# antonilo/unsupervised_detection

Hardware: NVIDIA B200
Metric: frame-pairs/sec adversarial train step 256x448 (higher is better)
Workload: dtype bf16

## Files before the change

### include/cis_b200.h

```cpp
#ifndef CIS_B200_H_
#define CIS_B200_H_
#include <stdint.h>
#include <stddef.h>

#ifdef __cplusplus
extern "C" {
#endif

typedef void* cis_stream_t;

enum { CIS_OK = 0, CIS_ERR_BAD_ARG = 1, CIS_ERR_UNSUPPORTED = 2, CIS_ERR_CUDA = 3 };
enum { CIS_ACT_NONE = 0, CIS_ACT_ELU = 1, CIS_ACT_LEAKY = 2 };
enum { CIS_MAX_TAPS = 49, CIS_MAX_SRC = 4 };

typedef struct {
  const void* ptr;
  int32_t pitch;
  int32_t c_off;
  int32_t chunks;
  int32_t n_mod;
} CisSrc;

typedef struct {
  int32_t N, H, W;
  int32_t OH, OW;
  int32_t sh, sw;
  int32_t ntaps;
  int16_t dh[CIS_MAX_TAPS];
  int16_t dw[CIS_MAX_TAPS];
  int32_t nsrc;
  CisSrc src[CIS_MAX_SRC];
  const void* wpack;
  int32_t K_pad;
  int32_t BN;
  int32_t n_tiles;
  const float* bias;
  int32_t act;
  float alpha;
  int32_t DH, DW;
  int32_t osh, osw, oa, ob;
  void* out;
  int32_t out_pitch, out_coff, out_ch;
  float* outf;
  int32_t outf_pitch, outf_coff, outf_ch;
  const void* add_pre;
  int32_t add_pre_pitch, add_pre_coff;
  const float* addf_pre;
  int32_t addf_pitch, addf_coff;
  const void* add_post;
  int32_t add_post_pitch, add_post_coff;
  int32_t mode;
  int32_t halo;
  int32_t dil;
  int32_t MT;
  int32_t hoy, hox;
  int32_t ey, ex;
  int32_t splits;
  float* sk_scratch;
  int32_t* sk_counters;
  int32_t nph;
  int32_t ph_tap[5];
  int32_t sk_cluster;
  int32_t nsub;
  struct {
    int32_t tap0, ntaps;
    int32_t hoy, hox;
    int32_t OH, OW, oa, ob;
    const void* wpack;
  } sub[4];
} CisConv;

typedef struct {
  int32_t N, H, W, OH, OW, sh, sw, ntaps;
  int16_t dh[CIS_MAX_TAPS];
  int16_t dw[CIS_MAX_TAPS];
  int32_t nsrc;
  CisSrc src[CIS_MAX_SRC];
  const void* g;
  int32_t g_pitch, g_coff, g_chunks;
  float* dwp;
  int32_t Cout;
  int32_t K_pad;
  int32_t splits;
  int32_t tma;
} CisWgrad;

const char* cis_last_error(void);
int cis_version(void);
uint32_t cis_crc32c(uint32_t crc, const void* data, size_t n);
int cis_host_resize_bilinear_legacy(const float* src, int32_t H, int32_t W, int32_t C, float* dst, int32_t OH, int32_t OW);
int cis_host_bgr8_to_rgb_resized(const unsigned char* bgr, int32_t H, int32_t W, float* dst, int32_t OH, int32_t OW);

int cis_conv_igemm(const CisConv* d, cis_stream_t stream);
int cis_set_persist_mode(int mode);
int cis_conv_wgrad(const CisWgrad* d, cis_stream_t stream);

int cis_pack_weights(const float* w, const int32_t* kmap, int32_t K_pad, int32_t rows, int32_t cout, int32_t sn, const int32_t* nmap,
                     void* wp, cis_stream_t stream);
int cis_pack_weights_tiled(const float* w, const int32_t* kmap, int32_t cin8, int32_t ntaps, int32_t n_tiles, int32_t BN, int32_t cout,
                           int32_t sn, const int32_t* nmap, void* out, cis_stream_t stream);
int cis_unpack_wgrad(const float* dwp, const int32_t* kmap, int32_t K_pad, int32_t cout, int32_t nsplit, float* dw, const float* colpart,
                     int32_t nblocks, int32_t nch, float* db, int32_t layout, cis_stream_t stream);
int cis_bn_fold(const float* w, const float* bias, const float* gamma, const float* beta, int64_t nw, int32_t cout, float* w_eff,
                float* b_eff, cis_stream_t stream);
int cis_bn_chain(const float* w, const float* bias, const float* gamma, float* dw_eff_to_dw, const float* db_eff, int64_t nw,
                 int32_t cout, float* dbias, float* dgamma, float* dbeta, cis_stream_t stream);

enum { CIS_JOB_PACK = 0, CIS_JOB_PACK_TILED = 1, CIS_JOB_UNPACK = 2, CIS_JOB_BN_FOLD = 3, CIS_JOB_BN_CHAIN = 4 };
typedef struct {
  int32_t kind;
  int32_t i[8];
  int64_t n;
  const void* p[8];
} CisParamJob;
int cis_param_multi(const CisParamJob* jobs_dev, int32_t njobs, int32_t total_blocks, cis_stream_t stream);

int cis_dact_mul(void* g, int32_t g_pitch, int32_t g_coff, const void* y, int32_t y_pitch, int32_t y_coff, const void* res,
                 int32_t res_pitch, int32_t res_coff, int64_t npix, int32_t chunks, int32_t act, float alpha, cis_stream_t stream);
int cis_add_slice(void* dst, int32_t dst_pitch, int32_t dst_coff, const void* src, int32_t src_pitch, int32_t src_coff,
                  int64_t npix_dst, int32_t chunks, int32_t reps, int32_t accumulate, cis_stream_t stream);
int cis_colsum(const void* g, int32_t g_pitch, int32_t g_coff, int64_t npix, int32_t nch, float* part, int32_t nblocks, cis_stream_t stream);

int cis_zero(void* ptr, int64_t nbytes, cis_stream_t stream);

int cis_dact_colsum(void* g, int32_t g_pitch, int32_t g_coff, const void* y, int32_t y_pitch, int32_t y_coff, const void* res,
                    int32_t res_pitch, int32_t res_coff, int64_t npix, int32_t nch, int32_t act, float alpha, float* part, int32_t nblocks,
                    cis_stream_t stream);

int cis_resize_bilinear_bf16(const void* src, int32_t s_pitch, int32_t s_coff, int32_t N, int32_t H, int32_t W, void* dst,
                             int32_t d_pitch, int32_t d_coff, int32_t OH, int32_t OW, int32_t chunks, cis_stream_t stream);
int cis_resize_concat_bf16(const CisSrc* srcs, int32_t nsrc, int32_t N, int32_t H, int32_t W, void* dst, int32_t d_pitch, int32_t d_coff,
                           int32_t OH, int32_t OW, cis_stream_t stream);
int cis_resize_concat_bf16_bwd(const void* ddst, int32_t d_pitch, int32_t d_coff, int32_t N, int32_t OH, int32_t OW, const CisSrc* grads,
                               const int32_t* want, const int32_t* accumulate, int32_t nsrc, int32_t H, int32_t W, cis_stream_t stream);
int cis_resize_bilinear_bf16_bwd(const void* ddst, int32_t d_pitch, int32_t d_coff, int32_t N, int32_t OH, int32_t OW, void* dsrc,
                                 int32_t s_pitch, int32_t s_coff, int32_t H, int32_t W, int32_t chunks, int32_t accumulate,
                                 cis_stream_t stream);
int cis_resize_bilinear_f32(const float* src, int32_t N, int32_t H, int32_t W, int32_t C, float* dst, int32_t OH, int32_t OW,
                            float scale, cis_stream_t stream);
int cis_upsample_nn2x(const void* src, int32_t N, int32_t H, int32_t W, int32_t pitch, void* dst, cis_stream_t stream);
int cis_upsample_nn2x_bwd(const void* ddst, int32_t N, int32_t H, int32_t W, int32_t pitch, void* dsrc, int32_t accumulate,
                          cis_stream_t stream);
int cis_crop_resize_bilinear_f32(const float* src, int32_t Hs, int32_t Ws, int32_t C, int32_t y0, int32_t x0, int32_t ch, int32_t cw, float* dst,
                                 int32_t OH, int32_t OW, cis_stream_t stream);
int cis_resize_nn_f32(const float* src, int32_t N, int32_t H, int32_t W, int32_t C, float* dst, int32_t OH, int32_t OW,
                      cis_stream_t stream);

int cis_warp_costvol(const void* c1, int32_t c1_pitch, int32_t c1_coff, const void* c2, int32_t c2_pitch, int32_t c2_coff,
                     const float* flow, float flow_scale, int32_t B, int32_t h, int32_t w, int32_t C, void* out, int32_t out_pitch,
                     int32_t out_coff, cis_stream_t stream);
int cis_dense_image_warp(const void* img, int32_t pitch, int32_t coff, const float* flow, float flow_scale, int32_t B, int32_t h,
                         int32_t w, int32_t C, void* out, int32_t out_pitch, cis_stream_t stream);

int cis_pack_f32_to_bf16(const float* src, int64_t npix, int32_t C, float offset, void* dst, int32_t d_pitch, int32_t d_coff,
                         cis_stream_t stream);
int cis_flow_stats(const float* flow, int32_t B, int64_t hw, double* stats, cis_stream_t stream);
int cis_pack_generator_input(const float* image, const float* flow, const double* stats, int32_t B, int64_t hw, void* dst,
                             cis_stream_t stream);

int cis_mask_apply(const float* flow, const float* mask, int32_t B, int64_t hw, void* dst, cis_stream_t stream);
int cis_charbonnier_sum(const float* gt, const float* pred, const float* mask, int32_t B, int64_t hw, int32_t C, int32_t mask_c, float cbn,
                        double* sums, cis_stream_t stream);
int cis_cis_loss_fwd(const float* flow, const float* mask, const float* flow1, int32_t B, int32_t H, int32_t W, int32_t h1,
                     int32_t w1, float cbn, double* sums, float* pred_out , cis_stream_t stream);
int cis_cis_loss_reduce(const double* sums, int32_t B, int32_t global_batch, int64_t hw, float epsilon, float* scalars, float* coef,
                        cis_stream_t stream);
int cis_cis_loss_bwd(const float* flow, const float* mask, const float* flow1, const float* coef, const float* scalars, int32_t B,
                     int32_t H, int32_t W, int32_t h1, int32_t w1, float cbn, int32_t which, float* dpred, float* dmask,
                     cis_stream_t stream);
int cis_resize_f32_bwd_to_bf16(const float* ddst, int32_t N, int32_t OH, int32_t OW, int32_t C, int32_t H, int32_t W, void* dsrc,
                               int32_t s_pitch, cis_stream_t stream);
int cis_mask_bwd(const float* flow, const float* mask, const float* dmask_direct, const void* d_in, int32_t B, int64_t hw,
                 void* dlogits, cis_stream_t stream);

int cis_abs_sum(const float* g, int64_t n, float* stat, cis_stream_t stream);
int cis_grad_avg_abs(const float* g, const int64_t* seg_off, int32_t nseg, float* out_avg, cis_stream_t stream);
int cis_clip_adam(float* param, float* m, float* v, const float* grad, int64_t n, float grad_scale, float clip, float lr, float beta1,
                  float beta2, float eps, int64_t* step_state, const float* avg_abs, int32_t can_change, uint64_t seed,
                  cis_stream_t stream);
int cis_cast_f32_to_bf16(const float* src, int64_t n, void* dst, cis_stream_t stream);
int cis_cast_bf16_to_f32(const void* src, int64_t npix, int32_t pitch, int32_t coff, int32_t C, float* dst, cis_stream_t stream);

#ifdef __cplusplus
// ... 4 lines not shown
```

### unsupervised_detection_b200/_lib.py

```python
import ctypes as C
import os

_HERE = os.path.dirname(os.path.abspath(__file__))
LIB_PATH = os.path.join(_HERE, os.environ.get('CIS_LIB_NAME', 'libcis_b200.so'))

MAX_TAPS, MAX_SRC = 49, 4
ACT_NONE, ACT_ELU, ACT_LEAKY = 0, 1, 2


class CisSrc(C.Structure):
    _fields_ = [('ptr', C.c_void_p), ('pitch', C.c_int32), ('c_off', C.c_int32), ('chunks', C.c_int32), ('n_mod', C.c_int32)]


class CisParamJob(C.Structure):
    _fields_ = [('kind', C.c_int32), ('i', C.c_int32 * 8), ('n', C.c_int64), ('p', C.c_void_p * 8)]


JOB_PACK, JOB_PACK_TILED, JOB_UNPACK, JOB_BN_FOLD, JOB_BN_CHAIN = range(5)


class CisSub(C.Structure):
    _fields_ = [('tap0', C.c_int32), ('ntaps', C.c_int32), ('hoy', C.c_int32), ('hox', C.c_int32), ('OH', C.c_int32), ('OW', C.c_int32),
                ('oa', C.c_int32), ('ob', C.c_int32), ('wpack', C.c_void_p)]


class CisConv(C.Structure):
    _fields_ = [('N', C.c_int32), ('H', C.c_int32), ('W', C.c_int32), ('OH', C.c_int32), ('OW', C.c_int32),
                ('sh', C.c_int32), ('sw', C.c_int32), ('ntaps', C.c_int32),
                ('dh', C.c_int16 * MAX_TAPS), ('dw', C.c_int16 * MAX_TAPS),
                ('nsrc', C.c_int32), ('src', CisSrc * MAX_SRC),
                ('wpack', C.c_void_p), ('K_pad', C.c_int32), ('BN', C.c_int32), ('n_tiles', C.c_int32),
                ('bias', C.c_void_p), ('act', C.c_int32), ('alpha', C.c_float),
                ('DH', C.c_int32), ('DW', C.c_int32), ('osh', C.c_int32), ('osw', C.c_int32), ('oa', C.c_int32), ('ob', C.c_int32),
                ('out', C.c_void_p), ('out_pitch', C.c_int32), ('out_coff', C.c_int32), ('out_ch', C.c_int32),
                ('outf', C.c_void_p), ('outf_pitch', C.c_int32), ('outf_coff', C.c_int32), ('outf_ch', C.c_int32),
                ('add_pre', C.c_void_p), ('add_pre_pitch', C.c_int32), ('add_pre_coff', C.c_int32),
                ('addf_pre', C.c_void_p), ('addf_pitch', C.c_int32), ('addf_coff', C.c_int32),
                ('add_post', C.c_void_p), ('add_post_pitch', C.c_int32), ('add_post_coff', C.c_int32),
                ('mode', C.c_int32),
                ('halo', C.c_int32), ('dil', C.c_int32), ('MT', C.c_int32), ('hoy', C.c_int32), ('hox', C.c_int32),
                ('ey', C.c_int32), ('ex', C.c_int32),
                ('splits', C.c_int32), ('sk_scratch', C.c_void_p), ('sk_counters', C.c_void_p),
                ('nph', C.c_int32), ('ph_tap', C.c_int32 * 5), ('sk_cluster', C.c_int32),
                ('nsub', C.c_int32), ('sub', CisSub * 4)]


class CisWgrad(C.Structure):
    _fields_ = [('N', C.c_int32), ('H', C.c_int32), ('W', C.c_int32), ('OH', C.c_int32), ('OW', C.c_int32),
                ('sh', C.c_int32), ('sw', C.c_int32), ('ntaps', C.c_int32),
                ('dh', C.c_int16 * MAX_TAPS), ('dw', C.c_int16 * MAX_TAPS),
                ('nsrc', C.c_int32), ('src', CisSrc * MAX_SRC),
                ('g', C.c_void_p), ('g_pitch', C.c_int32), ('g_coff', C.c_int32), ('g_chunks', C.c_int32),
                ('dwp', C.c_void_p), ('Cout', C.c_int32), ('K_pad', C.c_int32), ('splits', C.c_int32), ('tma', C.c_int32)]


_i32, _i64, _f32, _p, _u64 = C.c_int32, C.c_int64, C.c_float, C.c_void_p, C.c_uint64

_PROTOS = {
    'cis_conv_igemm': [C.POINTER(CisConv)],
    'cis_conv_wgrad': [C.POINTER(CisWgrad)],
    'cis_pack_weights': [_p, _p, _i32, _i32, _i32, _i32, _p, _p],
    'cis_pack_weights_tiled': [_p, _p, _i32, _i32, _i32, _i32, _i32, _i32, _p, _p],
    'cis_unpack_wgrad': [_p, _p, _i32, _i32, _i32, _p, _p, _i32, _i32, _p, _i32],
    'cis_bn_fold': [_p, _p, _p, _p, _i64, _i32, _p, _p],
    'cis_param_multi': [_p, _i32, _i32],
    'cis_bn_chain': [_p, _p, _p, _p, _p, _i64, _i32, _p, _p, _p],
    'cis_dact_mul': [_p, _i32, _i32, _p, _i32, _i32, _p, _i32, _i32, _i64, _i32, _i32, _f32],
    'cis_add_slice': [_p, _i32, _i32, _p, _i32, _i32, _i64, _i32, _i32, _i32],
    'cis_colsum': [_p, _i32, _i32, _i64, _i32, _p, _i32],
    'cis_zero': [_p, _i64],
    'cis_dact_colsum': [_p, _i32, _i32, _p, _i32, _i32, _p, _i32, _i32, _i64, _i32, _i32, _f32, _p, _i32],
    'cis_resize_bilinear_bf16': [_p, _i32, _i32, _i32, _i32, _i32, _p, _i32, _i32, _i32, _i32, _i32],
    'cis_resize_concat_bf16': [C.POINTER(CisSrc), _i32, _i32, _i32, _i32, _p, _i32, _i32, _i32, _i32],
    'cis_resize_concat_bf16_bwd': [_p, _i32, _i32, _i32, _i32, _i32, C.POINTER(CisSrc), C.POINTER(C.c_int32), C.POINTER(C.c_int32), _i32, _i32, _i32],
    'cis_resize_bilinear_bf16_bwd': [_p, _i32, _i32, _i32, _i32, _i32, _p, _i32, _i32, _i32, _i32, _i32, _i32],
    'cis_resize_bilinear_f32': [_p, _i32, _i32, _i32, _i32, _p, _i32, _i32, _f32],
    'cis_upsample_nn2x': [_p, _i32, _i32, _i32, _i32, _p],
    'cis_upsample_nn2x_bwd': [_p, _i32, _i32, _i32, _i32, _p, _i32],
    'cis_crop_resize_bilinear_f32': [_p, _i32, _i32, _i32, _i32, _i32, _i32, _i32, _p, _i32, _i32],
    'cis_resize_nn_f32': [_p, _i32, _i32, _i32, _i32, _p, _i32, _i32],
    'cis_warp_costvol': [_p, _i32, _i32, _p, _i32, _i32, _p, _f32, _i32, _i32, _i32, _i32, _p, _i32, _i32],
    'cis_dense_image_warp': [_p, _i32, _i32, _p, _f32, _i32, _i32, _i32, _i32, _p, _i32],
    'cis_pack_f32_to_bf16': [_p, _i64, _i32, _f32, _p, _i32, _i32],
    'cis_flow_stats': [_p, _i32, _i64, _p],
    'cis_pack_generator_input': [_p, _p, _p, _i32, _i64, _p],
    'cis_mask_apply': [_p, _p, _i32, _i64, _p],
    'cis_charbonnier_sum': [_p, _p, _p, _i32, _i64, _i32, _i32, _f32, _p],
    'cis_cis_loss_fwd': [_p, _p, _p, _i32, _i32, _i32, _i32, _i32, _f32, _p, _p],
    'cis_cis_loss_reduce': [_p, _i32, _i32, _i64, _f32, _p, _p],
    'cis_cis_loss_bwd': [_p, _p, _p, _p, _p, _i32, _i32, _i32, _i32, _i32, _f32, _i32, _p, _p],
    'cis_resize_f32_bwd_to_bf16': [_p, _i32, _i32, _i32, _i32, _i32, _i32, _p, _i32],
    'cis_mask_bwd': [_p, _p, _p, _p, _i32, _i64, _p],
    'cis_abs_sum': [_p, _i64, _p],
    'cis_grad_avg_abs': [_p, _p, _i32, _p],
    'cis_clip_adam': [_p, _p, _p, _p, _i64, _f32, _f32, _f32, _f32, _f32, _f32, _p, _p, _i32, _u64],
    'cis_cast_f32_to_bf16': [_p, _i64, _p],
    'cis_cast_bf16_to_f32': [_p, _i64, _i32, _i32, _i32, _p],
}
EXPORTS = sorted(list(_PROTOS) + ['cis_last_error', 'cis_version', 'cis_set_persist_mode', 'cis_crc32c', 'cis_host_resize_bilinear_legacy',
                                  'cis_host_bgr8_to_rgb_resized'])

_lib = None


def load():
    global _lib
    if _lib is None:
        if not os.path.exists(LIB_PATH):
            raise RuntimeError('libcis_b200.so not built: run `python -c "import __graft_entry__ as g; g.build()"` '
                               '(no CPU fallback exists for the product path)')
        lib = C.CDLL(LIB_PATH)
        lib.cis_last_error.restype = C.c_char_p
        lib.cis_version.restype = C.c_int
        lib.cis_set_persist_mode.argtypes = [C.c_int]
        lib.cis_set_persist_mode.restype = C.c_int
        lib.cis_crc32c.argtypes = [C.c_uint32, C.c_void_p, C.c_size_t]
        lib.cis_crc32c.restype = C.c_uint32
        lib.cis_host_resize_bilinear_legacy.argtypes = [C.c_void_p, C.c_int32, C.c_int32, C.c_int32, C.c_void_p, C.c_int32, C.c_int32]
        lib.cis_host_resize_bilinear_legacy.restype = C.c_int
        lib.cis_host_bgr8_to_rgb_resized.argtypes = [C.c_void_p, C.c_int32, C.c_int32, C.c_void_p, C.c_int32, C.c_int32]
        lib.cis_host_bgr8_to_rgb_resized.restype = C.c_int
        for name, args in _PROTOS.items():
            fn = getattr(lib, name)
            fn.argtypes = list(args) + [C.c_void_p]
            fn.restype = C.c_int
        _lib = lib
    return _lib


def check(rc, what=''):
    if rc != 0:
        raise RuntimeError('libcis_b200 %s failed (code %d): %s' % (what, rc, load().cis_last_error().decode()))


def call(name, *args):
    check(getattr(load(), name)(*args), name)
```

### unsupervised_detection_b200/csrc/conv_igemm.cu

```cuda
#include "ptx.cuh"
#include "../../include/cis_b200.h"
#include "common.cuh"
#include <cuda.h>
#include <stdlib.h>
#include <string.h>


namespace cis {

#ifdef CIS_TRACE
__device__ unsigned long long* g_trace = nullptr;
__device__ int g_trace_cap = 0;
#define CIS_TRACE_AT(slot)                                                                                         \
  do {                                                                                                             \
    if (g_trace && blockIdx.x == 0 && blockIdx.y == 0 && blockIdx.z == 0 && (slot) < g_trace_cap) g_trace[(slot)] = clock64(); \
  } while (0)
#else
#define CIS_TRACE_AT(slot) ((void)0)
#endif

static constexpr int kBM = 128;
static constexpr int kBK = 64;
static constexpr int kAStage = kBM * 128;
static constexpr int kThreads = 160;
// ... 421 lines not shown
    for (int i = Cfg::kLag - 1; i >= 0; --i) {
      if (nkb - 1 - i < 0) continue;
      if (i == 3) cp_async_wait<3>();
      else if (i == 2) cp_async_wait<2>();
      else if (i == 1) cp_async_wait<1>();
      else cp_async_wait<0>();
      fence_proxy_async();
      mbar_arrive(bar_full + 8 * ((nkb - 1 - i) % S));
    }

    mbar_wait(bar_accum, 0);
    tc_fence_after();
    if (tid == 0) CIS_TRACE_AT(2);
    const int qtr = warp & 3, half = warp >> 2;
    const int row = qtr * 32 + lane;
    const int g = blockIdx.x * kBM + row;
    const bool valid = g < M;
    size_t dpix = 0;
    if (valid) {
      const int ow = g % p.OW;
      const int t = g / p.OW;
      const int oh = t % p.OH;
      const int n = t / p.OH;
      dpix = (size_t)(n * p.DH + oh * p.osh + p.oa) * p.DW + ow * p.osw + p.ob;
    }
    const uint32_t t_row = tmem + ((uint32_t)(qtr * 32) << 16);
    const int cbase = ny * BN;
    constexpr int kHalf = BN >= 32 ? BN / 2 : BN;
    const int c_lo = half * kHalf, c_hi = (BN >= 32 || half == 0) ? c_lo + kHalf : c_lo;
    if (nsplit > 1 && p.sk_cluster) {
      tmem_to_stage(t_row, row, tile_base, c_lo, c_hi);
    } else if (nsplit > 1) {
      const int tile_id = blockIdx.x * gridDim.y + ny;
      float* tile0 = p.sk_scratch + (size_t)tile_id * nsplit * kBM * BN;
      splitk_store_partial<BN>(tile0 + (size_t)blockIdx.z * kBM * BN, t_row, row, c_lo, c_hi);
    } else {
      epi_cols<BN>(p, t_row, cbase, dpix, valid, s_bias, c_lo, c_hi);
    }
  } else {
    constexpr uint32_t idesc = make_idesc_bf16(kBM, BN, 0, 0);
    for (int kb = 0; kb < nkb; ++kb) {
      const int s = kb % S;
      const uint32_t ph = (uint32_t)((kb / S) & 1);
      mbar_wait(bar_full + 8 * s, ph);
      tc_fence_after();
      if (elect_one()) {
        CIS_TRACE_AT(8 + 2 * kb);
        const uint32_t alo = desc_lo(a_base + s * kAStage, 16), blo = desc_lo(b_base + s * Cfg::kBStage, 16);
        const uint32_t dhi = desc_hi(1024);
#pragma unroll
        for (int k = 0; k < kBK / 16; ++k) umma_bf16_lh(tmem, alo + 2 * k, dhi, blo + 2 * k, dhi, idesc, (uint32_t)((kb | k) != 0));
        umma_commit(bar_empty + 8 * s);
        if (kb == nkb - 1) umma_commit(bar_accum);
        CIS_TRACE_AT(9 + 2 * kb);
      }
      __syncwarp();
    }
  }
  if (nsplit > 1 && p.sk_cluster) {
    cluster_sync_all();
    if (warp < kMmaWarp) {
      const int cbase = ny * BN;
      cluster_reduce_rows<BN>(p, tile_base, nsplit, (int)cluster_ctarank(), tid, kGProducers, cbase, [&](int row, bool& valid) -> size_t {
        const int g = blockIdx.x * kBM + row;
        valid = g < M;
        if (!valid) return 0;
        const int ow = g % p.OW;
        const int t = g / p.OW;
        const int oh = t % p.OH;
        const int n = t / p.OH;
        return (size_t)(n * p.DH + oh * p.osh + p.oa) * p.DW + ow * p.osw + p.ob;
      });
    }
    cluster_sync_all();
  }
  tc_fence_before();
  __syncthreads();
  if (tid == 0) CIS_TRACE_AT(3);
  if (warp == kMmaWarp) tmem_dealloc<Cfg::kTmemCols>(tmem);
}


static constexpr int kHaloMaxBStages = 8;
struct HaloMaps {
  CUtensorMap m[CIS_MAX_SRC * 4];
};

template <int NK>
__device__ __forceinline__ void halo_issue_mt1(const uint32_t tmem, const uint32_t hlo, uint32_t blo, const uint32_t* s_aoff, const int gt,
                                               const uint32_t bstep, const uint32_t ahi, const uint32_t bhi, const uint32_t idesc,
                                               const bool first) {
  int tt = 0;
  uint32_t acc = first ? 0u : 1u;
  uint32_t o0 = 0, o1 = 0, o2 = 0, o3 = 0;
  if (gt >= 4) {
    o0 = s_aoff[0];
    o1 = s_aoff[1];
    o2 = s_aoff[2];
    o3 = s_aoff[3];
  }
  for (; tt + 4 <= gt; tt += 4) {
    const uint32_t a0 = hlo + o0, a1 = hlo + o1, a2 = hlo + o2, a3 = hlo + o3;
    if (tt + 8 <= gt) {
      o0 = s_aoff[tt + 4];
      o1 = s_aoff[tt + 5];
      o2 = s_aoff[tt + 6];
      o3 = s_aoff[tt + 7];
    }
#pragma unroll
    for (int k = 0; k < NK; ++k) umma_bf16_lh(tmem, a0 + 2 * k, ahi, blo + 2 * k, bhi, idesc, k ? 1u : acc);
#pragma unroll
    for (int k = 0; k < NK; ++k) umma_bf16_lh(tmem, a1 + 2 * k, ahi, blo + bstep + 2 * k, bhi, idesc, 1u);
#pragma unroll
    for (int k = 0; k < NK; ++k) umma_bf16_lh(tmem, a2 + 2 * k, ahi, blo + 2 * bstep + 2 * k, bhi, idesc, 1u);
#pragma unroll
    for (int k = 0; k < NK; ++k) umma_bf16_lh(tmem, a3 + 2 * k, ahi, blo + 3 * bstep + 2 * k, bhi, idesc, 1u);
    acc = 1u;
    blo += 4 * bstep;
  }
  if (tt < gt) {
    const uint32_t r0 = s_aoff[tt], r1 = tt + 1 < gt ? s_aoff[tt + 1] : 0u, r2 = tt + 2 < gt ? s_aoff[tt + 2] : 0u;
#pragma unroll
    for (int k = 0; k < NK; ++k) umma_bf16_lh(tmem, hlo + r0 + 2 * k, ahi, blo + 2 * k, bhi, idesc, k ? 1u : acc);
    if (tt + 1 < gt) {
#pragma unroll
      for (int k = 0; k < NK; ++k) umma_bf16_lh(tmem, hlo + r1 + 2 * k, ahi, blo + bstep + 2 * k, bhi, idesc, 1u);
    }
    if (tt + 2 < gt) {
#pragma unroll
      for (int k = 0; k < NK; ++k) umma_bf16_lh(tmem, hlo + r2 + 2 * k, ahi, blo + 2 * bstep + 2 * k, bhi, idesc, 1u);
    }
  }
}

template <int NK>
__device__ __forceinline__ void halo_issue_stage(const uint32_t tmem, const uint32_t hlo, uint32_t blo, const uint32_t* s_aoff, const int gt,
                                                 const int MT, const int BN, const uint32_t ahi, const uint32_t bhi, const uint32_t a_mstep,
                                                 const uint32_t idesc, const bool first) {
  const uint32_t bstep = (uint32_t)(BN * 128) >> 4;
  if (NK == 1 && MT == 1) {
    halo_issue_mt1<NK>(tmem, hlo, blo, s_aoff, gt, bstep, ahi, bhi, idesc, first);
    return;
  }
  uint32_t off0 = s_aoff[0], off1 = gt > 1 ? s_aoff[1] : 0u;
#pragma unroll 2
  for (int tt = 0; tt < gt; ++tt, blo += bstep) {
    const uint32_t off2 = tt + 2 < gt ? s_aoff[tt + 2] : 0u;
    uint32_t alo = hlo + off0;
    const uint32_t acc0 = (uint32_t)(!(first && tt == 0));
    if (MT == 1) {
#pragma unroll
      for (int k = 0; k < NK; ++k) umma_bf16_lh(tmem, alo + 2 * k, ahi, blo + 2 * k, bhi, idesc, k ? 1u : acc0);
    } else {
      for (int m = 0; m < MT; ++m, alo += a_mstep) {
        const uint32_t td = tmem + m * BN;
#pragma unroll
        for (int k = 0; k < NK; ++k) umma_bf16_lh(td, alo + 2 * k, ahi, blo + 2 * k, bhi, idesc, k ? 1u : acc0);
      }
    }
    off0 = off1;
    off1 = off2;
  }
}

template <int BN>
__global__ void __launch_bounds__(HaloCfg<BN>::kThreads, HaloCfg<BN>::kMinCtas) conv_halo_kernel(const __grid_constant__ CisConv p, const int halo_stage_bytes, const int BS, const int NHS,
                                                        const __grid_constant__ HaloMaps maps, const int use_tma, const int G) {
  constexpr int kBStage = BN * 128;
  constexpr int kHMmaWarp_ = HaloCfg<BN>::kMmaWarp, kHThreads_ = HaloCfg<BN>::kThreads;
  extern __shared__ uint8_t smem_raw[];
  __shared__ uint64_t bars[2 * 2 + 2 * kHaloMaxBStages + 1];
  __shared__ uint32_t tmem_slot;
  __shared__ uint32_t s_aoff[CIS_MAX_TAPS];
  __shared__ SrcS s_src[CIS_MAX_SRC];

  const int tid = threadIdx.x, warp = tid >> 5, lane = tid & 31;
  const int MT = p.MT, d = p.dil;
  const int nph = p.nph > 1 ? p.nph : 1;
  const int Wh = 8 + p.ex, Hh = 16 * MT + p.ey, HP = Wh * Hh;
  const uint32_t stage_bytes = (uint32_t)G * kBStage;
  const uint32_t tile_base = (smem_u32(smem_raw) + 1023u) & ~1023u;
  const uint32_t h_base = tile_base;
  const uint32_t b_base = tile_base + NHS * halo_stage_bytes;
  int* pixtab = reinterpret_cast<int*>(smem_raw + (b_base + BS * stage_bytes - smem_u32(smem_raw)));
  const uint32_t bar_hfull = smem_u32(&bars[0]), bar_hempty = smem_u32(&bars[2]);
  const uint32_t bar_bfull = smem_u32(&bars[4]), bar_bempty = smem_u32(&bars[4 + kHaloMaxBStages]);
  const uint32_t bar_accum = smem_u32(&bars[4 + 2 * kHaloMaxBStages]);

  const bool grouped = p.nsub > 1;
  const int tap0 = grouped ? p.sub[blockIdx.z].tap0 : 0, ntaps = grouped ? p.sub[blockIdx.z].ntaps : p.ntaps;
  const int hoy = grouped ? p.sub[blockIdx.z].hoy : p.hoy, hox = grouped ? p.sub[blockIdx.z].hox : p.hox;
  const int OHs = grouped ? p.sub[blockIdx.z].OH : p.OH, OWs = grouped ? p.sub[blockIdx.z].OW : p.OW;
  const int oa = grouped ? p.sub[blockIdx.z].oa : p.oa, ob = grouped ? p.sub[blockIdx.z].ob : p.ob;
  const void* const wpack = grouped ? p.sub[blockIdx.z].wpack : p.wpack;
  const int Hp0 = (OHs + d - 1) / d, Wp0 = (OWs + d - 1) / d;
  const int tiles_x = (Wp0 + 7) / 8, tiles_y = (Hp0 + 16 * MT - 1) / (16 * MT);
  if (grouped && (int)blockIdx.x >= tiles_x * tiles_y * p.N) return;
  int bid = blockIdx.x;
  const int tx = bid % tiles_x; bid /= tiles_x;
  const int ty = bid % tiles_y; bid /= tiles_y;
  const int ph = bid % (d * d);
  const int n = bid / (d * d);
  const int pa = ph / d, pb = ph % d;
  const int ny = blockIdx.y;
  int m_chunks = 0;
  for (int i = 0; i < p.nsrc; ++i) m_chunks += p.src[i].chunks;
  const int nchunks_all = (m_chunks + 7) / 8;
  const int nsplit = (!grouped && p.splits > 1) ? p.splits : 1;
  const int cper = (nchunks_all + nsplit - 1) / nsplit;
  const int cc_lo = grouped ? 0 : blockIdx.z * cper;
  const int nchunks = min(cper, nchunks_all - cc_lo);
  __shared__ __align__(16) float s_bias[BN];
  pdl_launch_dependents();
  const uint32_t ncols = (MT * BN <= 32) ? 32u : (MT * BN <= 64) ? 64u : (MT * BN <= 128) ? 128u : (MT * BN <= 256) ? 256u : 512u;

  if (tid < ntaps) s_aoff[tid] = (uint32_t)((p.dh[tap0 + tid] * Wh + p.dw[tap0 + tid]) * 8);
  if (tid < p.nsrc) {
    s_src[tid].ptr = reinterpret_cast<const __nv_bfloat16*>(p.src[tid].ptr);
    s_src[tid].pitch = p.src[tid].pitch;
    s_src[tid].c_off = p.src[tid].c_off;
    s_src[tid].chunks = p.src[tid].chunks;
    s_src[tid].n_mod = p.src[tid].n_mod;
  }
  for (int q = tid; q < (use_tma ? 0 : HP); q += kHThreads_) {
    const int hy = q / Wh, hx = q - hy * Wh;
    const int gy = ty * 16 * MT + hy + hoy, gx = tx * 8 + hx + hox;
    const int y = pa + d * gy, x = pb + d * gx;
    pixtab[q] = (gy >= 0 && gx >= 0 && y < p.H && x < p.W) ? (y * p.W + x) : -1;
  }
  if (warp == kHMmaWarp_) {
    if (lane == 0) {
      for (int s = 0; s < 2; ++s) {
        mbar_init(bar_hfull + 8 * s, use_tma ? 1 : 96);
        mbar_init(bar_hempty + 8 * s, 1);
      }
      for (int s = 0; s < BS; ++s) {
        mbar_init(bar_bfull + 8 * s, 1);
        mbar_init(bar_bempty + 8 * s, 1);
      }
      mbar_init(bar_accum, 1);
      fence_mbar_init();
    }
    __syncwarp();
    tmem_alloc_dyn(smem_u32(&tmem_slot), ncols);
  }
  if (use_tma && tid < p.nsrc) tma_prefetch_desc(&maps.m[tid]);
  pdl_wait();
  if (tid < BN) s_bias[tid] = p.bias ? p.bias[ny * BN + tid] : 0.f;
  tc_fence_before();
  __syncthreads();
  tc_fence_after();
  const uint32_t tmem = tmem_slot;
  if (tid == 0) CIS_TRACE_AT(0);

  if (warp < kHMmaWarp_) {
   if (warp < 4) {
    if (use_tma) {
      if (tid == 0) {
        int hcount = 0;
        for (int vc = 0; vc < nchunks * nph; ++vc) {
          const int cc = vc / nph, ph = vc - cc * nph;
          if (nph > 1 && p.ph_tap[ph + 1] == p.ph_tap[ph]) continue;
          const int hs = hcount % NHS;
          mbar_wait(bar_hempty + 8 * hs, (uint32_t)(((hcount / NHS) & 1) ^ 1));
          ++hcount;
          int c = (cc_lo + cc) * 8, si = 0;
          while (si < p.nsrc - 1 && c >= s_src[si].chunks) {
            c -= s_src[si].chunks;
            ++si;
          }
          const int nmod = s_src[si].n_mod;
          mbar_expect_tx(bar_hfull + 8 * hs, (uint32_t)(HP * 128));
          tma_load_4d(h_base + hs * halo_stage_bytes, &maps.m[si * nph + ph], bar_hfull + 8 * hs, c * 8, pb + d * (tx * 8 + hox),
                      pa + d * (ty * 16 * MT + hoy), nmod ? (n % nmod) : n);
        }
      }
      __syncwarp();
    } else if (warp != 2) {
      const int hid = warp == 3 ? tid - 32 : tid;
      const int j = hid & 7, pl = hid >> 3;
      for (int cc = 0; cc < nchunks; ++cc) {
        const int hs = cc % NHS;
        mbar_wait(bar_hempty + 8 * hs, (uint32_t)(((cc / NHS) & 1) ^ 1));
        const int rem = m_chunks - (cc_lo + cc) * 8;
        const int nk16 = rem >= 8 ? 4 : (rem + 1) / 2;
        const bool need = j < 2 * nk16;
        const bool cvalid = j < rem;
        int c = (cc_lo + cc) * 8 + j, si = 0;
        if (cvalid) {
          while (si < p.nsrc - 1 && c >= s_src[si].chunks) {
            c -= s_src[si].chunks;
            ++si;
          }
        } else {
          c = 0;
        }
        const int nmod = s_src[si].n_mod, pitch = s_src[si].pitch;
        const int ne = nmod ? (n % nmod) : n;
        const __nv_bfloat16* sp = s_src[si].ptr;
        const __nv_bfloat16* sb = sp + (size_t)ne * p.H * p.W * pitch + s_src[si].c_off + c * 8;
        if (need) {
          const uint32_t hdst = h_base + hs * halo_stage_bytes + (uint32_t)(j << 4);
          for (int q = pl; q < HP; q += 12) {
            const int off = pixtab[q];
            const bool ok = cvalid && off >= 0;
            cp_async16((hdst + q * 128) ^ (uint32_t)((q & 7) << 4), ok ? (const void*)(sb + (size_t)off * pitch) : (const void*)sp,
                       ok ? 16u : 0u);
          }
        }
        cp_async_commit();
        if (NHS == 1) {
          cp_async_wait<0>();
          fence_proxy_async();
          mbar_arrive(bar_hfull);
        } else if (cc >= 1) {
          cp_async_wait<1>();
          fence_proxy_async();
          mbar_arrive(bar_hfull + 8 * ((cc - 1) % NHS));
        }
      }
      if (NHS > 1) {
        cp_async_wait<0>();
        fence_proxy_async();
        mbar_arrive(bar_hfull + 8 * ((nchunks - 1) % NHS));
      }
    }
    if (tid == 64) {
      const uint8_t* wt = reinterpret_cast<const uint8_t*>(wpack) + ((size_t)ny * nchunks_all + cc_lo) * ntaps * kBStage;
      int bs = 0;
      uint32_t bph = 1;
      for (int vc = 0; vc < nchunks * nph; ++vc) {
        const int cc = vc / nph, ph = vc - cc * nph;
        const int tlo = nph > 1 ? p.ph_tap[ph] : 0, thi = nph > 1 ? p.ph_tap[ph + 1] : ntaps;
        for (int t0 = tlo; t0 < thi; t0 += G) {
          const uint32_t bytes = (uint32_t)min(G, thi - t0) * kBStage;
          mbar_wait(bar_bempty + 8 * bs, bph);
          mbar_expect_tx(bar_bfull + 8 * bs, bytes);
          bulk_g2s(b_base + bs * stage_bytes, wt + (size_t)(cc * ntaps + t0) * kBStage, bytes, bar_bfull + 8 * bs);
          if (++bs == BS) {
            bs = 0;
            bph ^= 1u;
          }
        }
      }
    }
    __syncwarp();
   }

    mbar_wait(bar_accum, 0);
    tc_fence_after();
    if (tid == 0) CIS_TRACE_AT(2);
    const int qtr = warp & 3, half = warp >> 2;
    const int r = qtr * 32 + lane;
    const int c_lo = (kHMmaWarp_ == 8) ? half * (BN / 2) : 0, c_hi = (kHMmaWarp_ == 8) ? c_lo + BN / 2 : BN;
    const uint32_t t_qtr = tmem + ((uint32_t)(qtr * 32) << 16);
    const int cbase = ny * BN;
    const int tile_id = blockIdx.x * gridDim.y + ny;
    if (nsplit > 1 && p.sk_cluster) {
      for (int m = 0; m < MT; ++m)
        if (c_lo < c_hi) tmem_to_stage(t_qtr + m * BN, r, tile_base + (uint32_t)m * (kBM * BN * 4), c_lo, c_hi);
    } else if (nsplit > 1) {
      for (int m = 0; m < MT; ++m)
        if (c_lo < c_hi)
          splitk_store_partial<BN>(p.sk_scratch + (((size_t)tile_id * MT + m) * nsplit + blockIdx.z) * kBM * BN, t_qtr + m * BN, r, c_lo, c_hi);
    } else if (c_lo < c_hi) {
      for (int m = 0; m < MT; ++m) {
        const int gy = ty * 16 * MT + 16 * m + (r >> 3), gx = tx * 8 + (r & 7);
        const int oy = pa + d * gy, ox = pb + d * gx;
        const bool valid = oy < OHs && ox < OWs;
        const size_t dpix = valid ? ((size_t)(n * p.DH + oy * p.osh + oa) * p.DW + ox * p.osw + ob) : 0;
        epi_cols<BN>(p, t_qtr + m * BN, cbase, dpix, valid, s_bias, c_lo, c_hi);
      }
    }
  } else {
    constexpr uint32_t idesc = make_idesc_bf16(kBM, BN, 0, 0);
    const uint32_t ahi = desc_hi((uint32_t)(Wh * 128)), bhi = desc_hi(1024);
    const uint32_t a_mstep = (uint32_t)(16 * Wh * 128) >> 4;
    int bs = 0, hs = 0, it = 0;
    uint32_t bph = 0, hph = 0;
    int vlast = nchunks * nph - 1;
    while (nph > 1 && vlast > 0 && p.ph_tap[vlast % nph + 1] == p.ph_tap[vlast % nph]) --vlast;
    bool any = false;
    for (int vc = 0; vc < nchunks * nph; ++vc) {
      const int cc = vc / nph, ph = vc - cc * nph;
      const int tlo = nph > 1 ? p.ph_tap[ph] : 0, thi = nph > 1 ? p.ph_tap[ph + 1] : ntaps;
      if (thi == tlo) continue;
      const int rem = m_chunks - (cc_lo + cc) * 8;
      const int nk16 = rem >= 8 ? 4 : (rem + 1) / 2;
      mbar_wait(bar_hfull + 8 * hs, hph);
      if (vc == 0 && lane == 0) CIS_TRACE_AT(1);
      const uint32_t hlo = desc_lo(h_base + hs * halo_stage_bytes, 16);
      for (int t0 = tlo; t0 < thi; t0 += G, ++it) {
        const int gt = min(G, thi - t0);
        mbar_wait(bar_bfull + 8 * bs, bph);
        tc_fence_after();
        if (elect_one()) {
          CIS_TRACE_AT(8 + 2 * it);
          const uint32_t blo = desc_lo(b_base + bs * stage_bytes, 16);
          const bool first = !any;
          if (nk16 == 4) halo_issue_stage<4>(tmem, hlo, blo, s_aoff + t0, gt, MT, BN, ahi, bhi, a_mstep, idesc, first);
          else if (nk16 == 1) halo_issue_stage<1>(tmem, hlo, blo, s_aoff + t0, gt, MT, BN, ahi, bhi, a_mstep, idesc, first);
          else if (nk16 == 2) halo_issue_stage<2>(tmem, hlo, blo, s_aoff + t0, gt, MT, BN, ahi, bhi, a_mstep, idesc, first);
          else halo_issue_stage<3>(tmem, hlo, blo, s_aoff + t0, gt, MT, BN, ahi, bhi, a_mstep, idesc, first);
          umma_commit(bar_bempty + 8 * bs);
          if (t0 + G >= thi) {
            umma_commit(bar_hempty + 8 * hs);
            if (vc == vlast) umma_commit(bar_accum);
          }
          CIS_TRACE_AT(9 + 2 * it);
        }
        __syncwarp();
        any = true;
        if (++bs == BS) {
          bs = 0;
          bph ^= 1u;
        }
      }
      if (++hs == NHS) {
        hs = 0;
        hph ^= 1u;
      }
    }
  }
  if (nsplit > 1 && p.sk_cluster) {
    cluster_sync_all();
    if (warp < 4) {
      const int cbase = ny * BN;
      for (int m = 0; m < MT; ++m)
        cluster_reduce_rows<BN>(p, tile_base + (uint32_t)m * (kBM * BN * 4), nsplit, (int)cluster_ctarank(), tid, 128, cbase,
                                [&](int row, bool& valid) -> size_t {
                                  const int gy = ty * 16 * MT + 16 * m + (row >> 3), gx = tx * 8 + (row & 7);
                                  const int oy = pa + d * gy, ox = pb + d * gx;
                                  valid = oy < OHs && ox < OWs;
                                  return valid ? ((size_t)(n * p.DH + oy * p.osh + oa) * p.DW + ox * p.osw + ob) : 0;
                                });
    }
    cluster_sync_all();
  }
  tc_fence_before();
  __syncthreads();
  if (tid == 0) CIS_TRACE_AT(3);
  if (warp == kHMmaWarp_) tmem_dealloc_dyn(tmem, ncols);
}

template <int BN>
__global__ void __launch_bounds__(256) splitk_finish_kernel(const __grid_constant__ CisConv p) {
  constexpr int G = BN / 16;
  constexpr int kBlock = (128 * G < 256) ? 128 * G : 256;
  constexpr int kSub = 128 * G / kBlock;
  pdl_launch_dependents();
  pdl_wait();
  const int tid = threadIdx.x;
  if (tid >= kBlock) return;
  const int m = blockIdx.z / kSub;
  const int item = (blockIdx.z % kSub) * kBlock + tid;
  const int r = item % 128, c0 = (item / 128) * 16;
  const int ny = blockIdx.y;
  const int nsplit = p.splits;
  const int tile_id = blockIdx.x * gridDim.y + ny;
  bool valid;
  size_t dpix = 0;
  const float* tile0;
  if (p.halo) {
    const int MT = p.MT, d = p.dil;
    const int Hp0 = (p.OH + d - 1) / d, Wp0 = (p.OW + d - 1) / d;
    const int tiles_x = (Wp0 + 7) / 8, tiles_y = (Hp0 + 16 * MT - 1) / (16 * MT);
    int bid = blockIdx.x;
    const int tx = bid % tiles_x; bid /= tiles_x;
    const int ty = bid % tiles_y; bid /= tiles_y;
    const int ph = bid % (d * d);
    const int n = bid / (d * d);
    const int pa = ph / d, pb = ph % d;
    const int gy = ty * 16 * MT + 16 * m + (r >> 3), gx = tx * 8 + (r & 7);
    const int oy = pa + d * gy, ox = pb + d * gx;
    valid = oy < p.OH && ox < p.OW;
    if (valid) dpix = (size_t)(n * p.DH + oy * p.osh + p.oa) * p.DW + ox * p.osw + p.ob;
    tile0 = p.sk_scratch + ((size_t)tile_id * MT + m) * nsplit * kBM * BN;
  } else {
    const int M = p.N * p.OH * p.OW;
    const int g = blockIdx.x * kBM + r;
    valid = g < M;
    if (valid) {
      const int ow = g % p.OW;
      const int t = g / p.OW;
      const int oh = t % p.OH;
      const int n = t / p.OH;
      dpix = (size_t)(n * p.DH + oh * p.osh + p.oa) * p.DW + ow * p.osw + p.ob;
    }
    tile0 = p.sk_scratch + (size_t)tile_id * nsplit * kBM * BN;
  }
  if (!valid) return;
  float v[16];
  splitk_reduce16<BN>(tile0, nsplit, r, c0, v);
  epi_chunk(p, v, ny * BN + c0, dpix);
}
static constexpr int kPThreads = 384;

template <int BN>
__global__ void __launch_bounds__(kPThreads, 2) conv_halo_persist_kernel(const __grid_constant__ CisConv p, const int halo_stage_bytes,
                                                                       const int BS, const int NHS, const int AS, const int G,
                                                                       const __grid_constant__ HaloMaps maps, const int ws) {
  constexpr int kBStage = BN * 128;
  constexpr int kMaxHS = 4;
  extern __shared__ uint8_t smem_raw[];
  __shared__ uint64_t bars[2 * kMaxHS + 2 * kHaloMaxBStages + 4];
  __shared__ uint32_t tmem_slot;
  __shared__ uint32_t s_aoff[CIS_MAX_TAPS];
  __shared__ __align__(16) float s_bias[BN];

  const int tid = threadIdx.x, warp = tid >> 5, lane = tid & 31;
  const int MT = p.MT;
  const int Wh = 8 + p.ex, Hh = 16 * MT + p.ey, HP = Wh * Hh;
  const uint32_t stage_bytes = (uint32_t)G * kBStage;
  const uint32_t tile_base = (smem_u32(smem_raw) + 1023u) & ~1023u;
  const uint32_t h_base = tile_base, b_base = tile_base + NHS * halo_stage_bytes;
  const uint32_t bar_hfull = smem_u32(&bars[0]), bar_hempty = smem_u32(&bars[kMaxHS]);
  const uint32_t bar_bfull = smem_u32(&bars[2 * kMaxHS]), bar_bempty = smem_u32(&bars[2 * kMaxHS + kHaloMaxBStages]);
  const uint32_t bar_tfull = smem_u32(&bars[2 * kMaxHS + 2 * kHaloMaxBStages]), bar_tempty = smem_u32(&bars[2 * kMaxHS + 2 * kHaloMaxBStages + 2]);

  const int tiles_x = (p.OW + 7) / 8, tiles_y = (p.OH + 16 * MT - 1) / (16 * MT);
  const int total = tiles_x * tiles_y * p.N;
  int m_chunks = 0;
  for (int i = 0; i < p.nsrc; ++i) m_chunks += p.src[i].chunks;
  const int nchunks = (m_chunks + 7) / 8;
  const uint32_t acc_cols = (uint32_t)(MT * BN);
  const uint32_t want = acc_cols * AS;
  const uint32_t ncols = want <= 32 ? 32u : want <= 64 ? 64u : want <= 128 ? 128u : want <= 256 ? 256u : 512u;

  pdl_launch_dependents();
  if (tid < p.ntaps) s_aoff[tid] = (uint32_t)((p.dh[tid] * Wh + p.dw[tid]) * 8);
  if (warp == 3) {
    if (lane == 0) {
      for (int s = 0; s < NHS; ++s) {
        mbar_init(bar_hfull + 8 * s, 1);
        mbar_init(bar_hempty + 8 * s, 1);
      }
      for (int s = 0; s < BS; ++s) {
        mbar_init(bar_bfull + 8 * s, 1);
        mbar_init(bar_bempty + 8 * s, 1);
      }
      for (int s = 0; s < AS; ++s) {
        mbar_init(bar_tfull + 8 * s, 1);
        mbar_init(bar_tempty + 8 * s, 4);
      }
      fence_mbar_init();
    }
    __syncwarp();
    tmem_alloc_dyn(smem_u32(&tmem_slot), ncols);
  }
  if (tid < p.nsrc) tma_prefetch_desc(&maps.m[tid]);
  pdl_wait();
  if (tid < BN) s_bias[tid] = p.bias ? p.bias[tid] : 0.f;
  tc_fence_before();
  __syncthreads();
  tc_fence_after();
  const uint32_t tmem = tmem_slot;
  if (tid == 0) {
    CIS_TRACE_AT(0);
    CIS_TRACE_AT(4);
  }

  if (warp == 0) {
    if (lane == 0) {
      int hs = 0;
      uint32_t hph = 1;
      for (int w = blockIdx.x; w < total; w += gridDim.x) {
        const int tx = w % tiles_x, r1 = w / tiles_x, ty = r1 % tiles_y, n = r1 / tiles_y;
        for (int cc = 0; cc < nchunks; ++cc) {
          mbar_wait(bar_hempty + 8 * hs, hph);
          int c = cc * 8, si = 0;
          while (si < p.nsrc - 1 && c >= p.src[si].chunks) {
            c -= p.src[si].chunks;
            ++si;
          }
          int nmod = p.src[0].n_mod;
          if (si == 1) nmod = p.src[1].n_mod;
          if (si == 2) nmod = p.src[2].n_mod;
          if (si == 3) nmod = p.src[3].n_mod;
          mbar_expect_tx(bar_hfull + 8 * hs, (uint32_t)(HP * 128));
          tma_load_4d(h_base + hs * halo_stage_bytes, &maps.m[si], bar_hfull + 8 * hs, c * 8, tx * 8 + p.hox, ty * 16 * MT + p.hoy,
                      nmod ? (n % nmod) : n);
          if (++hs == NHS) {
            hs = 0;
            hph ^= 1u;
          }
        }
      }
    }
  } else if (warp == 1) {
    if (lane == 0) {
      const uint8_t* wt = reinterpret_cast<const uint8_t*>(p.wpack);
      const int per_tile = nchunks * p.ntaps;
      if (ws) {
        if ((int)blockIdx.x < total) {
          mbar_expect_tx(bar_bfull, (uint32_t)(per_tile * kBStage));
          for (int it = 0; it < per_tile; it += 8) {
            const int nt = min(8, per_tile - it);
            bulk_g2s(b_base + it * kBStage, wt + (size_t)it * kBStage, (uint32_t)(nt * kBStage), bar_bfull);
          }
        }
      } else {
        int bs = 0;
        uint32_t bph = 1;
        for (int w = blockIdx.x; w < total; w += gridDim.x) {
          for (int cc = 0; cc < nchunks; ++cc) {
            for (int t0 = 0; t0 < p.ntaps; t0 += G) {
              const uint32_t bytes = (uint32_t)min(G, p.ntaps - t0) * kBStage;
              mbar_wait(bar_bempty + 8 * bs, bph);
              mbar_expect_tx(bar_bfull + 8 * bs, bytes);
              bulk_g2s(b_base + bs * stage_bytes, wt + (size_t)(cc * p.ntaps + t0) * kBStage, bytes, bar_bfull + 8 * bs);
              if (++bs == BS) {
                bs = 0;
                bph ^= 1u;
              }
            }
          }
        }
      }
    }
  } else if (warp == 2) {
    constexpr uint32_t idesc = make_idesc_bf16(kBM, BN, 0, 0);
    const uint32_t ahi = desc_hi((uint32_t)(Wh * 128)), bhi = desc_hi(1024);
    const uint32_t a_mstep = (uint32_t)(16 * Wh * 128) >> 4;
    int hs = 0, bs = 0, as = 0;
    uint32_t hph = 0, bph = 0, tph = 1;
    if (ws && (int)blockIdx.x < total) {
      mbar_wait(bar_bfull, 0u);
      tc_fence_after();
    }
    int wi = 0;
    for (int w = blockIdx.x; w < total; w += gridDim.x, ++wi) {
      if (lane == 0) CIS_TRACE_AT(8 + 5 * wi);
      mbar_wait(bar_tempty + 8 * as, tph);
      tc_fence_after();
      if (lane == 0) CIS_TRACE_AT(9 + 5 * wi);
      const uint32_t tacc = tmem + as * acc_cols;
      for (int cc = 0; cc < nchunks; ++cc) {
        const int rem = m_chunks - cc * 8;
        const int nk16 = rem >= 8 ? 4 : (rem + 1) / 2;
        mbar_wait(bar_hfull + 8 * hs, hph);
        if (cc == 0 && lane == 0) CIS_TRACE_AT(10 + 5 * wi);
        const uint32_t hlo = desc_lo(h_base + hs * halo_stage_bytes, 16);
        const int gstep = ws ? p.ntaps : G;
        for (int t0 = 0; t0 < p.ntaps; t0 += gstep) {
          const int gt = min(gstep, p.ntaps - t0);
          if (!ws) mbar_wait(bar_bfull + 8 * bs, bph);
          tc_fence_after();
          if (elect_one()) {
            const uint32_t blo = desc_lo(ws ? b_base + (uint32_t)(cc * p.ntaps) * kBStage : b_base + bs * stage_bytes, 16);
            const bool first = (cc | t0) == 0;
            if (nk16 == 4) halo_issue_stage<4>(tacc, hlo, blo, s_aoff + t0, gt, MT, BN, ahi, bhi, a_mstep, idesc, first);
            else if (nk16 == 1) halo_issue_stage<1>(tacc, hlo, blo, s_aoff + t0, gt, MT, BN, ahi, bhi, a_mstep, idesc, first);
            else if (nk16 == 2) halo_issue_stage<2>(tacc, hlo, blo, s_aoff + t0, gt, MT, BN, ahi, bhi, a_mstep, idesc, first);
            else halo_issue_stage<3>(tacc, hlo, blo, s_aoff + t0, gt, MT, BN, ahi, bhi, a_mstep, idesc, first);
            if (!ws) umma_commit(bar_bempty + 8 * bs);
            if (t0 + gstep >= p.ntaps) {
              umma_commit(bar_hempty + 8 * hs);
              if (cc == nchunks - 1) {
                umma_commit(bar_tfull + 8 * as);
                CIS_TRACE_AT(11 + 5 * wi);
              }
            }
          }
          __syncwarp();
          if (!ws && ++bs == BS) {
            bs = 0;
            bph ^= 1u;
          }
        }
        if (++hs == NHS) {
          hs = 0;
          hph ^= 1u;
        }
      }
      if (++as == AS) {
        as = 0;
        tph ^= 1u;
      }
    }
  } else if (warp >= 4) {
    const int grp = (warp - 4) >> 2, q = warp & 3;
    const int r = q * 32 + lane;
    if (grp < AS) {
      uint32_t tph = 0;
      int wi = 0;
      for (int w = blockIdx.x; w < total; w += gridDim.x, ++wi) {
        if (wi % AS != grp) continue;
        const int tx = w % tiles_x, r1 = w / tiles_x, ty = r1 % tiles_y, n = r1 / tiles_y;
        mbar_wait(bar_tfull + 8 * grp, tph);
        tph ^= 1u;
        tc_fence_after();
        for (int m = 0; m < MT; ++m) {
          const int oy = ty * 16 * MT + 16 * m + (r >> 3), ox = tx * 8 + (r & 7);
          const bool valid = oy < p.OH && ox < p.OW;
          const size_t dpix = valid ? ((size_t)(n * p.DH + oy * p.osh + p.oa) * p.DW + ox * p.osw + p.ob) : 0;
          epi_row<BN>(p, tmem + ((uint32_t)(q * 32) << 16) + grp * acc_cols + m * BN, 0, dpix, valid, s_bias);
        }
        tc_fence_before();
        __syncwarp();
        if (lane == 0) mbar_arrive(bar_tempty + 8 * grp);
        if (q == 0 && lane == 0) CIS_TRACE_AT(12 + 5 * wi);
      }
    }
  }
  tc_fence_before();
  __syncthreads();
  if (warp == 3) tmem_dealloc_dyn(tmem, ncols);
}

static constexpr int kWStages = 3;
static constexpr int kWTile = 64 * 128;
static constexpr int kWStage = 4 * kWTile;
static constexpr int kWSmem = kWStages * kWStage + 1024;

struct WgradMaps {
  CUtensorMap g;
  CUtensorMap x[CIS_MAX_SRC];
};

__global__ void __launch_bounds__(kGThreads) conv_wgrad_kernel(const __grid_constant__ CisWgrad p, const __grid_constant__ WgradMaps maps) {
  constexpr int S = kWStages;
  extern __shared__ uint8_t smem_raw[];
  __shared__ uint64_t bars[2 * S + 1];
  __shared__ uint32_t tmem_slot;
  __shared__ int s_dh[CIS_MAX_TAPS], s_dw[CIS_MAX_TAPS];
  const uint32_t tile_base = (smem_u32(smem_raw) + 1023u) & ~1023u;
  const uint32_t bar_full = smem_u32(&bars[0]);
  const uint32_t bar_empty = smem_u32(&bars[S]);
  const uint32_t bar_accum = smem_u32(&bars[2 * S]);
  const int tid = threadIdx.x, warp = tid >> 5, lane = tid & 31;
  const int nprod = (int)blockDim.x - 32, mma_warp = nprod >> 5;
  pdl_launch_dependents();
  if (tid < p.ntaps) {
    s_dh[tid] = p.dh[tid];
    s_dw[tid] = p.dw[tid];
  }
  const int M = p.N * p.OH * p.OW;
// ... 336 lines not shown
  cfg.dynamicSmemBytes = smem;
  cfg.stream = st;
  cudaLaunchAttribute attr[1];
  attr[0].id = cudaLaunchAttributeProgrammaticStreamSerialization;
  attr[0].val.programmaticStreamSerializationAllowed = 1;
  cfg.attrs = attr;
  cfg.numAttrs = pdl_enabled() ? 1 : 0;
  return cudaLaunchKernelEx(&cfg, kern, KArgs(args)...);
}

template <typename... KArgs, typename... Args>
static cudaError_t launch_pdl_zcluster(void (*kern)(KArgs...), dim3 grid, dim3 block, size_t smem, cudaStream_t st, int cz, Args... args) {
  cudaLaunchConfig_t cfg;
  memset(&cfg, 0, sizeof(cfg));
  cfg.gridDim = grid;
  cfg.blockDim = block;
  cfg.dynamicSmemBytes = smem;
  cfg.stream = st;
  cudaLaunchAttribute attr[2];
  attr[0].id = cudaLaunchAttributeClusterDimension;
  attr[0].val.clusterDim.x = 1;
  attr[0].val.clusterDim.y = 1;
  attr[0].val.clusterDim.z = cz;
  attr[1].id = cudaLaunchAttributeProgrammaticStreamSerialization;
  attr[1].val.programmaticStreamSerializationAllowed = 1;
  cfg.attrs = attr;
  cfg.numAttrs = pdl_enabled() ? 2 : 1;
  return cudaLaunchKernelEx(&cfg, kern, KArgs(args)...);
}

template <int BN>
static cudaError_t launch_splitk_finish(const CisConv* d, dim3 main_grid, cudaStream_t st) {
  constexpr int G = BN / 16;
  constexpr int kBlock = (128 * G < 256) ? 128 * G : 256;
  constexpr int kSub = 128 * G / kBlock;
  const int mt = d->halo ? d->MT : 1;
  return launch_pdl(splitk_finish_kernel<BN>, dim3(main_grid.x, main_grid.y, mt * kSub), dim3(kBlock), 0, st, *d);
}

template <int BN>
static int launch_fwd(const CisConv* d, cudaStream_t st) {
  using Cfg = FwdCfg<BN>;
  static bool attr_set = false;
  if (!attr_set) {
    cudaError_t e = cudaFuncSetAttribute(conv_igemm_kernel<BN>, cudaFuncAttributeMaxDynamicSharedMemorySize, Cfg::kSmem);
    if (e != cudaSuccess) return cis_set_cuda_error(e, "cudaFuncSetAttribute(conv_igemm)");
    attr_set = true;
  }
  const int M = d->N * d->OH * d->OW;
  int splits = d->splits > 1 ? d->splits : 1;
  if (splits > 1) {
    const int nkb = d->K_pad / kBK, per = (nkb + splits - 1) / splits;
    if ((!d->sk_scratch && !d->sk_cluster) || d->sk_counters || (splits - 1) * per >= nkb || (d->sk_cluster && splits > 8))
      return cis_set_error(CIS_ERR_BAD_ARG, "cis_conv_igemm: bad split-K setup");
  }
  dim3 grid((M + kBM - 1) / kBM, d->n_tiles, splits);
  cudaError_t le = (splits > 1 && d->sk_cluster)
                       ? launch_pdl_zcluster(conv_igemm_kernel<BN>, grid, dim3(kGThreads), Cfg::kSmem, st, splits, *d)
                       : launch_pdl(conv_igemm_kernel<BN>, grid, dim3(kGThreads), Cfg::kSmem, st, *d);
  if (le != cudaSuccess) return cis_set_cuda_error(le, "launch(conv_igemm)");
  if (splits > 1 && !d->sk_cluster) {
    le = launch_splitk_finish<BN>(d, grid, st);
    if (le != cudaSuccess) return cis_set_cuda_error(le, "launch(splitk_finish)");
  }
  return cis_check_launch("conv_igemm");
}


typedef CUresult (*EncodeTiledFn)(CUtensorMap*, CUtensorMapDataType, cuuint32_t, void*, const cuuint64_t*, const cuuint64_t*, const cuuint32_t*,
                                  const cuuint32_t*, CUtensorMapInterleave, CUtensorMapSwizzle, CUtensorMapL2promotion, CUtensorMapFloatOOBfill);
static EncodeTiledFn get_encode_tiled() {
  static EncodeTiledFn fn = nullptr;
  static bool tried = false;
  if (!tried) {
    tried = true;
    void* p = nullptr;
    cudaDriverEntryPointQueryResult q;
    if (cudaGetDriverEntryPoint("cuTensorMapEncodeTiled", &p, cudaEnableDefault, &q) == cudaSuccess && q == cudaDriverEntryPointSuccess)
      fn = (EncodeTiledFn)p;
  }
  return fn;
}
static bool encode_src_map(CUtensorMap* m, const CisSrc& s, int N, int H, int W, int bw, int bh, int step = 1, int py = 0, int px = 0,
                           int estride = 1) {
  EncodeTiledFn enc = get_encode_tiled();
  if (!enc) return false;
  const int nb = s.n_mod > 0 ? s.n_mod : N;
  const int Hq = (H - py + step - 1) / step, Wq = (W - px + step - 1) / step;
  if (Hq < 1 || Wq < 1) return false;
  cuuint64_t dims[4] = {(cuuint64_t)s.chunks * 8, (cuuint64_t)Wq, (cuuint64_t)Hq, (cuuint64_t)nb};
  cuuint64_t strides[3] = {(cuuint64_t)step * s.pitch * 2, (cuuint64_t)step * W * s.pitch * 2, (cuuint64_t)H * W * s.pitch * 2};
  cuuint32_t box[4] = {64, (cuuint32_t)(bw * estride), (cuuint32_t)(bh * estride), 1};
  cuuint32_t es[4] = {1, (cuuint32_t)estride, (cuuint32_t)estride, 1};
  void* base = (void*)((const char*)s.ptr + ((size_t)(py * W + px) * s.pitch + (size_t)s.c_off) * 2);
  return enc(m, CU_TENSOR_MAP_DATA_TYPE_BFLOAT16, 4, base, dims, strides, box, es, CU_TENSOR_MAP_INTERLEAVE_NONE, CU_TENSOR_MAP_SWIZZLE_128B,
             CU_TENSOR_MAP_L2_PROMOTION_L2_128B, CU_TENSOR_MAP_FLOAT_OOB_FILL_NONE) == CUDA_SUCCESS;
}

#ifdef CIS_TRACE
extern "C" int cis_trace_set(unsigned long long* buf, int cap) {
  cudaError_t e = cudaMemcpyToSymbol(cis::g_trace, &buf, sizeof(buf));
  if (e == cudaSuccess) e = cudaMemcpyToSymbol(cis::g_trace_cap, &cap, sizeof(cap));
  return e == cudaSuccess ? CIS_OK : cis_set_cuda_error(e, "cis_trace_set");
}
#endif

static int g_persist_mode = -1;
extern "C" int cis_set_persist_mode(int mode) {
  g_persist_mode = mode;
  return CIS_OK;
}

template <int BN>
static int launch_halo(const CisConv* d, cudaStream_t st) {
  const int Wh = 8 + d->ex, Hh = 16 * d->MT + d->ey, HP = Wh * Hh;
  const int halo_stage = (HP * 128 + 1023) & ~1023;
  int chunks = 0;
  for (int i = 0; i < d->nsrc; ++i) chunks += d->src[i].chunks;
  const int nchunks = (chunks + 7) / 8;
  const int nsub = d->nsub > 1 ? d->nsub : 1;
  const int nsp = (nsub == 1 && d->splits > 1) ? d->splits : 1;
  const int cper = (nchunks + nsp - 1) / nsp;
  const int nhs = cper > 1 ? 2 : 1;
  const int dd = d->dil;
  int tiles = 0, ntaps_max = d->ntaps;
  if (nsub > 1) {
    if (nsub > 4 || dd != 1 || d->splits > 1 || d->nph > 1) return cis_set_error(CIS_ERR_BAD_ARG, "cis_conv_igemm(halo): bad grouped launch");
    ntaps_max = 0;
    int tsum = 0;
    for (int i = 0; i < nsub; ++i) {
      const int t = ((d->sub[i].OW + 7) / 8) * ((d->sub[i].OH + 16 * d->MT - 1) / (16 * d->MT));
      if (t > tiles) tiles = t;
      if (d->sub[i].ntaps > ntaps_max) ntaps_max = d->sub[i].ntaps;
      if (d->sub[i].ntaps < 1 || d->sub[i].tap0 != tsum || !d->sub[i].wpack) return cis_set_error(CIS_ERR_BAD_ARG, "cis_conv_igemm(halo): bad sub-problem");
      tsum += d->sub[i].ntaps;
    }
    if (tsum != d->ntaps) return cis_set_error(CIS_ERR_BAD_ARG, "cis_conv_igemm(halo): sub-problem taps must add up to ntaps");
  } else {
    const int Hp0 = (d->OH + dd - 1) / dd, Wp0 = (d->OW + dd - 1) / dd;
    tiles = ((Wp0 + 7) / 8) * ((Hp0 + 16 * d->MT - 1) / (16 * d->MT));
  }
  const long ncta_all = (long)tiles * dd * dd * d->N * d->n_tiles * nsp * nsub;
  static const int g_env = getenv("CIS_HALO_G") ? atoi(getenv("CIS_HALO_G")) : 0;
  static const int stage_kb = getenv("CIS_HALO_STAGE_KB") ? atoi(getenv("CIS_HALO_STAGE_KB")) : 48;
  const int kB = BN * 128;
  int G = g_env > 0 ? g_env : (stage_kb * 1024) / kB;
  if (G < 1) G = 1;
  if (G > ntaps_max) G = ntaps_max;
  const int fixed = nhs * halo_stage + HP * 4 + 1024;
  static const int lim_small_kb = getenv("CIS_HALO_SMALL_KB") ? atoi(getenv("CIS_HALO_SMALL_KB")) : 226;
  static const int lim_kb_wide = getenv("CIS_HALO_LIMIT_KB") ? atoi(getenv("CIS_HALO_LIMIT_KB")) : 113;
  static const int lim_kb_thin = getenv("CIS_HALO_LIMIT_THIN_KB") ? atoi(getenv("CIS_HALO_LIMIT_THIN_KB")) : 113;
  const int lim_kb = BN <= 32 ? lim_kb_thin : lim_kb_wide;
  int limit = (ncta_all > 148 && fixed + 2 * kB <= lim_kb * 1024) ? lim_kb * 1024 : 226 * 1024;
  if (ncta_all <= 148 && fixed + 2 * kB <= lim_small_kb * 1024) limit = lim_small_kb * 1024;
  while (G > 1 && fixed + 2 * G * kB > limit) --G;
  const int groups = cper * ((nsub > 1 ? 1 : (ntaps_max + G - 1) / G));
  int BS = (limit - fixed) / (G * kB);
  if (BS > (ncta_all > 148 ? 4 : kHaloMaxBStages)) BS = ncta_all > 148 ? 4 : kHaloMaxBStages;
  if (BS > groups) BS = groups;
  if (BS < 1) return cis_set_error(CIS_ERR_UNSUPPORTED, "cis_conv_igemm(halo): tile does not fit shared memory");
  int smem = fixed + BS * G * kB;
  if (nsp > 1 && d->sk_cluster && smem < d->MT * kBM * BN * 4 + 1024) smem = d->MT * kBM * BN * 4 + 1024;
  if (smem > 226 * 1024) return cis_set_error(CIS_ERR_UNSUPPORTED, "cis_conv_igemm(halo): cluster split-K staging does not fit shared memory");
  static int attr_smem = 0;
  if (smem > attr_smem) {
    cudaError_t e = cudaFuncSetAttribute(conv_halo_kernel<BN>, cudaFuncAttributeMaxDynamicSharedMemorySize, smem);
    if (e != cudaSuccess) return cis_set_cuda_error(e, "cudaFuncSetAttribute(conv_halo)");
    attr_smem = smem;
  }

  int splits = d->splits > 1 ? d->splits : 1;
  if (splits > 1) {
    const int per = (nchunks + splits - 1) / splits;
    if ((!d->sk_scratch && !d->sk_cluster) || d->sk_counters || (splits - 1) * per >= nchunks || (d->sk_cluster && splits > 8))
      return cis_set_error(CIS_ERR_BAD_ARG, "cis_conv_igemm(halo): bad split-K setup");
  }
  dim3 grid(tiles * dd * dd * d->N, d->n_tiles, nsub > 1 ? nsub : splits);
  HaloMaps maps;
  const int nph = d->nph > 1 ? d->nph : 1;
  static const int dil_tma = getenv("CIS_DIL_TMA") ? atoi(getenv("CIS_DIL_TMA")) : 1;
  int use_tma = ((d->dil == 1 || dil_tma) && Wh * d->dil <= 256 && Hh * d->dil <= 256) ? 1 : 0;
  for (int i = 0; use_tma && i < d->nsrc - 1; ++i)
    if (d->src[i].chunks % 8) use_tma = 0;
  for (int i = 0; use_tma && i < d->nsrc; ++i) {
    if (((uintptr_t)d->src[i].ptr + (size_t)d->src[i].c_off * 2) % 16) use_tma = 0;
    for (int ph = 0; use_tma && ph < nph; ++ph)
      if (!encode_src_map(&maps.m[i * nph + ph], d->src[i], d->N, d->H, d->W, Wh, Hh, nph > 1 ? 2 : 1, ph >> 1, ph & 1, d->dil)) use_tma = 0;
  }
  if (!use_tma) memset(&maps, 0, sizeof(maps));
  if (nph > 1 && !use_tma) return cis_set_error(CIS_ERR_UNSUPPORTED, "cis_conv_igemm(halo): stride-2 phases need the TMA halo path");
  const int persist_mode = g_persist_mode >= 0 ? g_persist_mode : (getenv("CIS_PERSIST_MODE") ? atoi(getenv("CIS_PERSIST_MODE")) : 1);
  static const int p_min_tiles = getenv("CIS_PERSIST_MIN_TILES") ? atoi(getenv("CIS_PERSIST_MIN_TILES")) : 296;
  static const int p_ws_kb = getenv("CIS_PERSIST_WS_KB") ? atoi(getenv("CIS_PERSIST_WS_KB")) : 112;
  if (persist_mode > 0 && use_tma && d->n_tiles == 1 && splits == 1 && nph == 1 && nsub == 1 && dd == 1) {
    const int total = tiles * d->N;
    const int per_tile = nchunks * d->ntaps;
    const int AS = (2 * d->MT * BN <= 512) ? 2 : 1;
    const int ws_bytes = per_tile * kB;
    int p_nhs = nchunks >= 3 ? 4 : 3;
    while (p_nhs > 2 && p_nhs * halo_stage + 1024 + (ws_bytes <= p_ws_kb * 1024 ? ws_bytes : 2 * G * kB) > 226 * 1024) --p_nhs;
    const bool ws_fits = ws_bytes <= p_ws_kb * 1024 && p_nhs * halo_stage + 1024 + ws_bytes <= 226 * 1024;
    const bool take = persist_mode == 2 || (persist_mode == 3 && ws_fits) || (persist_mode == 1 && ws_fits && total >= p_min_tiles);
    int p_bs = 0, p_smem = 0;
    if (ws_fits) {
      p_bs = 1;
      p_smem = p_nhs * halo_stage + 1024 + ws_bytes;
    } else {
      p_bs = (226 * 1024 - p_nhs * halo_stage - 1024) / (G * kB);
      if (p_bs > 4) p_bs = 4;
      p_smem = p_nhs * halo_stage + 1024 + p_bs * G * kB;
    }
    if (take && p_bs >= (ws_fits ? 1 : 2)) {
      static int attr_p = 0;
      if (p_smem > attr_p) {
        cudaError_t e = cudaFuncSetAttribute(conv_halo_persist_kernel<BN>, cudaFuncAttributeMaxDynamicSharedMemorySize, p_smem);
        if (e != cudaSuccess) return cis_set_cuda_error(e, "cudaFuncSetAttribute(conv_halo_persist)");
        attr_p = p_smem;
      }
      const int want = AS * d->MT * BN;
      const int tcols = want <= 32 ? 32 : want <= 64 ? 64 : want <= 128 ? 128 : want <= 256 ? 256 : 512;
      int cps = (227 * 1024) / (p_smem + 1024);
      if (cps > 512 / tcols) cps = 512 / tcols;
      if (cps > 2048 / kPThreads) cps = 2048 / kPThreads;
      if (cps > 2) cps = 2;
      if (cps < 1) cps = 1;
      int g = total < 148 * cps ? total : 148 * cps;
      cudaError_t le = launch_pdl(conv_halo_persist_kernel<BN>, dim3(g), dim3(kPThreads), p_smem, st, *d, halo_stage, p_bs, p_nhs, AS, G, maps,
                                  ws_fits ? 1 : 0);
      if (le != cudaSuccess) return cis_set_cuda_error(le, "launch(conv_halo_persist)");
      return cis_check_launch("conv_halo_persist");
    }
  }
  cudaError_t le = (splits > 1 && d->sk_cluster)
                       ? launch_pdl_zcluster(conv_halo_kernel<BN>, grid, dim3(HaloCfg<BN>::kThreads), smem, st, splits, *d, halo_stage, BS, nhs, maps, use_tma, G)
                       : launch_pdl(conv_halo_kernel<BN>, grid, dim3(HaloCfg<BN>::kThreads), smem, st, *d, halo_stage, BS, nhs, maps, use_tma, G);
  if (le != cudaSuccess) return cis_set_cuda_error(le, "launch(conv_halo)");
  if (splits > 1 && !d->sk_cluster) {
    le = launch_splitk_finish<BN>(d, grid, st);
    if (le != cudaSuccess) return cis_set_cuda_error(le, "launch(splitk_finish)");
  }
  return cis_check_launch("conv_halo");
}

extern "C" int cis_conv_igemm(const CisConv* d, cis_stream_t stream) {
  if (!d || d->ntaps < 1 || d->ntaps > CIS_MAX_TAPS || d->nsrc < 1 || d->nsrc > CIS_MAX_SRC || d->K_pad % 64 != 0 || d->K_pad <= 0 ||
      d->n_tiles < 1 || !d->wpack)
    return cis_set_error(CIS_ERR_BAD_ARG, "cis_conv_igemm: bad descriptor");
  int chunks = 0;
  for (int i = 0; i < d->nsrc; ++i) {
    if ((d->src[i].pitch | d->src[i].c_off) & 7) return cis_set_error(CIS_ERR_BAD_ARG, "cis_conv_igemm: source pitch/c_off must be multiples of 8");
    chunks += d->src[i].chunks;
  }
  if (d->ntaps * chunks * 8 > d->K_pad) return cis_set_error(CIS_ERR_BAD_ARG, "cis_conv_igemm: K_pad smaller than taps*channels");
  if (d->mode == 1 && !d->outf) return cis_set_error(CIS_ERR_BAD_ARG, "cis_conv_igemm: mode 1 needs outf");
  if ((d->add_pre || d->add_post) && (((d->add_pre_pitch | d->add_pre_coff | d->add_post_pitch | d->add_post_coff | d->out_ch) & 7) != 0))
    return cis_set_error(CIS_ERR_BAD_ARG, "cis_conv_igemm: residual slices must be 8-channel aligned");
  cudaStream_t st = (cudaStream_t)stream;
  if (d->halo) {
    if (d->MT < 1 || d->MT > 4 || d->MT * d->BN > 512 || d->dil < 1 || d->sh != 1 || d->sw != 1 || d->ey < 0 || d->ex < 0 ||
        (d->dil > 1 && (d->OH != d->H || d->OW != d->W)) || (d->nph > 1 && (d->nph != 4 || d->dil != 1 || d->ph_tap[0] != 0 || d->ph_tap[4] != d->ntaps)))
      return cis_set_error(CIS_ERR_BAD_ARG, "cis_conv_igemm(halo): bad tile parameters");
    switch (d->BN) {
      case 16: return launch_halo<16>(d, st);
      case 32: return launch_halo<32>(d, st);
      case 64: return launch_halo<64>(d, st);
      case 128: return launch_halo<128>(d, st);
      default: return cis_set_error(CIS_ERR_UNSUPPORTED, "cis_conv_igemm: BN must be 16/32/64/128");
    }
  }
  switch (d->BN) {
    case 16: return launch_fwd<16>(d, st);
    case 32: return launch_fwd<32>(d, st);
// ... 93 lines not shown
```

### unsupervised_detection_b200/csrc/misc_kernels.cu

```cuda
#include "ptx.cuh"
#include "../../include/cis_b200.h"
#include "common.cuh"
#include <math.h>

namespace cis {

typedef __nv_bfloat16 bf16;

__device__ __forceinline__ void unpack8(const uint4& u, float* f) {
  f[0] = bf16lo(u.x); f[1] = bf16hi(u.x); f[2] = bf16lo(u.y); f[3] = bf16hi(u.y);
  f[4] = bf16lo(u.z); f[5] = bf16hi(u.z); f[6] = bf16lo(u.w); f[7] = bf16hi(u.w);
}
__device__ __forceinline__ uint4 pack8(const float* f) {
  return make_uint4(pack_bf16(f[0], f[1]), pack_bf16(f[2], f[3]), pack_bf16(f[4], f[5]), pack_bf16(f[6], f[7]));
}
__device__ __forceinline__ float warp_sum(float v) {
#pragma unroll
  for (int o = 16; o > 0; o >>= 1) v += __shfl_xor_sync(0xffffffffu, v, o);
  return v;
}
__device__ __forceinline__ double warp_sum_d(double v) {
#pragma unroll
  for (int o = 16; o > 0; o >>= 1) v += __shfl_xor_sync(0xffffffffu, v, o);
  return v;
}

__device__ __forceinline__ void pack_weights_body(size_t i, const float* __restrict__ w, const int* __restrict__ kmap, int K_pad, int rows, int cout,
                                                  int sn, const int* __restrict__ nmap, bf16* __restrict__ wp) {
  if (i >= (size_t)rows * K_pad) return;
  const int n = (int)(i / K_pad), k = (int)(i % K_pad);
  const int km = kmap[k];
  const int ne = nmap ? nmap[n] : (n < cout ? n : -1);
  const float v = (km >= 0 && ne >= 0) ? w[(size_t)km + (size_t)ne * sn] : 0.f;
  wp[i] = __float2bfloat16(v);
}
__device__ __forceinline__ void pack_weights_tiled_body(size_t i, const float* __restrict__ w, const int* __restrict__ kmap, int cin8, int ntaps,
                                                        int n_tiles, int BN, int cout, int sn, const int* __restrict__ nmap,
                                                        bf16* __restrict__ out) {
  const int nchunks = (cin8 + 63) / 64;
  const size_t total = (size_t)n_tiles * nchunks * ntaps * BN * 64;
  if (i >= total) return;
  const int pos = (int)(i % 64);
  size_t r = i / 64;
  const int n = (int)(r % BN); r /= BN;
  const int t = (int)(r % ntaps); r /= ntaps;
  const int cc = (int)(r % nchunks);
  const int ny = (int)(r / nchunks);
  const int kk = (((pos >> 3) ^ (n & 7)) << 3) | (pos & 7);
  const int c = cc * 64 + kk;
  float v = 0.f;
  if (c < cin8) {
    const int km = kmap[t * cin8 + c];
    const int ng = ny * BN + n;
    const int ne = nmap ? nmap[ng] : (ng < cout ? ng : -1);
    if (km >= 0 && ne >= 0) v = w[(size_t)km + (size_t)ne * sn];
  }
  out[i] = __float2bfloat16(v);
}
__device__ __forceinline__ void pack_weights_tiled_tile(int blk, const float* __restrict__ w, const int* __restrict__ kmap, int cin8, int ntaps,
                                                        int n_tiles, int BN, int cout, const int* __restrict__ nmap, bf16* __restrict__ out,
                                                        float* tile) {
  const int nchunks = (cin8 + 63) / 64;
  const int t = blk % ntaps;
  const int r = blk / ntaps;
  const int cc = r % nchunks, ny = r / nchunks;
  const int ld = BN + 1;
  for (int idx = threadIdx.x; idx < BN * 64; idx += blockDim.x) {
    const int n = idx % BN, kk = idx / BN;
    const int c = cc * 64 + kk;
    float v = 0.f;
    if (c < cin8) {
      const int km = kmap[t * cin8 + c];
      const int ng = ny * BN + n;
      const int ne = nmap ? nmap[ng] : (ng < cout ? ng : -1);
      if (km >= 0 && ne >= 0) v = w[(size_t)km + ne];
    }
    tile[kk * ld + n] = v;
  }
  __syncthreads();
  bf16* o = out + (size_t)blk * BN * 64;
  for (int idx = threadIdx.x; idx < BN * 64; idx += blockDim.x) {
    const int pos = idx & 63, n = idx >> 6;
    const int kk = (((pos >> 3) ^ (n & 7)) << 3) | (pos & 7);
    o[idx] = __float2bfloat16(tile[kk * ld + n]);
  }
}
__device__ __forceinline__ void unpack_wgrad_body(size_t i, const float* __restrict__ dwp, const int* __restrict__ kmap, int K_pad, int cout,
                                                  int nsplit, float* __restrict__ dw, const float* __restrict__ colpart, int nblocks, int nch,
                                                  float* __restrict__ db, int layout) {
  const size_t nw = (size_t)cout * K_pad;
  if (i < nw) {
    int n, k;
    if (layout == 0) {
      n = (int)(i / K_pad);
      k = (int)(i % K_pad);
    } else {
      const size_t g4 = i / ((size_t)cout * 4);
      const int rem = (int)(i - g4 * cout * 4);
      n = rem >> 2;
      k = (int)g4 * 4 + (rem & 3);
    }
    const int km = kmap[k];
    if (km < 0) return;
    float a[8] = {0.f, 0.f, 0.f, 0.f, 0.f, 0.f, 0.f, 0.f};
    const float* q = dwp + i;
    int s = 0;
    for (; s + 8 <= nsplit; s += 8) {
      float t[8];
#pragma unroll
      for (int u = 0; u < 8; ++u) t[u] = __ldcg(q + (size_t)(s + u) * nw);
#pragma unroll
      for (int u = 0; u < 8; ++u) a[u] += t[u];
    }
    for (; s < nsplit; ++s) a[0] += __ldcg(q + (size_t)s * nw);
    dw[(size_t)km + n] = ((a[0] + a[1]) + (a[2] + a[3])) + ((a[4] + a[5]) + (a[6] + a[7]));
  } else if (colpart != nullptr && i - nw < (size_t)nch) {
    const int c = (int)(i - nw);
    float a = 0.f;
    for (int b = 0; b < nblocks; ++b) a += __ldcg(colpart + (size_t)b * nch + c);
    db[c] = a;
  }
}
#define BN_RSQRT 0.99950037468777323f
__device__ __forceinline__ void bn_fold_body(size_t i, const float* __restrict__ w, const float* __restrict__ bias, const float* __restrict__ gamma,
                                             const float* __restrict__ beta, size_t nw, int cout, float* __restrict__ w_eff,
                                             float* __restrict__ b_eff) {
  if (i < nw) w_eff[i] = w[i] * gamma[i % cout] * BN_RSQRT;
  if (i < (size_t)cout) b_eff[i] = bias[i] * gamma[i] * BN_RSQRT + beta[i];
}
static constexpr int kBnChainCo = 8;
__device__ __forceinline__ void bn_chain_body(int blk, const float* __restrict__ w, const float* __restrict__ bias, const float* __restrict__ gamma,
                                              float* __restrict__ dwe, const float* __restrict__ dbe, size_t nw, int cout,
                                              float* __restrict__ dbias, float* __restrict__ dgamma, float* __restrict__ dbeta, float* red) {
  const int rows = (int)(nw / cout);
  const int cl = threadIdx.x & 7, rl = threadIdx.x >> 3;
  const int co = blk * kBnChainCo + cl;
  const bool ok = co < cout;
  float acc = 0.f;
  if (ok)
    for (int r = rl; r < rows; r += 32) acc += dwe[(size_t)r * cout + co] * w[(size_t)r * cout + co];
  red[rl * 8 + cl] = acc;
  __syncthreads();
  float g = 0.f;
  if (ok) {
    g = gamma[co] * BN_RSQRT;
    if (rl == 0) {
      float v = 0.f;
      for (int q = 0; q < 32; ++q) v += red[q * 8 + cl];
      dgamma[co] = BN_RSQRT * (v + dbe[co] * bias[co]);
      dbias[co] = dbe[co] * g;
      dbeta[co] = dbe[co];
    }
    for (int r = rl; r < rows; r += 32) dwe[(size_t)r * cout + co] *= g;
  }
}
__global__ void pack_weights_kernel(const float* __restrict__ w, const int* __restrict__ kmap, int K_pad, int rows, int cout, int sn,
                                    const int* __restrict__ nmap, bf16* __restrict__ wp) {
  pdl_launch_dependents();
  pdl_wait();
  pack_weights_body((size_t)blockIdx.x * blockDim.x + threadIdx.x, w, kmap, K_pad, rows, cout, sn, nmap, wp);
}
__global__ void pack_weights_tiled_kernel(const float* __restrict__ w, const int* __restrict__ kmap, int cin8, int ntaps, int n_tiles, int BN,
                                          int cout, int sn, const int* __restrict__ nmap, bf16* __restrict__ out) {
  pdl_launch_dependents();
  pdl_wait();
  __shared__ float tile[64 * 129];
  if (sn == 1) pack_weights_tiled_tile(blockIdx.x, w, kmap, cin8, ntaps, n_tiles, BN, cout, nmap, out, tile);
  else pack_weights_tiled_body((size_t)blockIdx.x * blockDim.x + threadIdx.x, w, kmap, cin8, ntaps, n_tiles, BN, cout, sn, nmap, out);
}
__global__ void unpack_wgrad_kernel(const float* __restrict__ dwp, const int* __restrict__ kmap, int K_pad, int cout, int nsplit,
                                    float* __restrict__ dw, const float* __restrict__ colpart, int nblocks, int nch, float* __restrict__ db,
                                    int layout) {
  pdl_launch_dependents();
  pdl_wait();
  unpack_wgrad_body((size_t)blockIdx.x * blockDim.x + threadIdx.x, dwp, kmap, K_pad, cout, nsplit, dw, colpart, nblocks, nch, db, layout);
}
__global__ void bn_fold_kernel(const float* __restrict__ w, const float* __restrict__ bias, const float* __restrict__ gamma,
                               const float* __restrict__ beta, size_t nw, int cout, float* __restrict__ w_eff, float* __restrict__ b_eff) {
  pdl_launch_dependents();
  pdl_wait();
  bn_fold_body((size_t)blockIdx.x * blockDim.x + threadIdx.x, w, bias, gamma, beta, nw, cout, w_eff, b_eff);
}
__global__ void bn_chain_kernel(const float* __restrict__ w, const float* __restrict__ bias, const float* __restrict__ gamma,
                                float* __restrict__ dwe, const float* __restrict__ dbe, size_t nw, int cout, float* __restrict__ dbias,
                                float* __restrict__ dgamma, float* __restrict__ dbeta) {
  pdl_launch_dependents();
  pdl_wait();
  __shared__ float red[256];
  bn_chain_body(blockIdx.x, w, bias, gamma, dwe, dbe, nw, cout, dbias, dgamma, dbeta, red);
}
__global__ void param_multi_kernel(const CisParamJob* __restrict__ jobs, int njobs) {
  pdl_launch_dependents();
  pdl_wait();
  int lo = 0, hi = njobs - 1;
  while (lo < hi) {
    const int mid = (lo + hi + 1) >> 1;
    if (jobs[mid].i[7] <= (int)blockIdx.x) lo = mid; else hi = mid - 1;
  }
  const CisParamJob j = jobs[lo];
  const int blk = (int)blockIdx.x - j.i[7];
  const size_t i = (size_t)blk * blockDim.x + threadIdx.x;
  __shared__ float red[256];
  __shared__ float tile[64 * 129];
  switch (j.kind) {
    case CIS_JOB_PACK:
      pack_weights_body(i, (const float*)j.p[0], (const int*)j.p[1], j.i[0], j.i[1], j.i[2], j.i[3], (const int*)j.p[2], (bf16*)j.p[3]);
      break;
    case CIS_JOB_PACK_TILED:
      if (j.i[5] == 1)
        pack_weights_tiled_tile(blk, (const float*)j.p[0], (const int*)j.p[1], j.i[0], j.i[1], j.i[2], j.i[3], j.i[4], (const int*)j.p[2],
                                (bf16*)j.p[3], tile);
      else
        pack_weights_tiled_body(i, (const float*)j.p[0], (const int*)j.p[1], j.i[0], j.i[1], j.i[2], j.i[3], j.i[4], j.i[5], (const int*)j.p[2],
                                (bf16*)j.p[3]);
      break;
    case CIS_JOB_UNPACK:
      unpack_wgrad_body(i, (const float*)j.p[0], (const int*)j.p[1], j.i[0], j.i[1], j.i[2], (float*)j.p[2], (const float*)j.p[3], j.i[3], j.i[4],
                        (float*)j.p[4], j.i[5]);
      break;
    case CIS_JOB_BN_FOLD:
      bn_fold_body(i, (const float*)j.p[0], (const float*)j.p[1], (const float*)j.p[2], (const float*)j.p[3], (size_t)j.n, j.i[0], (float*)j.p[4],
                   (float*)j.p[5]);
      break;
    case CIS_JOB_BN_CHAIN:
      bn_chain_body(blk, (const float*)j.p[0], (const float*)j.p[1], (const float*)j.p[2], (float*)j.p[3], (const float*)j.p[4], (size_t)j.n,
                    j.i[0], (float*)j.p[5], (float*)j.p[6], (float*)j.p[7], red);
      break;
  }
}

__global__ void dact_mul_kernel(bf16* g, int gp, int gc, const bf16* __restrict__ y, int yp, int yc, const bf16* __restrict__ res, int rp,
                                int rc, size_t npix, int chunks, int act, float alpha) {
  pdl_launch_dependents();
  pdl_wait();
  const size_t i = (size_t)blockIdx.x * blockDim.x + threadIdx.x;
  if (i >= npix * chunks) return;
  const size_t pix = i / chunks;
  const int c = (int)(i % chunks) * 8;
  uint4* gpp = reinterpret_cast<uint4*>(g + pix * gp + gc + c);
  float gv[8], yv[8], rv[8];
  unpack8(*gpp, gv);
  unpack8(*reinterpret_cast<const uint4*>(y + pix * yp + yc + c), yv);
  if (res) {
    unpack8(*reinterpret_cast<const uint4*>(res + pix * rp + rc + c), rv);
#pragma unroll
    for (int e = 0; e < 8; ++e) yv[e] -= rv[e];
  }
#pragma unroll
  for (int e = 0; e < 8; ++e) {
    const float u = yv[e];
    const float d = (act == CIS_ACT_ELU) ? (u > 0.f ? 1.f : u + 1.f) : (u > 0.f ? 1.f : alpha);
    gv[e] *= d;
  }
  *gpp = pack8(gv);
}
__global__ void add_slice_kernel(bf16* dst, int dp, int dc, const bf16* __restrict__ src, int sp, int sc, size_t npix, int chunks, int reps,
                                 int accumulate) {
  pdl_launch_dependents();
  pdl_wait();
  const size_t i = (size_t)blockIdx.x * blockDim.x + threadIdx.x;
  if (i >= npix * chunks) return;
  const size_t pix = i / chunks;
  const int c = (int)(i % chunks) * 8;
  float a[8] = {0, 0, 0, 0, 0, 0, 0, 0}, t[8];
  uint4* d = reinterpret_cast<uint4*>(dst + pix * dp + dc + c);
  if (accumulate) unpack8(*d, a);
  for (int j = 0; j < reps; ++j) {
    unpack8(*reinterpret_cast<const uint4*>(src + (pix + (size_t)j * npix) * sp + sc + c), t);
#pragma unroll
    for (int e = 0; e < 8; ++e) a[e] += t[e];
  }
  *d = pack8(a);
}
__global__ void colsum_kernel(const bf16* __restrict__ g, int gp, int gc, size_t npix, int nch, int chunks, float* __restrict__ part) {
  pdl_launch_dependents();
  pdl_wait();
  extern __shared__ float sm[];
  const int P = blockDim.x / chunks;
  const int ck = threadIdx.x % chunks, pl = threadIdx.x / chunks;
  float a[8] = {0, 0, 0, 0, 0, 0, 0, 0}, t[8];
  if (pl < P) {
    for (size_t p = (size_t)blockIdx.x * P + pl; p < npix; p += (size_t)gridDim.x * P) {
      unpack8(*reinterpret_cast<const uint4*>(g + p * gp + gc + ck * 8), t);
#pragma unroll
      for (int e = 0; e < 8; ++e) a[e] += t[e];
    }
#pragma unroll
    for (int e = 0; e < 8; ++e) sm[pl * chunks * 8 + ck * 8 + e] = a[e];
  }
  __syncthreads();
  for (int c = threadIdx.x; c < nch; c += blockDim.x) {
    float s = 0.f;
    for (int q = 0; q < P; ++q) s += sm[q * chunks * 8 + c];
    part[(size_t)blockIdx.x * nch + c] = s;
  }
}

// ... 775 lines not shown
  const size_t i = (size_t)blockIdx.x * blockDim.x + threadIdx.x;
  if (i >= n) return;
  const long long t = step[0] + 1;
  float g = grad[i] * gscale;
  if (can_change && avg_abs[0] < 1e-5f) {
    const uint32_t r = hash32(seed ^ ((uint64_t)t << 40) ^ (uint64_t)i);
    g = fabsf((((float)r + 0.5f) * (1.f / 4294967296.f)) * 2.f * clip - clip);
  } else {
    g = fminf(fmaxf(g, -clip), clip);
  }
  const float lr_t = lr * sqrtf(1.f - powf(b2, (float)t)) / (1.f - powf(b1, (float)t));
  const float mi = b1 * m[i] + (1.f - b1) * g;
  const float vi = b2 * v[i] + (1.f - b2) * g * g;
  m[i] = mi;
  v[i] = vi;
  param[i] -= lr_t * mi / (sqrtf(vi) + eps);
}
__global__ void step_inc_kernel(long long* step) {
  pdl_launch_dependents();
  pdl_wait(); step[0] += 1; }
__global__ void abs_sum_kernel(const float* __restrict__ g, size_t n, float* __restrict__ out) {
  pdl_launch_dependents();
  pdl_wait();
  float acc = 0.f;
  for (size_t i = (size_t)blockIdx.x * blockDim.x + threadIdx.x; i < n; i += (size_t)gridDim.x * blockDim.x) acc += fabsf(g[i]);
  acc = warp_sum(acc);
  if ((threadIdx.x & 31) == 0) atomicAdd(out, acc);
}
__global__ void cast_f32_bf16_kernel(const float* __restrict__ s, size_t n, bf16* __restrict__ d) {
  pdl_launch_dependents();
  pdl_wait();
  const size_t i = (size_t)blockIdx.x * blockDim.x + threadIdx.x;
  if (i < n) d[i] = __float2bfloat16(s[i]);
}
__global__ void cast_bf16_f32_kernel(const bf16* __restrict__ s, size_t npix, int pitch, int coff, int C, float* __restrict__ d) {
  pdl_launch_dependents();
  pdl_wait();
  const size_t i = (size_t)blockIdx.x * blockDim.x + threadIdx.x;
  if (i >= npix * C) return;
  const size_t p = i / C;
  const int c = (int)(i % C);
  d[i] = __bfloat162float(s[p * pitch + coff + c]);
}

}

using namespace cis;
#include <stdlib.h>
#include <string.h>

static bool misc_pdl_enabled() {
  static const bool on = !(getenv("CIS_PDL") && atoi(getenv("CIS_PDL")) == 0);
  return on;
}
template <typename... KArgs, typename... Args>
static void cis_launch(void (*kern)(KArgs...), dim3 grid, dim3 block, size_t smem, cudaStream_t st, Args... args) {
  cudaLaunchConfig_t cfg;
  memset(&cfg, 0, sizeof(cfg));
  cfg.gridDim = grid;
  cfg.blockDim = block;
  cfg.dynamicSmemBytes = smem;
  cfg.stream = st;
  cudaLaunchAttribute attr[1];
  attr[0].id = cudaLaunchAttributeProgrammaticStreamSerialization;
  attr[0].val.programmaticStreamSerializationAllowed = 1;
  cfg.attrs = attr;
  cfg.numAttrs = misc_pdl_enabled() ? 1 : 0;
  cudaLaunchKernelEx(&cfg, kern, KArgs(args)...);
}
#define CIS_LAUNCH(kern, grid, block, smem, st, ...) cis_launch(kern, dim3(grid), dim3(block), (size_t)(smem), st, __VA_ARGS__)
#define ST ((cudaStream_t)stream)
static inline unsigned nblk(size_t n, int t = 256) { return (unsigned)((n + t - 1) / t); }
typedef const __nv_bfloat16* cbf;
typedef __nv_bfloat16* mbf;

extern "C" {

int cis_pack_weights(const float* w, const int32_t* kmap, int32_t K_pad, int32_t rows, int32_t cout, int32_t sn, const int32_t* nmap, void* wp,
                     cis_stream_t stream) {
  CIS_LAUNCH(pack_weights_kernel, nblk((size_t)rows * K_pad), 256, 0, ST, w, kmap, K_pad, rows, cout, sn, nmap, (mbf)wp);
  return cis_check_launch("pack_weights");
}
int cis_pack_weights_tiled(const float* w, const int32_t* kmap, int32_t cin8, int32_t ntaps, int32_t n_tiles, int32_t BN, int32_t cout, int32_t sn,
                           const int32_t* nmap, void* out, cis_stream_t stream) {
  const size_t total = (size_t)n_tiles * ((cin8 + 63) / 64) * ntaps * BN * 64;
  const unsigned blocks = sn == 1 ? (unsigned)(n_tiles * ((cin8 + 63) / 64) * ntaps) : nblk(total);
  if (BN > 128) return cis_set_error(CIS_ERR_UNSUPPORTED, "cis_pack_weights_tiled: BN > 128");
  CIS_LAUNCH(pack_weights_tiled_kernel, blocks, 256, 0, ST, w, kmap, cin8, ntaps, n_tiles, BN, cout, sn, nmap, (mbf)out);
  return cis_check_launch("pack_weights_tiled");
}
int cis_unpack_wgrad(const float* dwp, const int32_t* kmap, int32_t K_pad, int32_t cout, int32_t nsplit, float* dw, const float* colpart,
                     int32_t nblocks, int32_t nch, float* db, int32_t layout, cis_stream_t stream) {
  if (nsplit < 1 || (colpart && (nblocks < 1 || !db)) || (layout != 0 && layout != 1) || K_pad % 4)
    return cis_set_error(CIS_ERR_BAD_ARG, "cis_unpack_wgrad: bad split / column-sum / layout arguments");
  CIS_LAUNCH(unpack_wgrad_kernel, nblk((size_t)cout * K_pad + (colpart ? nch : 0)), 256, 0, ST, dwp, kmap, K_pad, cout, nsplit, dw, colpart, nblocks,
             nch, db, layout);
  return cis_check_launch("unpack_wgrad");
}
int cis_param_multi(const CisParamJob* jobs_dev, int32_t njobs, int32_t total_blocks, cis_stream_t stream) {
  if (!jobs_dev || njobs < 1 || total_blocks < 1) return cis_set_error(CIS_ERR_BAD_ARG, "cis_param_multi: bad job table");
  CIS_LAUNCH(param_multi_kernel, (unsigned)total_blocks, 256, 0, ST, jobs_dev, njobs);
  return cis_check_launch("param_multi");
}
int cis_bn_fold(const float* w, const float* bias, const float* gamma, const float* beta, int64_t nw, int32_t cout, float* w_eff, float* b_eff,
                cis_stream_t stream) {
  CIS_LAUNCH(bn_fold_kernel, nblk((size_t)nw), 256, 0, ST, w, bias, gamma, beta, (size_t)nw, cout, w_eff, b_eff);
  return cis_check_launch("bn_fold");
}
int cis_bn_chain(const float* w, const float* bias, const float* gamma, float* dwe, const float* dbe, int64_t nw, int32_t cout, float* dbias,
                 float* dgamma, float* dbeta, cis_stream_t stream) {
  CIS_LAUNCH(bn_chain_kernel, (unsigned)((cout + kBnChainCo - 1) / kBnChainCo), 256, 0, ST, w, bias, gamma, dwe, dbe, (size_t)nw, cout, dbias, dgamma, dbeta);
  return cis_check_launch("bn_chain");
}
int cis_dact_mul(void* g, int32_t gp, int32_t gc, const void* y, int32_t yp, int32_t yc, const void* res, int32_t rp, int32_t rc, int64_t npix,
                 int32_t chunks, int32_t act, float alpha, cis_stream_t stream) {
  if (act == CIS_ACT_NONE) return CIS_OK;
  CIS_LAUNCH(dact_mul_kernel, nblk((size_t)npix * chunks), 256, 0, ST, (mbf)g, gp, gc, (cbf)y, yp, yc, (cbf)res, rp, rc, (size_t)npix, chunks, act, alpha);
  return cis_check_launch("dact_mul");
}
int cis_add_slice(void* dst, int32_t dp, int32_t dc, const void* src, int32_t sp, int32_t sc, int64_t npix, int32_t chunks, int32_t reps,
                  int32_t accumulate, cis_stream_t stream) {
  CIS_LAUNCH(add_slice_kernel, nblk((size_t)npix * chunks), 256, 0, ST, (mbf)dst, dp, dc, (cbf)src, sp, sc, (size_t)npix, chunks, reps, accumulate);
  return cis_check_launch("add_slice");
}
int cis_colsum(const void* g, int32_t gp, int32_t gc, int64_t npix, int32_t nch, float* part, int32_t nblocks, cis_stream_t stream) {
  const int chunks = (nch + 7) / 8;
  if (chunks > 32) return cis_set_error(CIS_ERR_UNSUPPORTED, "cis_colsum: more than 256 channels");
  if (nblocks < 1 || nblocks > 592) return cis_set_error(CIS_ERR_BAD_ARG, "cis_colsum: nblocks must be in [1, 592]");
  const int P = 256 / chunks;
  CIS_LAUNCH(colsum_kernel, (unsigned)nblocks, 256, P * chunks * 8 * sizeof(float), ST, (cbf)g, gp, gc, (size_t)npix, nch, chunks, part);
  return cis_check_launch("colsum");
}
int cis_zero(void* ptr, int64_t nbytes, cis_stream_t stream) {
  if (!ptr || nbytes < 0) return cis_set_error(CIS_ERR_BAD_ARG, "cis_zero: bad buffer");
  cudaError_t e = cudaMemsetAsync(ptr, 0, (size_t)nbytes, ST);
  if (e != cudaSuccess) return cis_set_cuda_error(e, "cudaMemsetAsync");
  return CIS_OK;
}
int cis_dact_colsum(void* g, int32_t gp, int32_t gc, const void* y, int32_t yp, int32_t yc, const void* res, int32_t rp, int32_t rc, int64_t npix,
                    int32_t nch, int32_t act, float alpha, float* part, int32_t nblocks, cis_stream_t stream) {
  const int chunks = (nch + 7) / 8;
  if (act == CIS_ACT_NONE) return cis_colsum(g, gp, gc, npix, nch, part, nblocks, stream);
  if (chunks > 32) return cis_set_error(CIS_ERR_UNSUPPORTED, "cis_dact_colsum: more than 256 channels");
  if (nblocks < 1 || nblocks > 592) return cis_set_error(CIS_ERR_BAD_ARG, "cis_dact_colsum: nblocks must be in [1, 592]");
  const int P = 256 / chunks;
  CIS_LAUNCH(dact_colsum_kernel, (unsigned)nblocks, 256, P * chunks * 8 * sizeof(float), ST, (mbf)g, gp, gc, (cbf)y, yp, yc, (cbf)res, rp, rc,
             (size_t)npix, nch, chunks, act, alpha, part);
  return cis_check_launch("dact_colsum");
}
int cis_resize_bilinear_bf16(const void* src, int32_t sp, int32_t sc, int32_t N, int32_t H, int32_t W, void* dst, int32_t dp, int32_t dc, int32_t OH,
                             int32_t OW, int32_t chunks, cis_stream_t stream) {
  CIS_LAUNCH(resize_bilinear_bf16_kernel, nblk((size_t)N * OH * OW * chunks), 256, 0, ST, (cbf)src, sp, sc, N, H, W, (mbf)dst, dp, dc, OH, OW, chunks);
  return cis_check_launch("resize_bilinear_bf16");
}
int cis_resize_bilinear_bf16_bwd(const void* dd, int32_t dp, int32_t dc, int32_t N, int32_t OH, int32_t OW, void* ds, int32_t sp, int32_t sc, int32_t H,
                                 int32_t W, int32_t chunks, int32_t accumulate, cis_stream_t stream) {
  CIS_LAUNCH(resize_bilinear_bf16_bwd_kernel, nblk((size_t)N * H * W * chunks), 256, 0, ST, (cbf)dd, dp, dc, N, OH, OW, (mbf)ds, sp, sc, H, W, chunks,
                                                                                     accumulate);
  return cis_check_launch("resize_bilinear_bf16_bwd");
}
int cis_resize_concat_bf16(const CisSrc* srcs, int32_t nsrc, int32_t N, int32_t H, int32_t W, void* dst, int32_t dp, int32_t dc, int32_t OH, int32_t OW,
                           cis_stream_t stream) {
  if (!srcs || nsrc < 1 || nsrc > CIS_MAX_SRC) return cis_set_error(CIS_ERR_BAD_ARG, "cis_resize_concat_bf16: 1..4 sources");
  RcArgs a;
  a.nsrc = nsrc;
  int total = 0;
  for (int i = 0; i < nsrc; ++i) {
    a.s[i] = srcs[i];
    if ((srcs[i].pitch | srcs[i].c_off) & 7) return cis_set_error(CIS_ERR_BAD_ARG, "cis_resize_concat_bf16: slices must be 8-channel aligned");
    total += srcs[i].chunks;
  }
// ... 160 lines not shown
```

### unsupervised_detection_b200/csrc/ptx.cuh

```cuda
#pragma once
#include <cuda_runtime.h>
#include <cuda_bf16.h>
#include <stdint.h>

namespace cis {

__device__ __forceinline__ uint32_t smem_u32(const void* p) {
  return static_cast<uint32_t>(__cvta_generic_to_shared(p));
}

__device__ __forceinline__ void mbar_init(uint32_t bar, uint32_t count) {
  asm volatile("mbarrier.init.shared::cta.b64 [%0], %1;" ::"r"(bar), "r"(count) : "memory");
}
__device__ __forceinline__ void fence_mbar_init() {
  asm volatile("fence.mbarrier_init.release.cluster;" ::: "memory");
}
__device__ __forceinline__ void mbar_arrive(uint32_t bar) {
  asm volatile("{\n\t.reg .b64 st;\n\tmbarrier.arrive.shared::cta.b64 st, [%0];\n\t}" ::"r"(bar) : "memory");
}
__device__ __forceinline__ void mbar_expect_tx(uint32_t bar, uint32_t bytes) {
  asm volatile("{\n\t.reg .b64 st;\n\tmbarrier.arrive.expect_tx.shared::cta.b64 st, [%0], %1;\n\t}" ::"r"(bar), "r"(bytes)
               : "memory");
}
__device__ __forceinline__ bool mbar_try_wait(uint32_t bar, uint32_t parity) {
// ... 64 lines not shown
  asm volatile("prefetch.tensormap [%0];" ::"l"(tmap) : "memory");
}

__device__ __forceinline__ bool elect_one() {
  uint32_t pred;
  asm volatile(
      "{\n\t.reg .pred p;\n\t"
      "elect.sync _|p, 0xffffffff;\n\t"
      "selp.u32 %0, 1, 0, p;\n\t}"
      : "=r"(pred)
      :
      : "memory");
  return pred != 0;
}

__device__ __forceinline__ void pdl_launch_dependents() { asm volatile("griddepcontrol.launch_dependents;" ::: "memory"); }
__device__ __forceinline__ void pdl_wait() { asm volatile("griddepcontrol.wait;" ::: "memory"); }

__device__ __forceinline__ void tc_fence_before() { asm volatile("tcgen05.fence::before_thread_sync;" ::: "memory"); }
__device__ __forceinline__ void tc_fence_after() { asm volatile("tcgen05.fence::after_thread_sync;" ::: "memory"); }

template <int NCOLS>
__device__ __forceinline__ void tmem_alloc(uint32_t smem_dst) {
  asm volatile("tcgen05.alloc.cta_group::1.sync.aligned.shared::cta.b32 [%0], %1;" ::"r"(smem_dst), "n"(NCOLS) : "memory");
  asm volatile("tcgen05.relinquish_alloc_permit.cta_group::1.sync.aligned;" ::: "memory");
}
__device__ __forceinline__ void tmem_alloc_dyn(uint32_t smem_dst, uint32_t ncols) {
  asm volatile("tcgen05.alloc.cta_group::1.sync.aligned.shared::cta.b32 [%0], %1;" ::"r"(smem_dst), "r"(ncols) : "memory");
  asm volatile("tcgen05.relinquish_alloc_permit.cta_group::1.sync.aligned;" ::: "memory");
}
__device__ __forceinline__ void tmem_dealloc_dyn(uint32_t taddr, uint32_t ncols) {
  asm volatile("tcgen05.dealloc.cta_group::1.sync.aligned.b32 %0, %1;" ::"r"(taddr), "r"(ncols) : "memory");
}
template <int NCOLS>
__device__ __forceinline__ void tmem_dealloc(uint32_t taddr) {
  asm volatile("tcgen05.dealloc.cta_group::1.sync.aligned.b32 %0, %1;" ::"r"(taddr), "n"(NCOLS) : "memory");
}

__device__ __forceinline__ void umma_bf16(uint32_t tmem_d, uint64_t desc_a, uint64_t desc_b, uint32_t idesc, uint32_t accum) {
  asm volatile(
      "{\n\t.reg .pred p;\n\t"
      "setp.ne.b32 p, %4, 0;\n\t"
      "tcgen05.mma.cta_group::1.kind::f16 [%0], %1, %2, %3, p;\n\t}" ::"r"(tmem_d),
      "l"(desc_a), "l"(desc_b), "r"(idesc), "r"(accum)
      : "memory");
}
__device__ __forceinline__ void umma_commit(uint32_t bar) {
  asm volatile("tcgen05.commit.cta_group::1.mbarrier::arrive::one.shared::cluster.b64 [%0];" ::"r"(bar) : "memory");
}

__device__ __forceinline__ void tmem_ld16(uint32_t taddr, float* v) {
  uint32_t r[16];
  asm volatile(
      "tcgen05.ld.sync.aligned.32x32b.x16.b32 {%0,%1,%2,%3,%4,%5,%6,%7,%8,%9,%10,%11,%12,%13,%14,%15}, [%16];"
      : "=r"(r[0]), "=r"(r[1]), "=r"(r[2]), "=r"(r[3]), "=r"(r[4]), "=r"(r[5]), "=r"(r[6]), "=r"(r[7]), "=r"(r[8]),
        "=r"(r[9]), "=r"(r[10]), "=r"(r[11]), "=r"(r[12]), "=r"(r[13]), "=r"(r[14]), "=r"(r[15])
      : "r"(taddr)
      : "memory");
  asm volatile("tcgen05.wait::ld.sync.aligned;" ::: "memory");
#pragma unroll
  for (int i = 0; i < 16; ++i) v[i] = __uint_as_float(r[i]);
}

__device__ __forceinline__ void tmem_ld16_nowait(uint32_t taddr, uint32_t* r) {
  asm volatile(
      "tcgen05.ld.sync.aligned.32x32b.x16.b32 {%0,%1,%2,%3,%4,%5,%6,%7,%8,%9,%10,%11,%12,%13,%14,%15}, [%16];"
      : "=r"(r[0]), "=r"(r[1]), "=r"(r[2]), "=r"(r[3]), "=r"(r[4]), "=r"(r[5]), "=r"(r[6]), "=r"(r[7]), "=r"(r[8]),
        "=r"(r[9]), "=r"(r[10]), "=r"(r[11]), "=r"(r[12]), "=r"(r[13]), "=r"(r[14]), "=r"(r[15])
      : "r"(taddr)
      : "memory");
}
__device__ __forceinline__ void tmem_ld_wait() { asm volatile("tcgen05.wait::ld.sync.aligned;" ::: "memory"); }

__device__ __forceinline__ uint64_t make_smem_desc(uint32_t saddr, uint32_t lbo_bytes, uint32_t sbo_bytes) {
  uint64_t d = 0;
  d |= (uint64_t)((saddr & 0x3FFFF) >> 4);
  d |= (uint64_t)((lbo_bytes >> 4) & 0x3FFF) << 16;
  d |= (uint64_t)((sbo_bytes >> 4) & 0x3FFF) << 32;
  d |= (uint64_t)1 << 46;
  d |= (uint64_t)2 << 61;
  return d;
}
__device__ __forceinline__ uint32_t desc_hi(uint32_t sbo_bytes) { return ((sbo_bytes >> 4) & 0x3FFF) | (1u << 14) | (2u << 29); }
__device__ __forceinline__ uint32_t desc_lo(uint32_t saddr, uint32_t lbo_bytes) {
  return ((saddr & 0x3FFFF) >> 4) | (((lbo_bytes >> 4) & 0x3FFF) << 16);
}
__device__ __forceinline__ void umma_bf16_lh(uint32_t tmem_d, uint32_t alo, uint32_t ahi, uint32_t blo, uint32_t bhi, uint32_t idesc,
                                             uint32_t accum) {
  asm volatile(
      "{\n\t.reg .pred p;\n\t.reg .b64 da, db;\n\t"
      "setp.ne.b32 p, %6, 0;\n\t"
      "mov.b64 da, {%1, %2};\n\t"
      "mov.b64 db, {%3, %4};\n\t"
      "tcgen05.mma.cta_group::1.kind::f16 [%0], da, db, %5, p;\n\t}" ::"r"(tmem_d),
      "r"(alo), "r"(ahi), "r"(blo), "r"(bhi), "r"(idesc), "r"(accum)
      : "memory");
}
__host__ __device__ constexpr uint32_t make_idesc_bf16(int M, int N, int a_mn, int b_mn) {
  return (1u << 4) | (1u << 7) | (1u << 10) | ((uint32_t)a_mn << 15) | ((uint32_t)b_mn << 16) | ((uint32_t)(N >> 3) << 17) |
         ((uint32_t)(M >> 4) << 24);
}

__device__ __forceinline__ float bf16lo(uint32_t u) { return __uint_as_float(u << 16); }
__device__ __forceinline__ float bf16hi(uint32_t u) { return __uint_as_float(u & 0xFFFF0000u); }
__device__ __forceinline__ uint32_t pack_bf16(float a, float b) {
  __nv_bfloat162 t = __floats2bfloat162_rn(a, b);
  return *reinterpret_cast<uint32_t*>(&t);
}

}
```

### unsupervised_detection_b200/engine.py

```python
import ctypes as C
import os

import numpy as np
import torch

from . import _lib
from ._lib import CisConv, CisWgrad, CisSrc, ACT_NONE, ACT_ELU, ACT_LEAKY


def ru(x, m):
    return (x + m - 1) // m * m


def same_pad(n_in, k, s=1, d=1):
    out = -(-n_in // s)
    total = max((out - 1) * s + (k - 1) * d + 1 - n_in, 0)
    return total // 2, total - total // 2


SIDE_STREAM = True
_SIDE = {}
MULTI_PARAM_OPS = os.environ.get('CIS_MULTI_PARAM', '1') == '1'
DACT_COLSUM = os.environ.get('CIS_DACT_COLSUM', '1') == '1'
PLAN_MODEL = int(os.environ.get('CIS_PLAN_MODEL', '4'))
# ... 6 lines not shown
        _SIDE[k] = torch.cuda.Stream(device=device)
    return _SIDE[k]


class Plan(object):

    def __init__(self, name=''):
        self.name = name
        self.ops = []
        self.keep = []

    def add(self, fname, *args, flops=0.0, lane=0):
        fn = getattr(_lib.load(), fname)
        self.ops.append((fn, args, fname, flops, lane))

    def add_py(self, fn, label='py'):
        self.ops.append((None, fn, label, 0.0, 0))

    def zero(self, t):
        self.keep.append(t)
        self.add('cis_zero', t.data_ptr(), t.numel() * t.element_size())

    def join(self):
        self.ops.append((None, None, 'join', 0.0, 0))

    def run(self, stream=None, lane_key=0):
        if stream is not None or not SIDE_STREAM or not any(op[4] for op in self.ops):
            st = stream if stream is not None else torch.cuda.current_stream().cuda_stream
            for fn, args, name, _, _ in self.ops:
                if fn is None:
                    if args is not None:
                        args()
                else:
                    rc = fn(*args, st)
                    if rc != 0:
                        _lib.check(rc, name)
            return
        main = torch.cuda.current_stream()
        side = _side_stream(main.device, lane_key)
        st0, st1 = main.cuda_stream, side.cuda_stream
        main_ahead, side_used = True, False
        for fn, args, name, _, lane in self.ops:
            if fn is None:
                if name == 'join':
                    if side_used:
                        ev = torch.cuda.Event()
                        ev.record(side)
                        main.wait_event(ev)
                        side_used = False
                elif args is not None:
                    args()
                    main_ahead = True
                continue
            if lane == 1:
                if main_ahead:
                    ev = torch.cuda.Event()
                    ev.record(main)
                    side.wait_event(ev)
                    main_ahead = False
                rc = fn(*args, st1)
                side_used = True
            else:
                rc = fn(*args, st0)
                main_ahead = True
            if rc != 0:
                _lib.check(rc, name)
        if side_used:
            ev = torch.cuda.Event()
            ev.record(side)
            main.wait_event(ev)

    def batch_param_ops(self, device):
        from ._lib import CisParamJob, JOB_PACK, JOB_PACK_TILED, JOB_UNPACK, JOB_BN_FOLD, JOB_BN_CHAIN
        if not MULTI_PARAM_OPS or not self.ops:
            return self
        jobs = {k: [] for k in range(5)}
        for fn, a, name, _, _ in self.ops:
            j = CisParamJob()
            if name == 'cis_pack_weights':
                w, kmap, K_pad, rows, cout, sn, nmap, wp = a
                j.kind, blocks = JOB_PACK, -(-(rows * K_pad) // 256)
                ptrs, ints = [w, kmap, nmap, wp], [K_pad, rows, cout, sn]
            elif name == 'cis_pack_weights_tiled':
                w, kmap, cin8, ntaps, n_tiles, BN, cout, sn, nmap, out = a
                j.kind, blocks = JOB_PACK_TILED, -(-(n_tiles * (-(-cin8 // 64)) * ntaps * BN * 64) // 256)
                if sn == 1:
                    blocks = n_tiles * (-(-cin8 // 64)) * ntaps
                ptrs, ints = [w, kmap, nmap, out], [cin8, ntaps, n_tiles, BN, cout, sn]
            elif name == 'cis_unpack_wgrad':
                dwp, kmap, K_pad, cout, nsplit, dw, colpart, nblocks, nch, db, layout = a
                j.kind, blocks = JOB_UNPACK, -(-(cout * K_pad + nch) // 256)
                ptrs, ints = [dwp, kmap, dw, colpart, db], [K_pad, cout, nsplit, nblocks, nch, layout]
            elif name == 'cis_bn_fold':
                w, bias, gamma, beta, nw, cout, w_eff, b_eff = a
                j.kind, blocks, j.n = JOB_BN_FOLD, -(-max(nw, cout) // 256), nw
                ptrs, ints = [w, bias, gamma, beta, w_eff, b_eff], [cout]
            elif name == 'cis_bn_chain':
                w, bias, gamma, dwe, dbe, nw, cout, dbias, dgamma, dbeta = a
                j.kind, blocks, j.n = JOB_BN_CHAIN, -(-cout // 8), nw
                ptrs, ints = [w, bias, gamma, dwe, dbe, dbias, dgamma, dbeta], [cout]
            else:
                return self
            for q, v in enumerate(ptrs):
                j.p[q] = v
            for q, v in enumerate(ints):
                j.i[q] = v
            jobs[j.kind].append((j, blocks))
        out = Plan(self.name + '.multi')
        out.keep = self.keep
        for kind in (JOB_BN_FOLD, JOB_PACK_TILED, JOB_PACK, JOB_UNPACK, JOB_BN_CHAIN):
            if not jobs[kind]:
                continue
            arr = (CisParamJob * len(jobs[kind]))()
            first = 0
            for q, (j, blocks) in enumerate(jobs[kind]):
                j.i[7] = first
                arr[q] = j
                first += blocks
            tab = torch.frombuffer(bytearray(bytes(arr)), dtype=torch.uint8).to(device)
            out.keep.append(tab)
            out.add('cis_param_multi', tab.data_ptr(), len(jobs[kind]), first)
        return out

    def count(self):
        n = 0
        for fn, args, name, _, _ in self.ops:
            if fn is None or name == 'cis_zero':
                continue
            n += 1
            if name == 'cis_conv_igemm':
                d = args[0]._obj
                if d.splits > 1 and not d.sk_cluster:
                    n += 1
        return n

    def extend(self, other):
        self.ops += other.ops
        self.keep += other.keep


class Act(object):

    def __init__(self, N, H, W, C, device, buf=None, c_off=0, chanmap=None, n_mod=0, dep=frozenset(), name=''):
        if chanmap is not None and not C:
            C = max(chanmap) + 1
        self.N, self.H, self.W, self.C = N, H, W, C
        self.C8 = ru(C, 8) if chanmap is None else len(chanmap)
        if buf is None:
            buf = torch.zeros(N, H, W, self.C8, dtype=torch.bfloat16, device=device)
        self.buf = buf
        self.pitch = buf.shape[-1]
        self.c_off = c_off
        self.chanmap = list(chanmap) if chanmap is not None else list(range(C)) + [-1] * (self.C8 - C)
        self.n_mod = n_mod
        self.dep = frozenset(dep)
        self.name = name
        self.grad = None
        self.grad_written = {}
        self.device = device
        self.gen_rows = None

    @property
    def ptr(self):
        return self.buf.data_ptr()

    def src(self):
        return CisSrc(self.ptr, self.pitch, self.c_off, self.C8 // 8, self.n_mod)

    def rows(self, mode):
        return self.gen_rows if (mode == 'G' and self.gen_rows) else self.N

# ... 9 lines not shown
            return self._owner.get_grad()
        if self.grad is None:
            self.grad = Act(self.N, self.H, self.W, self.C, self.device, chanmap=self.chanmap, name=self.name + '.grad')
        return self.grad

    def float(self):
        idx = [i for i, m in enumerate(self.chanmap) if m >= 0]
        return self.buf[..., self.c_off:self.c_off + self.C8].float()[..., idx]


def _fill_taps(d, taps):
    d.ntaps = len(taps)
    for i, (a, b) in enumerate(taps):
        d.dh[i] = a
        d.dw[i] = b


def _fill_srcs(d, srcs):
    d.nsrc = len(srcs)
    for i, s in enumerate(srcs):
        d.src[i] = s.src()


def pick_bn(cout, cap=None):
    if cout <= 16:
        return 16, 1
    if cout <= 32:
        return 32, 1
    if cap in (32, 64) and cout > cap:
        return cap, -(-cout // cap)
    if cout <= 64:
        return 64, 1
    return 128, -(-cout // 128)


def small_bn_cap(level):
    spec = os.environ.get('CIS_SMALL_BN', '')
    if not spec:
        return None
    cap, _, lvl = spec.partition(':')
    return int(cap) if level >= int(lvl or 5) else None



NUM_SMS = 148
HALO_ENABLED = True
WGRAD_TMA = True
MATERIALIZE_MISALIGNED_CONCAT = True


WGRAD_CTAS_PER_SM = int(os.environ.get('CIS_WGRAD_CTAS_PER_SM', '2'))
WGRAD_MAX_SLICE_MB = float(os.environ.get('CIS_WGRAD_MAX_SLICE_MB', '16'))
WGRAD_HALO_MIN_CH = int(os.environ.get('CIS_WGRAD_HALO_MIN_CH', '16'))
WGRAD_HALO = os.environ.get('CIS_WGRAD_HALO', '1') == '1'


def wgrad_halo_fits(taps, cout, stride):
    if stride != 1 or not taps:
        return False
    hoy, hox = min(a for a, _ in taps), min(b for _, b in taps)
    keys = [(a - hoy) * 1024 + (b - hox) for a, b in taps]
    if any(k1 <= k0 for k0, k1 in zip(keys, keys[1:])):
        return False
    wh, hh = 8 + max(b for _, b in taps) - hox, 8 + max(a for a, _ in taps) - hoy
    nh = 64 if cout > 64 else ru(cout, 16)
    if ((len(taps) + 1) // 2) * nh > 512 or wh > 256 or hh > 256:
        return False
    stage = ru(wh * hh * 128, 1024) + 8192
    return (200 * 1024) // stage >= 2


def _pow2_cols(c):
    for v in (32, 64, 128, 256, 512):
        if c <= v:
            return v
    return 1024


SPLITK = int(os.environ.get('CIS_SPLITK', '2'))
SPLITK_CLUSTER = os.environ.get('CIS_SPLITK_CLUSTER', '0') == '1'
SPLITK_MAX = int(os.environ.get('CIS_SPLITK_MAX', '16'))
SPLITK_NCTA = int(os.environ.get('CIS_SPLITK_NCTA', '64'))
SPLITK_MIN_UNITS = int(os.environ.get('CIS_SPLITK_MIN_UNITS', '18'))
HALO_SKIP_THIN = int(os.environ.get('CIS_HALO_SKIP_THIN', '0'))
HALO_MIN_UTIL = float(os.environ.get('CIS_HALO_MIN_UTIL', '0.2'))


def setup_splitk(d, device, keep):
    if not SPLITK:
        return
    m_chunks = sum(d.src[i].chunks for i in range(d.nsrc))
    if d.halo:
        Hp0, Wp0 = -(-d.OH // d.dil), -(-d.OW // d.dil)
        tiles = (-(-Wp0 // 8)) * (-(-Hp0 // (16 * d.MT))) * d.dil * d.dil * d.N
        ncta, units, min_units, mt = tiles * d.n_tiles, -(-m_chunks // 8), 1, d.MT
    else:
        ncta, units, min_units, mt = (-(-(d.N * d.OH * d.OW) // 128)) * d.n_tiles, d.K_pad // 64, 4, 1
    steps = units * (d.ntaps if d.halo else 1)
    if ncta > SPLITK_NCTA or steps < SPLITK_MIN_UNITS:
        return
    splits = min(units // min_units, -(-2 * NUM_SMS // ncta), SPLITK_MAX, 8 if SPLITK_CLUSTER else 1 << 30)
    if splits < 2:
        return
    per = -(-units // splits)
    splits = -(-units // per)
    if splits < 2:
        return
    if SPLITK_CLUSTER and splits <= 8 and mt * 128 * d.BN * 4 + 1024 <= 226 * 1024:
        d.splits, d.sk_scratch, d.sk_counters, d.sk_cluster = splits, None, None, 1
        return
    sc = torch.empty(ncta * mt * splits * 128 * d.BN, dtype=torch.float32, device=device)
    keep.append(sc)
    d.splits, d.sk_scratch, d.sk_counters = splits, sc.data_ptr(), None


def setup_halo(d, taps, dil, n_tiles):
    if not HALO_ENABLED or d.sh != 1 or d.sw != 1:
        return False
    if any(a % dil or b % dil for a, b in taps):
        return False
    if dil > 1 and (d.OH != d.H or d.OW != d.W):
        return False
    th = [(a // dil, b // dil) for a, b in taps]
    hoy, hox = min(a for a, _ in th), min(b for _, b in th)
    rel = [(a - hoy, b - hox) for a, b in th]
    ey, ex = max(a for a, _ in rel), max(b for _, b in rel)
    Hp0, Wp0 = -(-d.OH // dil), -(-d.OW // dil)
    tiles_x = -(-Wp0 // 8)
    best = None
    ntaps = len(taps)
    m_chunks = sum(d.src[i].chunks for i in range(d.nsrc))
    if HALO_SKIP_THIN and m_chunks * 8 <= HALO_SKIP_THIN and ntaps >= 16:
        return False
    nchunks = -(-m_chunks // 8)
    nhs = 2 if nchunks > 1 else 1
    force = int(os.environ.get('CIS_FORCE_MT128', '0')) if d.BN == 128 else 0
    for MT in (1, 2, 3, 4):
        if MT * d.BN > 512 or (force and MT != force):
            continue
        HP = (8 + ex) * (16 * MT + ey)
        fixed = nhs * ru(HP * 128, 1024) + HP * 4 + 1024
        smem = fixed + min(3, ntaps * nchunks) * d.BN * 128 + 1024
        if smem > 227 * 1024:
            continue
        tiles_y = -(-Hp0 // (16 * MT))
        util = (Hp0 * Wp0) / float(tiles_y * 16 * MT * tiles_x * 8)
        if util < (HALO_MIN_UTIL if dil == 1 else 0.5):
            continue
        ncta = d.N * dil * dil * tiles_x * tiles_y * n_tiles
        cps = max(1, min((225 * 1024) // smem, 512 // _pow2_cols(MT * d.BN), 6))
        t_mma = MT * 2.0 * d.BN * ntaps * nchunks
        t_mem = (d.BN * 128 * ntaps / 40.0 + HP * 128 / 16.0) * nchunks
        t_cta = max(t_mma, t_mem) + (4000.0 + 1500.0 * MT) / cps
        cost = -(-ncta // (NUM_SMS * cps)) * cps * t_cta / min(cps, max(1.0, ncta / float(NUM_SMS)))
        if PLAN_MODEL == 2:
            per_sm = -(-ncta // NUM_SMS)
            cost = per_sm * max(t_mma, t_mem) + (4000.0 + 1500.0 * MT) * (-(-per_sm // cps))
        if PLAN_MODEL == 3:
            cost = float(MT)
        if PLAN_MODEL == 4:
            n1 = d.N * dil * dil * tiles_x * (-(-Hp0 // 16)) * n_tiles
            if not (2.0 * d.BN * ntaps * nchunks < 6000.0 and n1 > 4 * NUM_SMS):
                cost = float(MT)
        if best is None or cost < best[0] - 1e-9:
            best = (cost, MT, util)
    if best is None:
        return False
    d.halo, d.dil, d.MT, d.hoy, d.hox, d.ey, d.ex = 1, dil, best[1], hoy, hox, ey, ex
    _fill_taps(d, rel)
    return True


S2_HALO = os.environ.get('CIS_S2_HALO', '0') == '1'


def setup_halo_s2(d, taps, n_tiles):
    if not (HALO_ENABLED and S2_HALO) or d.sh != 2 or d.sw != 2:
        return None
    if any(d.src[i].chunks % 8 for i in range(d.nsrc - 1)):
        return None
    ph = [((u % 2) * 2 + (v % 2), u // 2, v // 2) for u, v in taps]
    order = sorted(range(len(taps)), key=lambda i: (ph[i][0], i))
    hoy, hox = min(a for _, a, _ in ph), min(b for _, _, b in ph)
    rel = [(ph[i][1] - hoy, ph[i][2] - hox) for i in order]
    ey, ex = max(a for a, _ in rel), max(b for _, b in rel)
    m_chunks = sum(d.src[i].chunks for i in range(d.nsrc))
    nchunks = -(-m_chunks // 8)
    tiles_x = -(-d.OW // 8)
    best = None
    for MT in (1, 2, 3, 4):
        if MT * d.BN > 512:
            continue
        HP = (8 + ex) * (16 * MT + ey)
        smem = 2 * ru(HP * 128, 1024) + HP * 4 + 2048 + 2 * d.BN * 128
        if smem > 227 * 1024:
            continue
        tiles_y = -(-d.OH // (16 * MT))
        util = (d.OH * d.OW) / float(tiles_y * 16 * MT * tiles_x * 8)
        if util < HALO_MIN_UTIL:
            continue
        ncta = d.N * tiles_x * tiles_y * n_tiles
        cps = max(1, min((225 * 1024) // smem, 512 // _pow2_cols(MT * d.BN), 4))
        t_mma = MT * 2.0 * d.BN * len(taps) * nchunks
        t_mem = (d.BN * 128 * len(taps) / 40.0 + 4 * HP * 128 / 40.0) * nchunks
        t_cta = max(t_mma, t_mem) + (4000.0 + 1500.0 * MT) / cps
        cost = -(-ncta // (NUM_SMS * cps)) * cps * t_cta / min(cps, max(1.0, ncta / float(NUM_SMS)))
        if best is None or cost < best[0] - 1e-9:
            best = (cost, MT)
    if best is None:
        return None
    d.halo, d.dil, d.MT, d.hoy, d.hox, d.ey, d.ex = 1, 1, best[1], hoy, hox, ey, ex
    d.sh = d.sw = 1
    _fill_taps(d, rel)
    d.nph = 4
    bounds = [0]
    for q in range(4):
        bounds.append(bounds[-1] + sum(1 for i in order if ph[i][0] == q))
    for q in range(5):
        d.ph_tap[q] = bounds[q]
    return order


GROUP_PARITY = os.environ.get('CIS_GROUP_PARITY', '1') == '1'
GROUP_PARITY_MAX_TILES = int(os.environ.get('CIS_GROUP_PARITY_MAX_TILES', '1000000'))


def merge_parity_launches(descs):
    if not GROUP_PARITY or not (2 <= len(descs) <= 4):
        return None
    d0 = descs[0]
    same = ('N', 'H', 'W', 'BN', 'n_tiles', 'nsrc', 'act', 'DH', 'DW', 'osh', 'osw', 'out', 'out_pitch', 'out_coff', 'out_ch', 'outf', 'outf_pitch',
            'outf_coff', 'outf_ch', 'add_pre', 'add_pre_pitch', 'add_pre_coff', 'add_post', 'addf_pre', 'mode', 'bias')
    for d in descs:
        if not d.halo or d.dil != 1 or d.splits > 1 or d.nph > 1 or any(getattr(d, f) != getattr(d0, f) for f in same):
            return None
        if any(bytes(d.src[i]) != bytes(d0.src[i]) for i in range(d0.nsrc)):
            return None
    if sum(d.ntaps for d in descs) > _lib.MAX_TAPS:
        return None
    if max(d.N * (-(-d.OH // 16)) * (-(-d.OW // 8)) for d in descs) > GROUP_PARITY_MAX_TILES:
        return None
    g = CisConv.from_buffer_copy(bytes(d0))
    g.MT, g.ey, g.ex = min(d.MT for d in descs), max(d.ey for d in descs), max(d.ex for d in descs)
    g.OH, g.OW = max(d.OH for d in descs), max(d.OW for d in descs)
    t = 0
    for i, d in enumerate(descs):
        for k in range(d.ntaps):
            g.dh[t + k], g.dw[t + k] = d.dh[k], d.dw[k]
        sb = g.sub[i]
        sb.tap0, sb.ntaps, sb.hoy, sb.hox, sb.OH, sb.OW, sb.oa, sb.ob, sb.wpack = t, d.ntaps, d.hoy, d.hox, d.OH, d.OW, d.oa, d.ob, d.wpack
        t += d.ntaps
    m_chunks = sum(g.src[i].chunks for i in range(g.nsrc))
    g.ntaps, g.nsub, g.splits, g.K_pad = t, len(descs), 0, ru(t * m_chunks * 8, 64)
    return g


class ParamStore(object):

    def __init__(self, device):
        self.device = device
        self.entries = []
        self.index = {}
        self.size = 0
        self.flat = None

    def declare(self, name, shape, padded=None):
        n = int(np.prod(shape))
        pn = ru(padded or n, 4)
        self.index[name] = len(self.entries)
        self.entries.append((name, tuple(shape), n, self.size, pn))
        self.size += pn

    def finalize(self, trainable):
        self.flat = torch.zeros(self.size, dtype=torch.float32, device=self.device)
        if trainable:
            self.grad = torch.zeros_like(self.flat)
            self.m = torch.zeros_like(self.flat)
            self.v = torch.zeros_like(self.flat)
            seg = [0]
            for _, _, n, off, _ in self.entries:
                seg.append(off + n)
            self.seg_pairs = [(off, off + n) for _, _, n, off, _ in self.entries]

    def off(self, name):
        return self.entries[self.index[name]][3]

    def ptr(self, name, which='flat'):
        return getattr(self, which).data_ptr() + 4 * self.off(name)

    def view(self, name, which='flat'):
        _, shape, n, off, _ = self.entries[self.index[name]]
        return getattr(self, which)[off:off + n].view(shape)

    def load(self, params):
        for name, shape, n, off, _ in self.entries:
            if name not in params:
                raise KeyError('missing parameter ' + name)
            t = params[name].detach().to(torch.float32).reshape(-1)
            if t.numel() != n:
                raise ValueError('shape mismatch for %s: %d vs %d' % (name, t.numel(), n))
            self.flat[off:off + n].copy_(t)

    def export(self, which='flat'):
        return {name: getattr(self, which)[off:off + n].view(shape).clone() for name, shape, n, off, _ in self.entries}

    def real_count(self):
        return sum(e[2] for e in self.entries)


class ConvLayer(object):

    def __init__(self, store, name, k, cin, cout, stride=1, dil=1, act=ACT_NONE, alpha=0.2, tag='', bn=False,
                 wname='kernel', bname='bias', transposed=False, bn_cap=None):
        self.store, self.name, self.k, self.cin, self.cout = store, name, k, cin, cout
        self.stride, self.dil, self.act, self.alpha, self.tag, self.bn = stride, dil, act, alpha, tag, bn
        self.transposed = transposed
        self.bn_cap = bn_cap
        self.BN, self.n_tiles = pick_bn(cout, bn_cap)
        self.npad = self.BN * self.n_tiles
        self.wkey, self.bkey = '%s/%s' % (name, wname), '%s/%s' % (name, bname)
        if transposed:
            store.declare(self.wkey, (k, k, cout, cin))
        else:
            store.declare(self.wkey, (k, k, cin, cout))
        store.declare(self.bkey, (cout,), padded=self.npad)
        if bn:
            store.declare('%s/gamma' % name, (cout,))
            store.declare('%s/beta' % name, (cout,))
        self.fwd_pack = None
        self.dgrad_packs = None
        self.device = store.device

    def _kmap(self, taps_idx, chanmap, per_tap_stride, chan_stride):
        m = len(chanmap)
        K = len(taps_idx) * m
        Kp = ru(max(K, (len(taps_idx) - 1) * m + ru(m, 64)), 64)
        km = np.full(Kp, -1, dtype=np.int32)
        cm = np.asarray(chanmap, dtype=np.int64)
        for ti, t in enumerate(taps_idx):
            v = np.where(cm >= 0, t * per_tap_stride + cm * chan_stride, -1)
            km[ti * m:(ti + 1) * m] = v
        return torch.from_numpy(km).to(self.device), Kp

    def setup_fwd(self, chanmap):
        assert max(chanmap) == self.cin - 1, (self.name, max(chanmap), self.cin)
        self.in_chanmap = list(chanmap)
        kk = self.k * self.k
        if self.transposed:
            raise RuntimeError('use setup_transposed')
        kmap, Kp = self._kmap(range(kk), chanmap, self.cin * self.cout, self.cout)
        self.fwd_kmap, self.K_pad = kmap, Kp
        self.fwd_pack = torch.zeros(self.npad, Kp, dtype=torch.bfloat16, device=self.device)
        if self.bn:
            self.w_eff = torch.zeros(kk * self.cin * self.cout, dtype=torch.float32, device=self.device)
            self.b_eff = torch.zeros(self.npad, dtype=torch.float32, device=self.device)
            self.db_eff = torch.zeros(self.npad, dtype=torch.float32, device=self.device)

    def _alloc_tiles(self, ntaps, cin8, BN, n_tiles):
        nchunks = -(-cin8 // 64)
        return torch.zeros(n_tiles * nchunks * ntaps * BN * 64, dtype=torch.bfloat16, device=self.device)

    def fwd_tiles_buf(self, tap_order=None):
        if getattr(self, 'fwd_tiles', None) is None:
            self.fwd_tiles = self._alloc_tiles(self.k * self.k, len(self.in_chanmap), self.BN, self.n_tiles)
            self.fwd_tiles_kmap = self.fwd_kmap
            if tap_order is not None:
                self.fwd_tiles_kmap, _ = self._kmap(list(tap_order), self.in_chanmap, self.cin * self.cout, self.cout)
            self.fwd_tap_order = tap_order
        assert getattr(self, 'fwd_tap_order', None) == tap_order, self.name
        return self.fwd_tiles

    def w_src_ptr(self):
        return self.w_eff.data_ptr() if self.bn else self.store.ptr(self.wkey)

    def bias_ptr(self):
        return self.b_eff.data_ptr() if self.bn else self.store.ptr(self.bkey)

    def plan_pack(self, plan, dgrad=False):
        s = self.store
        if self.bn:
            plan.add('cis_bn_fold', s.ptr(self.wkey), s.ptr(self.bkey), s.ptr(self.name + '/gamma'), s.ptr(self.name + '/beta'),
                     self.k * self.k * self.cin * self.cout, self.cout, self.w_eff.data_ptr(), self.b_eff.data_ptr())
        if self.fwd_pack is not None:
            if self.transposed:
                for pk in self.tr_packs:
                    if pk.get('wt') is not None:
                        plan.add('cis_pack_weights_tiled', self.w_src_ptr(), pk['kmap'].data_ptr(), len(self.in_chanmap), len(pk['taps']),
                                 self.n_tiles, self.BN, self.cout, self.cin, None, pk['wt'].data_ptr())
                    if pk.get('rows_used', True):
                        plan.add('cis_pack_weights', self.w_src_ptr(), pk['kmap'].data_ptr(), pk['K_pad'], self.npad, self.cout, self.cin,
                                 None, pk['w'].data_ptr())
            else:
                if getattr(self, 'fwd_tiles', None) is not None:
                    plan.add('cis_pack_weights_tiled', self.w_src_ptr(), self.fwd_tiles_kmap.data_ptr(), len(self.in_chanmap), self.k * self.k,
                             self.n_tiles, self.BN, self.cout, 1, None, self.fwd_tiles.data_ptr())
                if getattr(self, 'fwd_rows_used', True):
                    plan.add('cis_pack_weights', self.w_src_ptr(), self.fwd_kmap.data_ptr(), self.K_pad, self.npad, self.cout, 1,
                             None, self.fwd_pack.data_ptr())
        if dgrad and self.dgrad_packs:
            cout8 = ru(self.cout, 8)
            for pk in self.dgrad_packs:
                if pk.get('wt') is not None:
                    plan.add('cis_pack_weights_tiled', self.w_src_ptr(), pk['kmap'].data_ptr(), cout8, len(pk['taps']), pk['n_tiles'], pk['BN'],
                             len(self.in_chanmap), self.cout, pk['nmap'].data_ptr(), pk['wt'].data_ptr())
                if pk.get('rows_used', True):
                    plan.add('cis_pack_weights', self.w_src_ptr(), pk['kmap'].data_ptr(), pk['K_pad'], pk['rows'], len(self.in_chanmap),
                             self.cout, pk['nmap'].data_ptr(), pk['w'].data_ptr())

    def plan_finalize(self, bp, mode):
        if not hasattr(self, 'dwp') or mode not in getattr(self, 'wg_splits', {}):
            return
        s = self.store
        bp.add('cis_unpack_wgrad', self.dwp.data_ptr(), self.wg_kmap.data_ptr(), self.wg_K_pad, self.cout, self.wg_splits[mode],
               s.ptr(self.wkey, 'grad'), self.colpart.data_ptr(), self.col_blocks[mode], self.cout,
               (self.db_eff.data_ptr() if self.bn else s.ptr(self.bkey, 'grad')), 0 if self.wg_halo else 1)
        if self.bn:
            bp.add('cis_bn_chain', s.ptr(self.wkey), s.ptr(self.bkey), s.ptr(self.name + '/gamma'), s.ptr(self.wkey, 'grad'),
                   self.db_eff.data_ptr(), self.k * self.k * self.cin * self.cout, self.cout, s.ptr(self.bkey, 'grad'),
                   s.ptr(self.name + '/gamma', 'grad'), s.ptr(self.name + '/beta', 'grad'))

    def fwd_taps(self, H, W):
        pt, _ = same_pad(H, self.k, self.stride, self.dil)
        pl, _ = same_pad(W, self.k, self.stride, self.dil)
        return [(r * self.dil - pt, c * self.dil - pl) for r in range(self.k) for c in range(self.k)], pt, pl

    def setup_dgrad(self, H, W):
        if self.dgrad_packs is not None:
            return
        _, pt, pl = self.fwd_taps(H, W)
        k, s, d = self.k, self.stride, self.dil
        g_chan = list(range(self.cout)) + [-1] * (ru(self.cout, 8) - self.cout)
        cin8 = len(self.in_chanmap)
        bn_, nt = pick_bn(cin8, self.bn_cap)
        rows = bn_ * nt
        nmap = torch.tensor(list(self.in_chanmap) + [-1] * (rows - cin8), dtype=torch.int32, device=self.device)
        packs = []
        for a in range(s):
            for b in range(s):
                tl, offs = [], []
                for r in range(k):
                    if (a + pt - r * d) % s:
                        continue
                    for c in range(k):
                        if (b + pl - c * d) % s:
                            continue
                        tl.append(r * k + c)
                        offs.append(((a + pt - r * d) // s, (b + pl - c * d) // s))
                kmap, Kp = self._kmap(tl, g_chan, self.cin * self.cout, 1)
                packs.append(dict(a=a, b=b, taps=offs, kmap=kmap, K_pad=Kp, rows=rows, BN=bn_, n_tiles=nt, nmap=nmap,
                                  w=torch.zeros(rows, Kp, dtype=torch.bfloat16, device=self.device)))
        self.dgrad_packs = packs

    def setup_transposed(self, chanmap):
        assert self.transposed and self.k == 4
        self.in_chanmap = list(chanmap)
        packs = []
        for a in range(2):
            for b in range(2):
                tl, offs = [], []
                for ky in range(4):
                    if (a + 1 - ky) % 2:
                        continue
                    for kx in range(4):
                        if (b + 1 - kx) % 2:
                            continue
                        tl.append(ky * 4 + kx)
                        offs.append(((a + 1 - ky) // 2, (b + 1 - kx) // 2))
                kmap, Kp = self._kmap(tl, chanmap, self.cout * self.cin, 1)
                packs.append(dict(a=a, b=b, taps=offs, kmap=kmap, K_pad=Kp,
                                  w=torch.zeros(self.npad, Kp, dtype=torch.bfloat16, device=self.device)))
        self.tr_packs = packs
        self.fwd_pack = True


class Builder(object):

    def __init__(self, device):
        self.device = device
        self.fwd = Plan('fwd')
        self.lane = 0
        self.tape = []
        self.keep = []

    def new_act(self, N, H, W, C, name='', dep=frozenset(), n_mod=0):
        a = Act(N, H, W, C, self.device, name=name, dep=dep, n_mod=n_mod)
        self.keep.append(a)
        return a

    def hold(self, obj):
        self.keep.append(obj)
        return obj

    def f32(self, *shape):
        return self.hold(torch.zeros(*shape, dtype=torch.float32, device=self.device))

    def conv(self, layer, srcs, out=None, post_add=None, addf=None, outf=None, outf_ch=0, mode=0, want_bf16=True, name=None,
             plan=None, out_rows=None):
        plan = plan or self.fwd
        if MATERIALIZE_MISALIGNED_CONCAT and len(srcs) > 1 and layer.tag and layer.stride == 1 and \
                any(s.C8 % 64 for s in srcs[:-1]):
            srcs = [self.concat(srcs, name=layer.name + '.cat')]
        s0 = srcs[0]
        N = out_rows or max(s.N for s in srcs)
        H, W = s0.H, s0.W
        for s in srcs:
            assert (s.H, s.W) == (H, W), (layer.name, [(q.H, q.W) for q in srcs])
        chanmap = []
        base = 0
        for s in srcs:
            chanmap += [(m + base if m >= 0 else -1) for m in s.chanmap]
            base += s.C
        if layer.fwd_pack is None:
            layer.setup_fwd(chanmap)
        else:
            assert layer.in_chanmap == chanmap, layer.name
        OH, OW = -(-H // layer.stride), -(-W // layer.stride)
        dep = frozenset().union(*[s.dep for s in srcs]) | ({layer.tag} if layer.tag else frozenset())
        if post_add is not None:
            dep = dep | post_add.dep
        if out is None and want_bf16:
            out = self.new_act(N, OH, OW, layer.cout, name=name or layer.name, dep=dep)
        if out is not None:
            out.dep = out.dep | dep
            gr = [s.gen_rows for s in srcs if s.gen_rows]
            if gr:
                out.gen_rows = gr[0]
        taps, _, _ = layer.fwd_taps(H, W)
        d = CisConv()
        d.N, d.H, d.W, d.OH, d.OW, d.sh, d.sw = N, H, W, OH, OW, layer.stride, layer.stride
        _fill_taps(d, taps)
        _fill_srcs(d, srcs)
        d.wpack, d.K_pad, d.BN, d.n_tiles = layer.fwd_pack.data_ptr(), layer.K_pad, layer.BN, layer.n_tiles
        d.bias, d.act, d.alpha = layer.bias_ptr(), layer.act, layer.alpha
        d.DH, d.DW, d.osh, d.osw, d.oa, d.ob = OH, OW, 1, 1, 0, 0
        if out is not None:
            d.out, d.out_pitch, d.out_coff, d.out_ch = out.ptr, out.pitch, out.c_off, out.C8
        if outf is not None:
            d.outf, d.outf_pitch, d.outf_coff, d.outf_ch = outf.data_ptr(), outf.shape[-1], 0, outf_ch or outf.shape[-1]
        if addf is not None:
            d.addf_pre, d.addf_pitch, d.addf_coff = addf.data_ptr(), addf.shape[-1], 0
            if outf is None:
                d.outf_ch = addf.shape[-1]
        if post_add is not None:
            d.add_post, d.add_post_pitch, d.add_post_coff = post_add.ptr, post_add.pitch, post_add.c_off
        d.mode = mode
        order = setup_halo_s2(d, taps, layer.n_tiles) if (layer.stride == 2 and layer.dil == 1) else None
        if order is not None:
            d.wpack = layer.fwd_tiles_buf(order).data_ptr()
            layer.fwd_rows_used = getattr(layer, 'fwd_rows_used', False)
        elif layer.stride == 1 and setup_halo(d, taps, layer.dil, layer.n_tiles):
            d.wpack = layer.fwd_tiles_buf().data_ptr()
            layer.fwd_rows_used = getattr(layer, 'fwd_rows_used', False)
        else:
            layer.fwd_rows_used = True
        setup_splitk(d, self.device, plan.keep)
        plan.keep.append(d)
        plan.keep += [srcs, out, outf, addf, post_add, layer]
        plan.add('cis_conv_igemm', C.byref(d), flops=2.0 * N * OH * OW * layer.k * layer.k * layer.cin * layer.cout, lane=self.lane)
        if layer.tag:
            self.tape.append(lambda bp, m, L=layer, S=list(srcs), O=out, P=post_add: self._conv_bwd(bp, m, L, S, O, P))
        return out

    def _conv_bwd(self, bp, mode, layer, srcs, out, post_add):
        if out is None or mode not in out.dep or not out.grad_written.get(mode):
            return
        G = out.get_grad()
        nb = out.rows(mode)
        npix = nb * out.H * out.W
        if post_add is not None and mode in post_add.dep:
            pg = post_add.get_grad()
            bp.add('cis_add_slice', pg.ptr, pg.pitch, pg.c_off, G.ptr, G.pitch, G.c_off, npix, G.C8 // 8, 1,
                   1 if post_add.grad_written.get(mode) else 0)
            post_add.grad_written[mode] = True
        if layer.tag == mode:
            chunks = -(-layer.cout // 8)
            ppb = (256 // chunks) * COLSUM_PIX
            if not hasattr(layer, 'col_blocks'):
                layer.col_blocks = {}
            layer.col_blocks[mode] = max(1, min(592, -(-npix // ppb)))
            if getattr(layer, 'colpart', None) is None:
                layer.colpart = torch.empty(592 * layer.cout, dtype=torch.float32, device=self.device)
        res = (post_add.ptr, post_add.pitch, post_add.c_off) if post_add is not None else (None, 0, 0)
        fused_colsum = bool(DACT_COLSUM and layer.act != ACT_NONE and layer.tag == mode)
        if fused_colsum:
            bp.add('cis_dact_colsum', G.ptr, G.pitch, G.c_off, out.ptr, out.pitch, out.c_off, res[0], res[1], res[2], npix, layer.cout,
                   layer.act, layer.alpha, layer.colpart.data_ptr(), layer.col_blocks[mode])
        elif layer.act != ACT_NONE:
            bp.add('cis_dact_mul', G.ptr, G.pitch, G.c_off, out.ptr, out.pitch, out.c_off, res[0], res[1], res[2], npix, G.C8 // 8,
                   layer.act, layer.alpha)
        s0 = srcs[0]
        H, W = s0.H, s0.W
        taps, _, _ = layer.fwd_taps(H, W)
        if layer.tag == mode:
            if not hasattr(layer, 'dwp'):
                layer.wg_tma = bool(WGRAD_TMA and layer.stride == 1 and len(layer.in_chanmap) >= 32 and
                                    all(s_.C8 % 64 == 0 for s_ in srcs[:-1]))
                layer.wg_halo = bool(WGRAD_HALO and len(layer.in_chanmap) >= WGRAD_HALO_MIN_CH and wgrad_halo_fits(taps, layer.cout, layer.stride) and
                                     all(s_.C8 % 64 == 0 for s_ in srcs[:-1]))
                if layer.wg_tma or layer.wg_halo:
                    cin8 = len(layer.in_chanmap)
                    nch64 = -(-cin8 // 64)
                    ncol = layer.k * layer.k * nch64 * 64
                    layer.wg_K_pad = ru(ncol, 128)
                    km = np.full(layer.wg_K_pad, -1, dtype=np.int32)
                    fk = layer.fwd_kmap.cpu().numpy()
                    for t in range(layer.k * layer.k):
                        for pos in range(cin8):
                            km[(t * nch64 + pos // 64) * 64 + pos % 64] = fk[t * cin8 + pos]
                    layer.wg_kmap = torch.from_numpy(km).to(self.device)
                else:
                    layer.wg_K_pad, layer.wg_kmap = layer.K_pad, layer.fwd_kmap
                layer.dwp, layer.wg_splits = None, {}
            w = CisWgrad()
            w.N, w.H, w.W, w.OH, w.OW, w.sh, w.sw = nb, H, W, out.H, out.W, layer.stride, layer.stride
            _fill_taps(w, taps)
            _fill_srcs(w, srcs)
            w.g, w.g_pitch, w.g_coff, w.g_chunks = G.ptr, G.pitch, G.c_off, G.C8 // 8
            w.Cout, w.K_pad = layer.cout, layer.wg_K_pad
            w.tma = 2 if layer.wg_halo else (1 if layer.wg_tma else 0)
            nkb = (nb * (-(-out.H // 8)) * (-(-out.W // 8))) if w.tma else -(-npix // 64)
            ntile = -(-layer.wg_K_pad // 128)
            if w.tma == 2:
                ntile = (-(-len(layer.in_chanmap) // 64)) * (2 if layer.cout > 64 else 1)
            splits = max(1, min(nkb // 8 if nkb >= 8 else 1, max(1, (WGRAD_CTAS_PER_SM * NUM_SMS) // ntile)))
            if WGRAD_MAX_SLICE_MB > 0:
                splits = max(1, min(splits, int(WGRAD_MAX_SLICE_MB * 1e6 / (layer.cout * layer.wg_K_pad * 4.0))))
            splits = -(-nkb // (-(-nkb // splits)))
            w.splits = splits
            layer.wg_splits[mode] = splits
            if layer.dwp is None or layer.dwp.numel() < splits * layer.cout * layer.wg_K_pad:
                assert not getattr(layer, 'wgrad_modes', None), 'slice buffer must be sized by the first (largest) mode'
                layer.dwp = torch.empty(max(layer.wg_splits.values()) * layer.cout * layer.wg_K_pad, dtype=torch.float32, device=self.device)
            w.dwp = layer.dwp.data_ptr()
            bp.keep.append(w)
            bp.add('cis_conv_wgrad', C.byref(w), flops=2.0 * npix * layer.k * layer.k * layer.cin * layer.cout, lane=1)
            layer.wgrad_modes = getattr(layer, 'wgrad_modes', set()) | {mode}
            if not fused_colsum:
                bp.add('cis_colsum', G.ptr, G.pitch, G.c_off, npix, layer.cout, layer.colpart.data_ptr(), layer.col_blocks[mode], lane=1)
        need = [s for s in srcs if mode in s.dep]
        if not need:
            return
        layer.setup_dgrad(H, W)
        layer.dgrad_used = True
        cin8 = len(layer.in_chanmap)
        single = (len(srcs) == 1 and srcs[0].n_mod == 0)
        if single:
            tgt = srcs[0].get_grad()
            acc = bool(srcs[0].grad_written.get(mode))
        else:
            if not hasattr(layer, 'dcat'):
                layer.dcat = Act(max(s.N for s in srcs), H, W, cin8, self.device, chanmap=layer.in_chanmap, name=layer.name + '.dcat')
            tgt, acc = layer.dcat, False
        emitted = []
        for pk in layer.dgrad_packs:
            s = layer.stride
            oh = -(-(H - pk['a']) // s)
            ow = -(-(W - pk['b']) // s)
            if oh <= 0 or ow <= 0:
                continue
            d = CisConv()
            d.N, d.H, d.W, d.OH, d.OW, d.sh, d.sw = nb, out.H, out.W, oh, ow, 1, 1
            _fill_taps(d, pk['taps'])
            d.nsrc = 1
            d.src[0] = G.src()
            d.wpack, d.K_pad, d.BN, d.n_tiles = pk['w'].data_ptr(), pk['K_pad'], pk['BN'], pk['n_tiles']
            d.bias, d.act = None, ACT_NONE
            d.DH, d.DW, d.osh, d.osw, d.oa, d.ob = H, W, s, s, pk['a'], pk['b']
            d.out, d.out_pitch, d.out_coff, d.out_ch = tgt.ptr, tgt.pitch, tgt.c_off, tgt.C8
            if acc:
                d.add_pre, d.add_pre_pitch, d.add_pre_coff = tgt.ptr, tgt.pitch, tgt.c_off
            if setup_halo(d, pk['taps'], layer.dil if s == 1 else 1, pk['n_tiles']):
                if pk.get('wt') is None:
                    pk['wt'] = layer._alloc_tiles(len(pk['taps']), ru(layer.cout, 8), pk['BN'], pk['n_tiles'])
                d.wpack = pk['wt'].data_ptr()
                pk['rows_used'] = pk.get('rows_used', False)
            else:
                pk['rows_used'] = True
            emitted.append((d, 2.0 * nb * oh * ow * len(pk['taps']) * layer.cin * layer.cout))
        grp = merge_parity_launches([d for d, _ in emitted]) if len(emitted) > 1 else None
        if grp is not None:
            bp.keep.append(grp)
            bp.add('cis_conv_igemm', C.byref(grp), flops=sum(f for _, f in emitted))
        else:
            for d, fl in emitted:
                setup_splitk(d, self.device, bp.keep)
                bp.keep.append(d)
                bp.add('cis_conv_igemm', C.byref(d), flops=fl)
        if single:
            srcs[0].grad_written[mode] = True
        else:
            want = [1 if mode in s_.dep else 0 for s_ in srcs]
            garr, acc = [], []
            for s_, w_ in zip(srcs, want):
                if w_:
                    sg = s_.get_grad()
                    garr.append(CisSrc(sg.ptr, sg.pitch, sg.c_off, s_.C8 // 8, s_.n_mod))
                    acc.append(1 if s_.grad_written.get(mode) else 0)
                    s_.grad_written[mode] = True
                else:
                    garr.append(CisSrc(None, 8, 0, s_.C8 // 8, s_.n_mod))
                    acc.append(0)
            ga = (CisSrc * len(srcs))(*garr)
            wa, aa = (C.c_int32 * len(srcs))(*want), (C.c_int32 * len(srcs))(*acc)
            bp.keep += [ga, wa, aa]
            bp.add('cis_resize_concat_bf16_bwd', tgt.ptr, tgt.pitch, 0, nb, H, W, ga, wa, aa, len(srcs), H, W)

    def resize_concat(self, srcs, OH=None, OW=None, name='cat'):
        srcs = list(srcs)
        assert 1 <= len(srcs) <= 4
        N = max(s.N for s in srcs)
        H, W = srcs[0].H, srcs[0].W
        OH, OW = OH or H, OW or W
        for s in srcs:
            assert (s.H, s.W) == (H, W) and (s.n_mod == 0 or N % s.n_mod == 0)
        chanmap, base = [], 0
        for s in srcs:
            chanmap += [(m + base if m >= 0 else -1) for m in s.chanmap]
            base += s.C
        dep = frozenset().union(*[s.dep for s in srcs])
        cat = Act(N, OH, OW, base, self.device, chanmap=chanmap, dep=dep, name=name)
        gr = [s.gen_rows for s in srcs if s.gen_rows]
        if gr:
            cat.gen_rows = gr[0]
        arr = (CisSrc * len(srcs))(*[s.src() for s in srcs])
        self.keep += [srcs, cat, arr]
        self.fwd.add('cis_resize_concat_bf16', arr, len(srcs), N, H, W, cat.ptr, cat.pitch, cat.c_off, OH, OW, lane=self.lane)

        def bwd(bp, mode):
            if mode not in cat.dep or not cat.grad_written.get(mode):
                return
            g = cat.get_grad()
            nb = cat.rows(mode)
            want = [1 if mode in s_.dep else 0 for s_ in srcs]
            if not any(want):
                return
            garr, acc = [], []
            for s_, w_ in zip(srcs, want):
                if w_:
                    sg = s_.get_grad()
                    garr.append(CisSrc(sg.ptr, sg.pitch, sg.c_off, s_.C8 // 8, s_.n_mod))
                    acc.append(1 if s_.grad_written.get(mode) else 0)
                    s_.grad_written[mode] = True
                else:
                    garr.append(CisSrc(None, 8, 0, s_.C8 // 8, s_.n_mod))
                    acc.append(0)
            ga = (CisSrc * len(srcs))(*garr)
            wa, aa = (C.c_int32 * len(srcs))(*want), (C.c_int32 * len(srcs))(*acc)
            bp.keep += [ga, wa, aa]
            bp.add('cis_resize_concat_bf16_bwd', g.ptr, g.pitch, g.c_off, nb, OH, OW, ga, wa, aa, len(srcs), H, W)
        self.tape.append(bwd)
        return cat

    def concat(self, srcs, name='cat'):
        return self.resize_concat(srcs, name=name)

    def conv_transpose(self, layer, src, out=None, outf=None, plan=None, name=None):
        plan = plan or self.fwd
        if layer.fwd_pack is None:
            layer.setup_transposed(src.chanmap)
        N, H, W = src.N, src.H, src.W
        if out is None:
            out = self.new_act(N, 2 * H, 2 * W, layer.cout, name=name or layer.name, dep=src.dep)
        emitted = []
        for pk in layer.tr_packs:
            d = CisConv()
            d.N, d.H, d.W, d.OH, d.OW, d.sh, d.sw = N, H, W, H, W, 1, 1
            _fill_taps(d, pk['taps'])
            _fill_srcs(d, [src])
            d.wpack, d.K_pad, d.BN, d.n_tiles = pk['w'].data_ptr(), pk['K_pad'], layer.BN, layer.n_tiles
            d.bias, d.act = layer.bias_ptr(), ACT_NONE
            d.DH, d.DW, d.osh, d.osw, d.oa, d.ob = 2 * H, 2 * W, 2, 2, pk['a'], pk['b']
            d.out, d.out_pitch, d.out_coff, d.out_ch = out.ptr, out.pitch, out.c_off, layer.cout
            if outf is not None:
                d.outf, d.outf_pitch, d.outf_coff, d.outf_ch = outf.data_ptr(), outf.shape[-1], 0, layer.cout
            if setup_halo(d, pk['taps'], 1, layer.n_tiles):
                if pk.get('wt') is None:
                    pk['wt'] = layer._alloc_tiles(len(pk['taps']), len(layer.in_chanmap), layer.BN, layer.n_tiles)
                d.wpack = pk['wt'].data_ptr()
                pk['rows_used'] = pk.get('rows_used', False)
            else:
                pk['rows_used'] = True
            plan.keep += [src, out, outf, layer]
            emitted.append((d, 2.0 * N * H * W * len(pk['taps']) * layer.cin * layer.cout))
        grp = merge_parity_launches([d for d, _ in emitted])
        if grp is not None:
            plan.keep.append(grp)
            plan.add('cis_conv_igemm', C.byref(grp), flops=sum(f for _, f in emitted), lane=self.lane)
        else:
            for d, fl in emitted:
                setup_splitk(d, self.device, plan.keep)
                plan.keep.append(d)
                plan.add('cis_conv_igemm', C.byref(d), flops=fl)
        return out

    def resize_bilinear(self, src, OH, OW, name=''):
        if (src.H, src.W) == (OH, OW):
            return src
        out = Act(src.N, OH, OW, src.C, self.device, chanmap=src.chanmap, n_mod=src.n_mod, dep=src.dep, name=name or src.name + '.rs')
        out.gen_rows = src.gen_rows
        self.keep += [src, out]
        self.fwd.add('cis_resize_bilinear_bf16', src.ptr, src.pitch, src.c_off, src.N, src.H, src.W, out.ptr, out.pitch, out.c_off, OH, OW,
                     src.C8 // 8)

        def bwd(bp, mode):
            if mode not in out.dep or not out.grad_written.get(mode):
                return
            g, sg = out.get_grad(), src.get_grad()
            bp.add('cis_resize_bilinear_bf16_bwd', g.ptr, g.pitch, g.c_off, out.rows(mode), OH, OW, sg.ptr, sg.pitch, sg.c_off, src.H, src.W,
                   src.C8 // 8, 1 if src.grad_written.get(mode) else 0)
            src.grad_written[mode] = True
        self.tape.append(bwd)
        return out

    def upsample_nn2x(self, src, name=''):
        assert src.c_off == 0 and src.pitch == src.C8
        out = Act(src.N, 2 * src.H, 2 * src.W, src.C, self.device, chanmap=src.chanmap, dep=src.dep, name=name or src.name + '.up')
        self.keep += [src, out]
        self.fwd.add('cis_upsample_nn2x', src.ptr, src.N, src.H, src.W, src.pitch, out.ptr)

        def bwd(bp, mode):
            if mode not in out.dep or not out.grad_written.get(mode):
                return
            g, sg = out.get_grad(), src.get_grad()
            bp.add('cis_upsample_nn2x_bwd', g.ptr, src.N, src.H, src.W, src.pitch, sg.ptr, 1 if src.grad_written.get(mode) else 0)
            src.grad_written[mode] = True
        self.tape.append(bwd)
        return out

    def build_backward(self, mode, seeds):
        bp = Plan('bwd_' + mode)
        for a in seeds:
            a.grad_written[mode] = True
        for fn in reversed(self.tape):
            fn(bp, mode)
        return bp
```

Measured before the change: 985.4.

## Add compact thin-channel halo layout for low-channel convolutions

```diff
diff --git a/include/cis_b200.h b/include/cis_b200.h
--- a/include/cis_b200.h
+++ b/include/cis_b200.h
@@ -68,6 +68,7 @@
     int32_t OH, OW, oa, ob;
     const void* wpack;
   } sub[4];
+  int32_t thin;
 } CisConv;
 
 typedef struct {
@@ -98,7 +99,7 @@
 int cis_pack_weights(const float* w, const int32_t* kmap, int32_t K_pad, int32_t rows, int32_t cout, int32_t sn, const int32_t* nmap,
                      void* wp, cis_stream_t stream);
 int cis_pack_weights_tiled(const float* w, const int32_t* kmap, int32_t cin8, int32_t ntaps, int32_t n_tiles, int32_t BN, int32_t cout,
-                           int32_t sn, const int32_t* nmap, void* out, cis_stream_t stream);
+                           int32_t sn, const int32_t* nmap, void* out, int32_t layout, cis_stream_t stream);
 int cis_unpack_wgrad(const float* dwp, const int32_t* kmap, int32_t K_pad, int32_t cout, int32_t nsplit, float* dw, const float* colpart,
                      int32_t nblocks, int32_t nch, float* db, int32_t layout, cis_stream_t stream);
 int cis_bn_fold(const float* w, const float* bias, const float* gamma, const float* beta, int64_t nw, int32_t cout, float* w_eff,
diff --git a/unsupervised_detection_b200/_lib.py b/unsupervised_detection_b200/_lib.py
--- a/unsupervised_detection_b200/_lib.py
+++ b/unsupervised_detection_b200/_lib.py
@@ -42,7 +42,7 @@
                 ('ey', C.c_int32), ('ex', C.c_int32),
                 ('splits', C.c_int32), ('sk_scratch', C.c_void_p), ('sk_counters', C.c_void_p),
                 ('nph', C.c_int32), ('ph_tap', C.c_int32 * 5), ('sk_cluster', C.c_int32),
-                ('nsub', C.c_int32), ('sub', CisSub * 4)]
+                ('nsub', C.c_int32), ('sub', CisSub * 4), ('thin', C.c_int32)]
 
 
 class CisWgrad(C.Structure):
@@ -60,7 +60,7 @@
     'cis_conv_igemm': [C.POINTER(CisConv)],
     'cis_conv_wgrad': [C.POINTER(CisWgrad)],
     'cis_pack_weights': [_p, _p, _i32, _i32, _i32, _i32, _p, _p],
-    'cis_pack_weights_tiled': [_p, _p, _i32, _i32, _i32, _i32, _i32, _i32, _p, _p],
+    'cis_pack_weights_tiled': [_p, _p, _i32, _i32, _i32, _i32, _i32, _i32, _p, _p, _i32],
     'cis_unpack_wgrad': [_p, _p, _i32, _i32, _i32, _p, _p, _i32, _i32, _p, _i32],
     'cis_bn_fold': [_p, _p, _p, _p, _i64, _i32, _p, _p],
     'cis_param_multi': [_p, _i32, _i32],
diff --git a/unsupervised_detection_b200/csrc/conv_igemm.cu b/unsupervised_detection_b200/csrc/conv_igemm.cu
--- a/unsupervised_detection_b200/csrc/conv_igemm.cu
+++ b/unsupervised_detection_b200/csrc/conv_igemm.cu
@@ -527,6 +527,7 @@
 
 
 static constexpr int kHaloMaxBStages = 8;
+__host__ __device__ __forceinline__ uint32_t thin_plane_bytes(int HP) { return ((uint32_t)HP * 16u + 127u) & ~127u; }
 struct HaloMaps {
   CUtensorMap m[CIS_MAX_SRC * 4];
 };
@@ -581,8 +582,7 @@
 template <int NK>
 __device__ __forceinline__ void halo_issue_stage(const uint32_t tmem, const uint32_t hlo, uint32_t blo, const uint32_t* s_aoff, const int gt,
                                                  const int MT, const int BN, const uint32_t ahi, const uint32_t bhi, const uint32_t a_mstep,
-                                                 const uint32_t idesc, const bool first) {
-  const uint32_t bstep = (uint32_t)(BN * 128) >> 4;
+                                                 const uint32_t bstep, const uint32_t idesc, const bool first) {
   if (NK == 1 && MT == 1) {
     halo_issue_mt1<NK>(tmem, hlo, blo, s_aoff, gt, bstep, ahi, bhi, idesc, first);
     return;
@@ -611,7 +611,8 @@
 template <int BN>
 __global__ void __launch_bounds__(HaloCfg<BN>::kThreads, HaloCfg<BN>::kMinCtas) conv_halo_kernel(const __grid_constant__ CisConv p, const int halo_stage_bytes, const int BS, const int NHS,
                                                         const __grid_constant__ HaloMaps maps, const int use_tma, const int G) {
-  constexpr int kBStage = BN * 128;
+  const int thin = p.thin;
+  const int kBStage = thin ? BN * 32 : BN * 128;
   constexpr int kHMmaWarp_ = HaloCfg<BN>::kMmaWarp, kHThreads_ = HaloCfg<BN>::kThreads;
   extern __shared__ uint8_t smem_raw[];
   __shared__ uint64_t bars[2 * 2 + 2 * kHaloMaxBStages + 1];
@@ -659,7 +660,7 @@
   pdl_launch_dependents();
   const uint32_t ncols = (MT * BN <= 32) ? 32u : (MT * BN <= 64) ? 64u : (MT * BN <= 128) ? 128u : (MT * BN <= 256) ? 256u : 512u;
 
-  if (tid < ntaps) s_aoff[tid] = (uint32_t)((p.dh[tap0 + tid] * Wh + p.dw[tap0 + tid]) * 8);
+  if (tid < ntaps) s_aoff[tid] = (uint32_t)((p.dh[tap0 + tid] * Wh + p.dw[tap0 + tid]) * (thin ? 1 : 8));
   if (tid < p.nsrc) {
     s_src[tid].ptr = reinterpret_cast<const __nv_bfloat16*>(p.src[tid].ptr);
     s_src[tid].pitch = p.src[tid].pitch;
@@ -713,6 +714,17 @@
           while (si < p.nsrc - 1 && c >= s_src[si].chunks) {
             c -= s_src[si].chunks;
             ++si;
+          }
+          if (thin) {
+            const uint32_t plane = thin_plane_bytes(HP);
+            mbar_expect_tx(bar_hfull + 8 * hs, (uint32_t)(m_chunks * HP * 16));
+            for (int q = 0; q < m_chunks; ++q) {
+              const int sq = q < s_src[0].chunks ? 0 : 1, cq = q - (sq ? s_src[0].chunks : 0);
+              const int nm = s_src[sq].n_mod;
+              tma_load_4d(h_base + hs * halo_stage_bytes + q * plane, &maps.m[sq * nph + ph], bar_hfull + 8 * hs, cq * 8, tx * 8 + hox,
+                          ty * 16 * MT + hoy, nm ? (n % nm) : n);
+            }
+            continue;
           }
           const int nmod = s_src[si].n_mod;
           mbar_expect_tx(bar_hfull + 8 * hs, (uint32_t)(HP * 128));
@@ -819,8 +831,11 @@
     }
   } else {
     constexpr uint32_t idesc = make_idesc_bf16(kBM, BN, 0, 0);
-    const uint32_t ahi = desc_hi((uint32_t)(Wh * 128)), bhi = desc_hi(1024);
-    const uint32_t a_mstep = (uint32_t)(16 * Wh * 128) >> 4;
+    const uint32_t ahi = thin ? desc_hi_noswz((uint32_t)(Wh * 16)) : desc_hi((uint32_t)(Wh * 128));
+    const uint32_t bhi = thin ? desc_hi_noswz(128u) : desc_hi(1024);
+    const uint32_t a_lbo = thin ? (m_chunks == 1 ? 16u : thin_plane_bytes(HP)) : 16u, b_lbo = thin ? (uint32_t)(BN * 16) : 16u;
+    const uint32_t a_mstep = (uint32_t)(16 * Wh * (thin ? 16 : 128)) >> 4;
+    const uint32_t bstep = (uint32_t)kBStage >> 4;
     int bs = 0, hs = 0, it = 0;
     uint32_t bph = 0, hph = 0;
     int vlast = nchunks * nph - 1;
@@ -834,19 +849,19 @@
       const int nk16 = rem >= 8 ? 4 : (rem + 1) / 2;
       mbar_wait(bar_hfull + 8 * hs, hph);
       if (vc == 0 && lane == 0) CIS_TRACE_AT(1);
-      const uint32_t hlo = desc_lo(h_base + hs * halo_stage_bytes, 16);
+      const uint32_t hlo = desc_lo(h_base + hs * halo_stage_bytes, a_lbo);
       for (int t0 = tlo; t0 < thi; t0 += G, ++it) {
         const int gt = min(G, thi - t0);
         mbar_wait(bar_bfull + 8 * bs, bph);
         tc_fence_after();
         if (elect_one()) {
           CIS_TRACE_AT(8 + 2 * it);
-          const uint32_t blo = desc_lo(b_base + bs * stage_bytes, 16);
+          const uint32_t blo = desc_lo(b_base + bs * stage_bytes, b_lbo);
           const bool first = !any;
-          if (nk16 == 4) halo_issue_stage<4>(tmem, hlo, blo, s_aoff + t0, gt, MT, BN, ahi, bhi, a_mstep, idesc, first);
-          else if (nk16 == 1) halo_issue_stage<1>(tmem, hlo, blo, s_aoff + t0, gt, MT, BN, ahi, bhi, a_mstep, idesc, first);
-          else if (nk16 == 2) halo_issue_stage<2>(tmem, hlo, blo, s_aoff + t0, gt, MT, BN, ahi, bhi, a_mstep, idesc, first);
-          else halo_issue_stage<3>(tmem, hlo, blo, s_aoff + t0, gt, MT, BN, ahi, bhi, a_mstep, idesc, first);
+          if (nk16 == 4) halo_issue_stage<4>(tmem, hlo, blo, s_aoff + t0, gt, MT, BN, ahi, bhi, a_mstep, bstep, idesc, first);
+          else if (nk16 == 1) halo_issue_stage<1>(tmem, hlo, blo, s_aoff + t0, gt, MT, BN, ahi, bhi, a_mstep, bstep, idesc, first);
+          else if (nk16 == 2) halo_issue_stage<2>(tmem, hlo, blo, s_aoff + t0, gt, MT, BN, ahi, bhi, a_mstep, bstep, idesc, first);
+          else halo_issue_stage<3>(tmem, hlo, blo, s_aoff + t0, gt, MT, BN, ahi, bhi, a_mstep, bstep, idesc, first);
           umma_commit(bar_bempty + 8 * bs);
           if (t0 + G >= thi) {
             umma_commit(bar_hempty + 8 * hs);
@@ -945,7 +960,8 @@
 __global__ void __launch_bounds__(kPThreads, 2) conv_halo_persist_kernel(const __grid_constant__ CisConv p, const int halo_stage_bytes,
                                                                        const int BS, const int NHS, const int AS, const int G,
                                                                        const __grid_constant__ HaloMaps maps, const int ws) {
-  constexpr int kBStage = BN * 128;
+  const int thin = p.thin;
+  const int kBStage = thin ? BN * 32 : BN * 128;
   constexpr int kMaxHS = 4;
   extern __shared__ uint8_t smem_raw[];
   __shared__ uint64_t bars[2 * kMaxHS + 2 * kHaloMaxBStages + 4];
@@ -973,7 +989,7 @@
   const uint32_t ncols = want <= 32 ? 32u : want <= 64 ? 64u : want <= 128 ? 128u : want <= 256 ? 256u : 512u;
 
   pdl_launch_dependents();
-  if (tid < p.ntaps) s_aoff[tid] = (uint32_t)((p.dh[tid] * Wh + p.dw[tid]) * 8);
+  if (tid < p.ntaps) s_aoff[tid] = (uint32_t)((p.dh[tid] * Wh + p.dw[tid]) * (thin ? 1 : 8));
   if (warp == 3) {
     if (lane == 0) {
       for (int s = 0; s < NHS; ++s) {
@@ -1018,13 +1034,24 @@
             c -= p.src[si].chunks;
             ++si;
           }
-          int nmod = p.src[0].n_mod;
-          if (si == 1) nmod = p.src[1].n_mod;
-          if (si == 2) nmod = p.src[2].n_mod;
-          if (si == 3) nmod = p.src[3].n_mod;
-          mbar_expect_tx(bar_hfull + 8 * hs, (uint32_t)(HP * 128));
-          tma_load_4d(h_base + hs * halo_stage_bytes, &maps.m[si], bar_hfull + 8 * hs, c * 8, tx * 8 + p.hox, ty * 16 * MT + p.hoy,
-                      nmod ? (n % nmod) : n);
+          if (thin) {
+            const uint32_t plane = thin_plane_bytes(HP);
+            mbar_expect_tx(bar_hfull + 8 * hs, (uint32_t)(m_chunks * HP * 16));
+            for (int q = 0; q < m_chunks; ++q) {
+              const int sq = q < p.src[0].chunks ? 0 : 1, cq = q - (sq ? p.src[0].chunks : 0);
+              const int nm = sq ? p.src[1].n_mod : p.src[0].n_mod;
+              tma_load_4d(h_base + hs * halo_stage_bytes + q * plane, &maps.m[sq], bar_hfull + 8 * hs, cq * 8, tx * 8 + p.hox,
+                          ty * 16 * MT + p.hoy, nm ? (n % nm) : n);
+            }
+          } else {
+            int nmod = p.src[0].n_mod;
+            if (si == 1) nmod = p.src[1].n_mod;
+            if (si == 2) nmod = p.src[2].n_mod;
+            if (si == 3) nmod = p.src[3].n_mod;
+            mbar_expect_tx(bar_hfull + 8 * hs, (uint32_t)(HP * 128));
+            tma_load_4d(h_base + hs * halo_stage_bytes, &maps.m[si], bar_hfull + 8 * hs, c * 8, tx * 8 + p.hox, ty * 16 * MT + p.hoy,
+                        nmod ? (n % nmod) : n);
+          }
           if (++hs == NHS) {
             hs = 0;
             hph ^= 1u;
@@ -1065,8 +1092,11 @@
     }
   } else if (warp == 2) {
     constexpr uint32_t idesc = make_idesc_bf16(kBM, BN, 0, 0);
-    const uint32_t ahi = desc_hi((uint32_t)(Wh * 128)), bhi = desc_hi(1024);
-    const uint32_t a_mstep = (uint32_t)(16 * Wh * 128) >> 4;
+    const uint32_t ahi = thin ? desc_hi_noswz((uint32_t)(Wh * 16)) : desc_hi((uint32_t)(Wh * 128));
+    const uint32_t bhi = thin ? desc_hi_noswz(128u) : desc_hi(1024);
+    const uint32_t a_lbo = thin ? (m_chunks == 1 ? 16u : thin_plane_bytes(HP)) : 16u, b_lbo = thin ? (uint32_t)(BN * 16) : 16u;
+    const uint32_t a_mstep = (uint32_t)(16 * Wh * (thin ? 16 : 128)) >> 4;
+    const uint32_t bstep = (uint32_t)kBStage >> 4;
     int hs = 0, bs = 0, as = 0;
     uint32_t hph = 0, bph = 0, tph = 1;
     if (ws && (int)blockIdx.x < total) {
@@ -1085,19 +1115,19 @@
         const int nk16 = rem >= 8 ? 4 : (rem + 1) / 2;
         mbar_wait(bar_hfull + 8 * hs, hph);
         if (cc == 0 && lane == 0) CIS_TRACE_AT(10 + 5 * wi);
-        const uint32_t hlo = desc_lo(h_base + hs * halo_stage_bytes, 16);
+        const uint32_t hlo = desc_lo(h_base + hs * halo_stage_bytes, a_lbo);
         const int gstep = ws ? p.ntaps : G;
         for (int t0 = 0; t0 < p.ntaps; t0 += gstep) {
           const int gt = min(gstep, p.ntaps - t0);
           if (!ws) mbar_wait(bar_bfull + 8 * bs, bph);
           tc_fence_after();
           if (elect_one()) {
-            const uint32_t blo = desc_lo(ws ? b_base + (uint32_t)(cc * p.ntaps) * kBStage : b_base + bs * stage_bytes, 16);
+            const uint32_t blo = desc_lo(ws ? b_base + (uint32_t)(cc * p.ntaps) * kBStage : b_base + bs * stage_bytes, b_lbo);
             const bool first = (cc | t0) == 0;
-            if (nk16 == 4) halo_issue_stage<4>(tacc, hlo, blo, s_aoff + t0, gt, MT, BN, ahi, bhi, a_mstep, idesc, first);
-            else if (nk16 == 1) halo_issue_stage<1>(tacc, hlo, blo, s_aoff + t0, gt, MT, BN, ahi, bhi, a_mstep, idesc, first);
-            else if (nk16 == 2) halo_issue_stage<2>(tacc, hlo, blo, s_aoff + t0, gt, MT, BN, ahi, bhi, a_mstep, idesc, first);
-            else halo_issue_stage<3>(tacc, hlo, blo, s_aoff + t0, gt, MT, BN, ahi, bhi, a_mstep, idesc, first);
+            if (nk16 == 4) halo_issue_stage<4>(tacc, hlo, blo, s_aoff + t0, gt, MT, BN, ahi, bhi, a_mstep, bstep, idesc, first);
+            else if (nk16 == 1) halo_issue_stage<1>(tacc, hlo, blo, s_aoff + t0, gt, MT, BN, ahi, bhi, a_mstep, bstep, idesc, first);
+            else if (nk16 == 2) halo_issue_stage<2>(tacc, hlo, blo, s_aoff + t0, gt, MT, BN, ahi, bhi, a_mstep, bstep, idesc, first);
+            else halo_issue_stage<3>(tacc, hlo, blo, s_aoff + t0, gt, MT, BN, ahi, bhi, a_mstep, bstep, idesc, first);
             if (!ws) umma_commit(bar_bempty + 8 * bs);
             if (t0 + gstep >= p.ntaps) {
               umma_commit(bar_hempty + 8 * hs);
@@ -1600,7 +1630,7 @@
   return fn;
 }
 static bool encode_src_map(CUtensorMap* m, const CisSrc& s, int N, int H, int W, int bw, int bh, int step = 1, int py = 0, int px = 0,
-                           int estride = 1) {
+                           int estride = 1, bool thin = false) {
   EncodeTiledFn enc = get_encode_tiled();
   if (!enc) return false;
   const int nb = s.n_mod > 0 ? s.n_mod : N;
@@ -1608,10 +1638,11 @@
   if (Hq < 1 || Wq < 1) return false;
   cuuint64_t dims[4] = {(cuuint64_t)s.chunks * 8, (cuuint64_t)Wq, (cuuint64_t)Hq, (cuuint64_t)nb};
   cuuint64_t strides[3] = {(cuuint64_t)step * s.pitch * 2, (cuuint64_t)step * W * s.pitch * 2, (cuuint64_t)H * W * s.pitch * 2};
-  cuuint32_t box[4] = {64, (cuuint32_t)(bw * estride), (cuuint32_t)(bh * estride), 1};
+  cuuint32_t box[4] = {thin ? 8u : 64u, (cuuint32_t)(bw * estride), (cuuint32_t)(bh * estride), 1};
   cuuint32_t es[4] = {1, (cuuint32_t)estride, (cuuint32_t)estride, 1};
   void* base = (void*)((const char*)s.ptr + ((size_t)(py * W + px) * s.pitch + (size_t)s.c_off) * 2);
-  return enc(m, CU_TENSOR_MAP_DATA_TYPE_BFLOAT16, 4, base, dims, strides, box, es, CU_TENSOR_MAP_INTERLEAVE_NONE, CU_TENSOR_MAP_SWIZZLE_128B,
+  return enc(m, CU_TENSOR_MAP_DATA_TYPE_BFLOAT16, 4, base, dims, strides, box, es, CU_TENSOR_MAP_INTERLEAVE_NONE,
+             thin ? CU_TENSOR_MAP_SWIZZLE_NONE : CU_TENSOR_MAP_SWIZZLE_128B,
              CU_TENSOR_MAP_L2_PROMOTION_L2_128B, CU_TENSOR_MAP_FLOAT_OOB_FILL_NONE) == CUDA_SUCCESS;
 }
 
@@ -1632,14 +1663,17 @@
 template <int BN>
 static int launch_halo(const CisConv* d, cudaStream_t st) {
   const int Wh = 8 + d->ex, Hh = 16 * d->MT + d->ey, HP = Wh * Hh;
-  const int halo_stage = (HP * 128 + 1023) & ~1023;
   int chunks = 0;
   for (int i = 0; i < d->nsrc; ++i) chunks += d->src[i].chunks;
+  const bool thin = d->thin != 0;
+  if (thin && (chunks > 2 || d->dil != 1 || d->splits > 1))
+    return cis_set_error(CIS_ERR_BAD_ARG, "cis_conv_igemm(halo): the compact thin halo takes <= 16 channels, no dilation, no split-K");
+  const int halo_stage = thin ? (int)((chunks * thin_plane_bytes(HP) + 1023) & ~1023u) : (HP * 128 + 1023) & ~1023;
   const int nchunks = (chunks + 7) / 8;
   const int nsub = d->nsub > 1 ? d->nsub : 1;
   const int nsp = (nsub == 1 && d->splits > 1) ? d->splits : 1;
   const int cper = (nchunks + nsp - 1) / nsp;
-  const int nhs = cper > 1 ? 2 : 1;
+  const int nhs = cper * (d->nph > 1 ? d->nph : 1) > 1 ? 2 : 1;
   const int dd = d->dil;
   int tiles = 0, ntaps_max = d->ntaps;
   if (nsub > 1) {
@@ -1661,7 +1695,7 @@
   const long ncta_all = (long)tiles * dd * dd * d->N * d->n_tiles * nsp * nsub;
   static const int g_env = getenv("CIS_HALO_G") ? atoi(getenv("CIS_HALO_G")) : 0;
   static const int stage_kb = getenv("CIS_HALO_STAGE_KB") ? atoi(getenv("CIS_HALO_STAGE_KB")) : 48;
-  const int kB = BN * 128;
+  const int kB = thin ? BN * 32 : BN * 128;
   int G = g_env > 0 ? g_env : (stage_kb * 1024) / kB;
   if (G < 1) G = 1;
   if (G > ntaps_max) G = ntaps_max;
@@ -1699,14 +1733,15 @@
   const int nph = d->nph > 1 ? d->nph : 1;
   static const int dil_tma = getenv("CIS_DIL_TMA") ? atoi(getenv("CIS_DIL_TMA")) : 1;
   int use_tma = ((d->dil == 1 || dil_tma) && Wh * d->dil <= 256 && Hh * d->dil <= 256) ? 1 : 0;
-  for (int i = 0; use_tma && i < d->nsrc - 1; ++i)
+  for (int i = 0; use_tma && !thin && i < d->nsrc - 1; ++i)
     if (d->src[i].chunks % 8) use_tma = 0;
   for (int i = 0; use_tma && i < d->nsrc; ++i) {
     if (((uintptr_t)d->src[i].ptr + (size_t)d->src[i].c_off * 2) % 16) use_tma = 0;
     for (int ph = 0; use_tma && ph < nph; ++ph)
-      if (!encode_src_map(&maps.m[i * nph + ph], d->src[i], d->N, d->H, d->W, Wh, Hh, nph > 1 ? 2 : 1, ph >> 1, ph & 1, d->dil)) use_tma = 0;
+      if (!encode_src_map(&maps.m[i * nph + ph], d->src[i], d->N, d->H, d->W, Wh, Hh, nph > 1 ? 2 : 1, ph >> 1, ph & 1, d->dil, thin)) use_tma = 0;
   }
   if (!use_tma) memset(&maps, 0, sizeof(maps));
+  if (thin && !use_tma) return cis_set_error(CIS_ERR_UNSUPPORTED, "cis_conv_igemm(halo): the compact thin halo needs the TMA halo path");
   if (nph > 1 && !use_tma) return cis_set_error(CIS_ERR_UNSUPPORTED, "cis_conv_igemm(halo): stride-2 phases need the TMA halo path");
   const int persist_mode = g_persist_mode >= 0 ? g_persist_mode : (getenv("CIS_PERSIST_MODE") ? atoi(getenv("CIS_PERSIST_MODE")) : 1);
   static const int p_min_tiles = getenv("CIS_PERSIST_MIN_TILES") ? atoi(getenv("CIS_PERSIST_MIN_TILES")) : 296;
diff --git a/unsupervised_detection_b200/csrc/misc_kernels.cu b/unsupervised_detection_b200/csrc/misc_kernels.cu
--- a/unsupervised_detection_b200/csrc/misc_kernels.cu
+++ b/unsupervised_detection_b200/csrc/misc_kernels.cu
@@ -34,19 +34,28 @@
   const float v = (km >= 0 && ne >= 0) ? w[(size_t)km + (size_t)ne * sn] : 0.f;
   wp[i] = __float2bfloat16(v);
 }
+__device__ __forceinline__ int tiled_kk(int q, int BN, int layout, int& n) {
+  if (layout) {
+    n = (q >> 3) % BN;
+    return ((q / (BN * 8)) << 3) | (q & 7);
+  }
+  n = q >> 6;
+  const int pos = q & 63;
+  return (((pos >> 3) ^ (n & 7)) << 3) | (pos & 7);
+}
 __device__ __forceinline__ void pack_weights_tiled_body(size_t i, const float* __restrict__ w, const int* __restrict__ kmap, int cin8, int ntaps,
                                                         int n_tiles, int BN, int cout, int sn, const int* __restrict__ nmap,
-                                                        bf16* __restrict__ out) {
+                                                        bf16* __restrict__ out, int layout) {
   const int nchunks = (cin8 + 63) / 64;
-  const size_t total = (size_t)n_tiles * nchunks * ntaps * BN * 64;
+  const int KT = layout ? 16 : 64;
+  const size_t total = (size_t)n_tiles * nchunks * ntaps * BN * KT;
   if (i >= total) return;
-  const int pos = (int)(i % 64);
-  size_t r = i / 64;
-  const int n = (int)(r % BN); r /= BN;
+  size_t r = i / ((size_t)BN * KT);
+  int n;
+  const int kk = tiled_kk((int)(i % ((size_t)BN * KT)), BN, layout, n);
   const int t = (int)(r % ntaps); r /= ntaps;
   const int cc = (int)(r % nchunks);
   const int ny = (int)(r / nchunks);
-  const int kk = (((pos >> 3) ^ (n & 7)) << 3) | (pos & 7);
   const int c = cc * 64 + kk;
   float v = 0.f;
   if (c < cin8) {
@@ -59,13 +68,14 @@
 }
 __device__ __forceinline__ void pack_weights_tiled_tile(int blk, const float* __restrict__ w, const int* __restrict__ kmap, int cin8, int ntaps,
                                                         int n_tiles, int BN, int cout, const int* __restrict__ nmap, bf16* __restrict__ out,
-                                                        float* tile) {
+                                                        float* tile, int layout) {
   const int nchunks = (cin8 + 63) / 64;
+  const int KT = layout ? 16 : 64;
   const int t = blk % ntaps;
   const int r = blk / ntaps;
   const int cc = r % nchunks, ny = r / nchunks;
   const int ld = BN + 1;
-  for (int idx = threadIdx.x; idx < BN * 64; idx += blockDim.x) {
+  for (int idx = threadIdx.x; idx < BN * KT; idx += blockDim.x) {
     const int n = idx % BN, kk = idx / BN;
     const int c = cc * 64 + kk;
     float v = 0.f;
@@ -78,10 +88,10 @@
     tile[kk * ld + n] = v;
   }
   __syncthreads();
-  bf16* o = out + (size_t)blk * BN * 64;
-  for (int idx = threadIdx.x; idx < BN * 64; idx += blockDim.x) {
-    const int pos = idx & 63, n = idx >> 6;
-    const int kk = (((pos >> 3) ^ (n & 7)) << 3) | (pos & 7);
+  bf16* o = out + (size_t)blk * BN * KT;
+  for (int idx = threadIdx.x; idx < BN * KT; idx += blockDim.x) {
+    int n;
+    const int kk = tiled_kk(idx, BN, layout, n);
     o[idx] = __float2bfloat16(tile[kk * ld + n]);
   }
 }
@@ -161,12 +171,12 @@
   pack_weights_body((size_t)blockIdx.x * blockDim.x + threadIdx.x, w, kmap, K_pad, rows, cout, sn, nmap, wp);
 }
 __global__ void pack_weights_tiled_kernel(const float* __restrict__ w, const int* __restrict__ kmap, int cin8, int ntaps, int n_tiles, int BN,
-                                          int cout, int sn, const int* __restrict__ nmap, bf16* __restrict__ out) {
+                                          int cout, int sn, const int* __restrict__ nmap, bf16* __restrict__ out, int layout) {
   pdl_launch_dependents();
   pdl_wait();
   __shared__ float tile[64 * 129];
-  if (sn == 1) pack_weights_tiled_tile(blockIdx.x, w, kmap, cin8, ntaps, n_tiles, BN, cout, nmap, out, tile);
-  else pack_weights_tiled_body((size_t)blockIdx.x * blockDim.x + threadIdx.x, w, kmap, cin8, ntaps, n_tiles, BN, cout, sn, nmap, out);
+  if (sn == 1) pack_weights_tiled_tile(blockIdx.x, w, kmap, cin8, ntaps, n_tiles, BN, cout, nmap, out, tile, layout);
+  else pack_weights_tiled_body((size_t)blockIdx.x * blockDim.x + threadIdx.x, w, kmap, cin8, ntaps, n_tiles, BN, cout, sn, nmap, out, layout);
 }
 __global__ void unpack_wgrad_kernel(const float* __restrict__ dwp, const int* __restrict__ kmap, int K_pad, int cout, int nsplit,
                                     float* __restrict__ dw, const float* __restrict__ colpart, int nblocks, int nch, float* __restrict__ db,
@@ -209,10 +219,10 @@
     case CIS_JOB_PACK_TILED:
       if (j.i[5] == 1)
         pack_weights_tiled_tile(blk, (const float*)j.p[0], (const int*)j.p[1], j.i[0], j.i[1], j.i[2], j.i[3], j.i[4], (const int*)j.p[2],
-                                (bf16*)j.p[3], tile);
+                                (bf16*)j.p[3], tile, j.i[6]);
       else
         pack_weights_tiled_body(i, (const float*)j.p[0], (const int*)j.p[1], j.i[0], j.i[1], j.i[2], j.i[3], j.i[4], j.i[5], (const int*)j.p[2],
-                                (bf16*)j.p[3]);
+                                (bf16*)j.p[3], j.i[6]);
       break;
     case CIS_JOB_UNPACK:
       unpack_wgrad_body(i, (const float*)j.p[0], (const int*)j.p[1], j.i[0], j.i[1], j.i[2], (float*)j.p[2], (const float*)j.p[3], j.i[3], j.i[4],
@@ -1154,11 +1164,12 @@
   return cis_check_launch("pack_weights");
 }
 int cis_pack_weights_tiled(const float* w, const int32_t* kmap, int32_t cin8, int32_t ntaps, int32_t n_tiles, int32_t BN, int32_t cout, int32_t sn,
-                           const int32_t* nmap, void* out, cis_stream_t stream) {
+                           const int32_t* nmap, void* out, int32_t layout, cis_stream_t stream) {
+  if (layout && cin8 != 16) return cis_set_error(CIS_ERR_BAD_ARG, "cis_pack_weights_tiled: layout 1 packs 16 K positions per tile");
   const size_t total = (size_t)n_tiles * ((cin8 + 63) / 64) * ntaps * BN * 64;
   const unsigned blocks = sn == 1 ? (unsigned)(n_tiles * ((cin8 + 63) / 64) * ntaps) : nblk(total);
   if (BN > 128) return cis_set_error(CIS_ERR_UNSUPPORTED, "cis_pack_weights_tiled: BN > 128");
-  CIS_LAUNCH(pack_weights_tiled_kernel, blocks, 256, 0, ST, w, kmap, cin8, ntaps, n_tiles, BN, cout, sn, nmap, (mbf)out);
+  CIS_LAUNCH(pack_weights_tiled_kernel, blocks, 256, 0, ST, w, kmap, cin8, ntaps, n_tiles, BN, cout, sn, nmap, (mbf)out, layout);
   return cis_check_launch("pack_weights_tiled");
 }
 int cis_unpack_wgrad(const float* dwp, const int32_t* kmap, int32_t K_pad, int32_t cout, int32_t nsplit, float* dw, const float* colpart,
diff --git a/unsupervised_detection_b200/csrc/ptx.cuh b/unsupervised_detection_b200/csrc/ptx.cuh
--- a/unsupervised_detection_b200/csrc/ptx.cuh
+++ b/unsupervised_detection_b200/csrc/ptx.cuh
@@ -170,6 +170,7 @@
   return d;
 }
 __device__ __forceinline__ uint32_t desc_hi(uint32_t sbo_bytes) { return ((sbo_bytes >> 4) & 0x3FFF) | (1u << 14) | (2u << 29); }
+__device__ __forceinline__ uint32_t desc_hi_noswz(uint32_t sbo_bytes) { return ((sbo_bytes >> 4) & 0x3FFF) | (1u << 14); }
 __device__ __forceinline__ uint32_t desc_lo(uint32_t saddr, uint32_t lbo_bytes) {
   return ((saddr & 0x3FFFF) >> 4) | (((lbo_bytes >> 4) & 0x3FFF) << 16);
 }
diff --git a/unsupervised_detection_b200/engine.py b/unsupervised_detection_b200/engine.py
--- a/unsupervised_detection_b200/engine.py
+++ b/unsupervised_detection_b200/engine.py
@@ -112,11 +112,11 @@
                 j.kind, blocks = JOB_PACK, -(-(rows * K_pad) // 256)
                 ptrs, ints = [w, kmap, nmap, wp], [K_pad, rows, cout, sn]
             elif name == 'cis_pack_weights_tiled':
-                w, kmap, cin8, ntaps, n_tiles, BN, cout, sn, nmap, out = a
+                w, kmap, cin8, ntaps, n_tiles, BN, cout, sn, nmap, out, layout = a
                 j.kind, blocks = JOB_PACK_TILED, -(-(n_tiles * (-(-cin8 // 64)) * ntaps * BN * 64) // 256)
                 if sn == 1:
                     blocks = n_tiles * (-(-cin8 // 64)) * ntaps
-                ptrs, ints = [w, kmap, nmap, out], [cin8, ntaps, n_tiles, BN, cout, sn]
+                ptrs, ints = [w, kmap, nmap, out], [cin8, ntaps, n_tiles, BN, cout, sn, layout]
             elif name == 'cis_unpack_wgrad':
                 dwp, kmap, K_pad, cout, nsplit, dw, colpart, nblocks, nch, db, layout = a
                 j.kind, blocks = JOB_UNPACK, -(-(cout * K_pad + nch) // 256)
@@ -292,8 +292,8 @@
 SPLITK_MAX = int(os.environ.get('CIS_SPLITK_MAX', '16'))
 SPLITK_NCTA = int(os.environ.get('CIS_SPLITK_NCTA', '64'))
 SPLITK_MIN_UNITS = int(os.environ.get('CIS_SPLITK_MIN_UNITS', '18'))
+HALO_MIN_UTIL = float(os.environ.get('CIS_HALO_MIN_UTIL', '0.2'))
 HALO_SKIP_THIN = int(os.environ.get('CIS_HALO_SKIP_THIN', '0'))
-HALO_MIN_UTIL = float(os.environ.get('CIS_HALO_MIN_UTIL', '0.2'))
 
 
 def setup_splitk(d, device, keep):
@@ -324,6 +324,33 @@
     d.splits, d.sk_scratch, d.sk_counters = splits, sc.data_ptr(), None
 
 
+def thin_items(rel, m_chunks):
+    if m_chunks == 2:
+        return [(a, b, (i, 0), (i, 8)) for i, (a, b) in enumerate(rel)]
+    pos = {t: i for i, t in enumerate(rel)}
+    used, items = set(), []
+    for i in sorted(range(len(rel)), key=lambda q: rel[q]):
+        a, b = rel[i]
+        if i in used:
+            continue
+        used.add(i)
+        j = pos.get((a, b + 1))
+        if j is not None and j not in used:
+            used.add(j)
+            items.append((a, b, (i, 0), (j, 0)))
+        elif b > 0:
+            items.append((a, b - 1, (-1, 0), (i, 0)))
+        else:
+            items.append((a, b, (i, 0), (-1, 0)))
+    return items
+
+
+def _thin_footprint(HP, m_chunks, nmma, BN, nhs):
+    plane = ru(HP * 16, 128)
+    smem = nhs * ru(m_chunks * plane, 1024) + HP * 4 + 1024 + nmma * BN * 32 + 1024
+    return smem, m_chunks * HP * 16 + nmma * BN * 32
+
+
 def setup_halo(d, taps, dil, n_tiles):
     if not HALO_ENABLED or d.sh != 1 or d.sw != 1:
         return False
@@ -340,6 +367,13 @@
     best = None
     ntaps = len(taps)
     m_chunks = sum(d.src[i].chunks for i in range(d.nsrc))
+    thin = m_chunks <= 2 and dil == 1
+    items = None
+    if thin:
+        items = thin_items(rel, m_chunks)
+        if m_chunks == 1:
+            ex = max(ex, max(b for _, b, _, _ in items) + 1)
+        ntaps = len(items)
     if HALO_SKIP_THIN and m_chunks * 8 <= HALO_SKIP_THIN and ntaps >= 16:
         return False
     nchunks = -(-m_chunks // 8)
@@ -353,6 +387,8 @@
         smem = fixed + min(3, ntaps * nchunks) * d.BN * 128 + 1024
         if smem > 227 * 1024:
             continue
+        if thin:
+            smem, opb = _thin_footprint(HP, m_chunks, ntaps, d.BN, 1)
         tiles_y = -(-Hp0 // (16 * MT))
         util = (Hp0 * Wp0) / float(tiles_y * 16 * MT * tiles_x * 8)
         if util < (HALO_MIN_UTIL if dil == 1 else 0.5):
@@ -361,6 +397,8 @@
         cps = max(1, min((225 * 1024) // smem, 512 // _pow2_cols(MT * d.BN), 6))
         t_mma = MT * 2.0 * d.BN * ntaps * nchunks
         t_mem = (d.BN * 128 * ntaps / 40.0 + HP * 128 / 16.0) * nchunks
+        if thin:
+            t_mem = opb / 40.0
         t_cta = max(t_mma, t_mem) + (4000.0 + 1500.0 * MT) / cps
         cost = -(-ncta // (NUM_SMS * cps)) * cps * t_cta / min(cps, max(1.0, ncta / float(NUM_SMS)))
         if PLAN_MODEL == 2:
@@ -377,6 +415,10 @@
     if best is None:
         return False
     d.halo, d.dil, d.MT, d.hoy, d.hox, d.ey, d.ex = 1, dil, best[1], hoy, hox, ey, ex
+    if thin:
+        d.thin = 1
+        _fill_taps(d, [(a, b) for a, b, _, _ in items])
+        return items
     _fill_taps(d, rel)
     return True
 
@@ -385,17 +427,33 @@
 
 
 def setup_halo_s2(d, taps, n_tiles):
-    if not (HALO_ENABLED and S2_HALO) or d.sh != 2 or d.sw != 2:
+    if not HALO_ENABLED or d.sh != 2 or d.sw != 2:
         return None
-    if any(d.src[i].chunks % 8 for i in range(d.nsrc - 1)):
+    m_chunks = sum(d.src[i].chunks for i in range(d.nsrc))
+    thin = m_chunks <= 2
+    if not (thin or S2_HALO):
+        return None
+    if not thin and any(d.src[i].chunks % 8 for i in range(d.nsrc - 1)):
         return None
     ph = [((u % 2) * 2 + (v % 2), u // 2, v // 2) for u, v in taps]
     order = sorted(range(len(taps)), key=lambda i: (ph[i][0], i))
     hoy, hox = min(a for _, a, _ in ph), min(b for _, _, b in ph)
     rel = [(ph[i][1] - hoy, ph[i][2] - hox) for i in order]
     ey, ex = max(a for a, _ in rel), max(b for _, b in rel)
-    m_chunks = sum(d.src[i].chunks for i in range(d.nsrc))
     nchunks = -(-m_chunks // 8)
+    nmma, items, bounds = len(taps), None, [0]
+    if thin:
+        items = []
+        for q in range(4):
+            idx = [k for k in range(len(order)) if ph[order[k]][0] == q]
+            for a, b, h0, h1 in thin_items([rel[k] for k in idx], m_chunks):
+                items.append((a, b) + tuple((order[idx[t]] if t >= 0 else -1, c) for t, c in (h0, h1)))
+            bounds.append(len(items))
+        if m_chunks == 1:
+            ex = max(ex, max(b for _, b, _, _ in items) + 1)
+        nmma = len(items)
+        if HALO_SKIP_THIN and m_chunks * 8 <= HALO_SKIP_THIN and nmma >= 16:
+            return None
     tiles_x = -(-d.OW // 8)
     best = None
     for MT in (1, 2, 3, 4):
@@ -405,14 +463,18 @@
         smem = 2 * ru(HP * 128, 1024) + HP * 4 + 2048 + 2 * d.BN * 128
         if smem > 227 * 1024:
             continue
+        if thin:
+            smem, opb = _thin_footprint(HP, m_chunks, nmma, d.BN, 2)
         tiles_y = -(-d.OH // (16 * MT))
         util = (d.OH * d.OW) / float(tiles_y * 16 * MT * tiles_x * 8)
         if util < HALO_MIN_UTIL:
             continue
         ncta = d.N * tiles_x * tiles_y * n_tiles
         cps = max(1, min((225 * 1024) // smem, 512 // _pow2_cols(MT * d.BN), 4))
-        t_mma = MT * 2.0 * d.BN * len(taps) * nchunks
+        t_mma = MT * 2.0 * d.BN * nmma * nchunks
         t_mem = (d.BN * 128 * len(taps) / 40.0 + 4 * HP * 128 / 40.0) * nchunks
+        if thin:
+            t_mem = 4 * opb / 40.0
         t_cta = max(t_mma, t_mem) + (4000.0 + 1500.0 * MT) / cps
         cost = -(-ncta // (NUM_SMS * cps)) * cps * t_cta / min(cps, max(1.0, ncta / float(NUM_SMS)))
         if best is None or cost < best[0] - 1e-9:
@@ -421,11 +483,14 @@
         return None
     d.halo, d.dil, d.MT, d.hoy, d.hox, d.ey, d.ex = 1, 1, best[1], hoy, hox, ey, ex
     d.sh = d.sw = 1
-    _fill_taps(d, rel)
     d.nph = 4
-    bounds = [0]
-    for q in range(4):
-        bounds.append(bounds[-1] + sum(1 for i in order if ph[i][0] == q))
+    if thin:
+        d.thin, d.thin_items = 1, items
+        _fill_taps(d, [(a, b) for a, b, _, _ in items])
+    else:
+        _fill_taps(d, rel)
+        for q in range(4):
+            bounds.append(bounds[-1] + sum(1 for i in order if ph[i][0] == q))
     for q in range(5):
         d.ph_tap[q] = bounds[q]
     return order
@@ -440,7 +505,7 @@
         return None
     d0 = descs[0]
     same = ('N', 'H', 'W', 'BN', 'n_tiles', 'nsrc', 'act', 'DH', 'DW', 'osh', 'osw', 'out', 'out_pitch', 'out_coff', 'out_ch', 'outf', 'outf_pitch',
-            'outf_coff', 'outf_ch', 'add_pre', 'add_pre_pitch', 'add_pre_coff', 'add_post', 'addf_pre', 'mode', 'bias')
+            'outf_coff', 'outf_ch', 'add_pre', 'add_pre_pitch', 'add_pre_coff', 'add_post', 'addf_pre', 'mode', 'bias', 'thin')
     for d in descs:
         if not d.halo or d.dil != 1 or d.splits > 1 or d.nph > 1 or any(getattr(d, f) != getattr(d0, f) for f in same):
             return None
@@ -570,14 +635,29 @@
         nchunks = -(-cin8 // 64)
         return torch.zeros(n_tiles * nchunks * ntaps * BN * 64, dtype=torch.bfloat16, device=self.device)
 
-    def fwd_tiles_buf(self, tap_order=None):
+    def _thin_tiles(self, items, tap_ids, chanmap, per_tap_stride, chan_stride, BN, n_tiles):
+        km = np.full(len(items) * 16, -1, dtype=np.int32)
+        for it, (_, _, h0, h1) in enumerate(items):
+            for h, (t, c0) in enumerate((h0, h1)):
+                if t < 0:
+                    continue
+                for e in range(8):
+                    if c0 + e < len(chanmap) and chanmap[c0 + e] >= 0:
+                        km[it * 16 + h * 8 + e] = tap_ids[t] * per_tap_stride + chanmap[c0 + e] * chan_stride
+        return torch.from_numpy(km).to(self.device), torch.zeros(n_tiles * len(items) * BN * 16, dtype=torch.bfloat16, device=self.device)
+
+    def fwd_tiles_buf(self, tap_order=None, items=None):
         if getattr(self, 'fwd_tiles', None) is None:
-            self.fwd_tiles = self._alloc_tiles(self.k * self.k, len(self.in_chanmap), self.BN, self.n_tiles)
-            self.fwd_tiles_kmap = self.fwd_kmap
-            if tap_order is not None:
-                self.fwd_tiles_kmap, _ = self._kmap(list(tap_order), self.in_chanmap, self.cin * self.cout, self.cout)
-            self.fwd_tap_order = tap_order
-        assert getattr(self, 'fwd_tap_order', None) == tap_order, self.name
+            if items is not None:
+                self.fwd_tiles_kmap, self.fwd_tiles = self._thin_tiles(items, range(self.k * self.k), self.in_chanmap, self.cin * self.cout,
+                                                                       self.cout, self.BN, self.n_tiles)
+            else:
+                self.fwd_tiles = self._alloc_tiles(self.k * self.k, len(self.in_chanmap), self.BN, self.n_tiles)
+                self.fwd_tiles_kmap = self.fwd_kmap
+                if tap_order is not None:
+                    self.fwd_tiles_kmap, _ = self._kmap(list(tap_order), self.in_chanmap, self.cin * self.cout, self.cout)
+            self.fwd_tap_order, self.fwd_items = tap_order, items
+        assert getattr(self, 'fwd_tap_order', None) == tap_order and getattr(self, 'fwd_items', None) == items, self.name
         return self.fwd_tiles
 
     def w_src_ptr(self):
@@ -594,25 +674,34 @@
         if self.fwd_pack is not None:
             if self.transposed:
                 for pk in self.tr_packs:
-                    if pk.get('wt') is not None:
+                    if pk.get('wt') is not None and pk.get('items'):
+                        plan.add('cis_pack_weights_tiled', self.w_src_ptr(), pk['tkmap'].data_ptr(), 16, len(pk['items']),
+                                 self.n_tiles, self.BN, self.cout, self.cin, None, pk['wt'].data_ptr(), 1)
+                    elif pk.get('wt') is not None:
                         plan.add('cis_pack_weights_tiled', self.w_src_ptr(), pk['kmap'].data_ptr(), len(self.in_chanmap), len(pk['taps']),
-                                 self.n_tiles, self.BN, self.cout, self.cin, None, pk['wt'].data_ptr())
+                                 self.n_tiles, self.BN, self.cout, self.cin, None, pk['wt'].data_ptr(), 0)
                     if pk.get('rows_used', True):
                         plan.add('cis_pack_weights', self.w_src_ptr(), pk['kmap'].data_ptr(), pk['K_pad'], self.npad, self.cout, self.cin,
                                  None, pk['w'].data_ptr())
             else:
-                if getattr(self, 'fwd_tiles', None) is not None:
+                if getattr(self, 'fwd_tiles', None) is not None and self.fwd_items:
+                    plan.add('cis_pack_weights_tiled', self.w_src_ptr(), self.fwd_tiles_kmap.data_ptr(), 16, len(self.fwd_items),
+                             self.n_tiles, self.BN, self.cout, 1, None, self.fwd_tiles.data_ptr(), 1)
+                elif getattr(self, 'fwd_tiles', None) is not None:
                     plan.add('cis_pack_weights_tiled', self.w_src_ptr(), self.fwd_tiles_kmap.data_ptr(), len(self.in_chanmap), self.k * self.k,
-                             self.n_tiles, self.BN, self.cout, 1, None, self.fwd_tiles.data_ptr())
+                             self.n_tiles, self.BN, self.cout, 1, None, self.fwd_tiles.data_ptr(), 0)
                 if getattr(self, 'fwd_rows_used', True):
                     plan.add('cis_pack_weights', self.w_src_ptr(), self.fwd_kmap.data_ptr(), self.K_pad, self.npad, self.cout, 1,
                              None, self.fwd_pack.data_ptr())
         if dgrad and self.dgrad_packs:
             cout8 = ru(self.cout, 8)
             for pk in self.dgrad_packs:
-                if pk.get('wt') is not None:
+                if pk.get('wt') is not None and pk.get('items'):
+                    plan.add('cis_pack_weights_tiled', self.w_src_ptr(), pk['tkmap'].data_ptr(), 16, len(pk['items']), pk['n_tiles'], pk['BN'],
+                             len(self.in_chanmap), self.cout, pk['nmap'].data_ptr(), pk['wt'].data_ptr(), 1)
+                elif pk.get('wt') is not None:
                     plan.add('cis_pack_weights_tiled', self.w_src_ptr(), pk['kmap'].data_ptr(), cout8, len(pk['taps']), pk['n_tiles'], pk['BN'],
-                             len(self.in_chanmap), self.cout, pk['nmap'].data_ptr(), pk['wt'].data_ptr())
+                             len(self.in_chanmap), self.cout, pk['nmap'].data_ptr(), pk['wt'].data_ptr(), 0)
                 if pk.get('rows_used', True):
                     plan.add('cis_pack_weights', self.w_src_ptr(), pk['kmap'].data_ptr(), pk['K_pad'], pk['rows'], len(self.in_chanmap),
                              self.cout, pk['nmap'].data_ptr(), pk['w'].data_ptr())
@@ -657,7 +746,7 @@
                         tl.append(r * k + c)
                         offs.append(((a + pt - r * d) // s, (b + pl - c * d) // s))
                 kmap, Kp = self._kmap(tl, g_chan, self.cin * self.cout, 1)
-                packs.append(dict(a=a, b=b, taps=offs, kmap=kmap, K_pad=Kp, rows=rows, BN=bn_, n_tiles=nt, nmap=nmap,
+                packs.append(dict(a=a, b=b, taps=offs, tl=tl, chan=g_chan, kmap=kmap, K_pad=Kp, rows=rows, BN=bn_, n_tiles=nt, nmap=nmap,
                                   w=torch.zeros(rows, Kp, dtype=torch.bfloat16, device=self.device)))
         self.dgrad_packs = packs
 
@@ -677,7 +766,7 @@
                         tl.append(ky * 4 + kx)
                         offs.append(((a + 1 - ky) // 2, (b + 1 - kx) // 2))
                 kmap, Kp = self._kmap(tl, chanmap, self.cout * self.cin, 1)
-                packs.append(dict(a=a, b=b, taps=offs, kmap=kmap, K_pad=Kp,
+                packs.append(dict(a=a, b=b, taps=offs, tl=tl, kmap=kmap, K_pad=Kp,
                                   w=torch.zeros(self.npad, Kp, dtype=torch.bfloat16, device=self.device)))
         self.tr_packs = packs
         self.fwd_pack = True
@@ -755,11 +844,12 @@
             d.add_post, d.add_post_pitch, d.add_post_coff = post_add.ptr, post_add.pitch, post_add.c_off
         d.mode = mode
         order = setup_halo_s2(d, taps, layer.n_tiles) if (layer.stride == 2 and layer.dil == 1) else None
+        hl = layer.stride == 1 and order is None and setup_halo(d, taps, layer.dil, layer.n_tiles)
         if order is not None:
-            d.wpack = layer.fwd_tiles_buf(order).data_ptr()
+            d.wpack = layer.fwd_tiles_buf(order, getattr(d, 'thin_items', None)).data_ptr()
             layer.fwd_rows_used = getattr(layer, 'fwd_rows_used', False)
-        elif layer.stride == 1 and setup_halo(d, taps, layer.dil, layer.n_tiles):
-            d.wpack = layer.fwd_tiles_buf().data_ptr()
+        elif hl:
+            d.wpack = layer.fwd_tiles_buf(None, hl if hl is not True else None).data_ptr()
             layer.fwd_rows_used = getattr(layer, 'fwd_rows_used', False)
         else:
             layer.fwd_rows_used = True
@@ -879,9 +969,16 @@
             d.out, d.out_pitch, d.out_coff, d.out_ch = tgt.ptr, tgt.pitch, tgt.c_off, tgt.C8
             if acc:
                 d.add_pre, d.add_pre_pitch, d.add_pre_coff = tgt.ptr, tgt.pitch, tgt.c_off
-            if setup_halo(d, pk['taps'], layer.dil if s == 1 else 1, pk['n_tiles']):
+            hl = setup_halo(d, pk['taps'], layer.dil if s == 1 else 1, pk['n_tiles'])
+            if hl:
+                items = hl if hl is not True else None
                 if pk.get('wt') is None:
-                    pk['wt'] = layer._alloc_tiles(len(pk['taps']), ru(layer.cout, 8), pk['BN'], pk['n_tiles'])
+                    pk['items'] = items
+                    if items:
+                        pk['tkmap'], pk['wt'] = layer._thin_tiles(items, pk['tl'], pk['chan'], layer.cin * layer.cout, 1, pk['BN'], pk['n_tiles'])
+                    else:
+                        pk['wt'] = layer._alloc_tiles(len(pk['taps']), ru(layer.cout, 8), pk['BN'], pk['n_tiles'])
+                assert pk['items'] == items, layer.name
                 d.wpack = pk['wt'].data_ptr()
                 pk['rows_used'] = pk.get('rows_used', False)
             else:
@@ -983,9 +1080,17 @@
             d.out, d.out_pitch, d.out_coff, d.out_ch = out.ptr, out.pitch, out.c_off, layer.cout
             if outf is not None:
                 d.outf, d.outf_pitch, d.outf_coff, d.outf_ch = outf.data_ptr(), outf.shape[-1], 0, layer.cout
-            if setup_halo(d, pk['taps'], 1, layer.n_tiles):
+            hl = setup_halo(d, pk['taps'], 1, layer.n_tiles)
+            if hl:
+                items = hl if hl is not True else None
                 if pk.get('wt') is None:
-                    pk['wt'] = layer._alloc_tiles(len(pk['taps']), len(layer.in_chanmap), layer.BN, layer.n_tiles)
+                    pk['items'] = items
+                    if items:
+                        pk['tkmap'], pk['wt'] = layer._thin_tiles(items, pk['tl'], layer.in_chanmap, layer.cout * layer.cin, 1, layer.BN,
+                                                                  layer.n_tiles)
+                    else:
+                        pk['wt'] = layer._alloc_tiles(len(pk['taps']), len(layer.in_chanmap), layer.BN, layer.n_tiles)
+                assert pk['items'] == items, layer.name
                 d.wpack = pk['wt'].data_ptr()
                 pk['rows_used'] = pk.get('rows_used', False)
             else:
```

Measured after the change: 1041, median of 6. 5.6% higher.
